# CookiePPP/cookietts

Hardware: AMD Instinct MI355X
Metric: audio samples/sec (22.05kHz) WaveGlow infer, 80×900 mel, 1/2/4/8 GPU; real-time factor (higher is better)
Workload: dtype f32; 1 GPU; WaveGlow full (12 flows, 512 WN ch, 8 groups, 8 layers) fp32 infer, batch 8 x (80x900) mel per GPU, sigma 0.6, random-init weights; batch_per_gpu=8, frames=900, parallelism=utterance-batch shard x1

## Files before the change

cookietts_amd/_lib.py:

```python
from __future__ import annotations

import ctypes as C
import os
import threading

import torch

from . import build as _build

_LOCK = threading.Lock()
_LIB = None


class WaveGlowConfig(C.Structure):
    _fields_ = [(n, C.c_int32) for n in (
        "n_mel_channels", "n_group", "n_flows", "n_early_every", "n_early_size",
        "win_length", "hop_length", "n_layers", "n_channels", "kernel_size", "cond_hidden", "speaker_embed_dim",
        "f32_gemm_mode")]


class StftConfig(C.Structure):
    _fields_ = [("filter_length", C.c_int32), ("hop_length", C.c_int32), ("win_length", C.c_int32),
                ("n_mel_channels", C.c_int32), ("clamp_val", C.c_float)]

# ... 70 lines not shown


class TorchMojiConfig(C.Structure):
    _fields_ = [(n, C.c_int32) for n in ("nb_tokens", "embedding_dim", "hidden_size")]


class TorchMojiWeights(C.Structure):
    _fields_ = [("embed", _FP), ("lstm", (LstmWeights * 2) * 2), ("attention_vector", _FP)]


class TacoDecoderWeights(C.Structure):
    _fields_ = [("bottleneck_w", _FP), ("memory_layer_w", _FP), ("query_w", _FP), ("v_w", _FP), ("loc_conv_w", _FP),
                ("loc_dense_w", _FP), ("prenet_w1", _FP), ("prenet_w2", _FP),
                ("att_rnn", LstmWeights), ("dec_rnn", LstmWeights), ("dec2_rnn", LstmWeights),
                ("proj_w", _FP), ("proj_b", _FP), ("gate_w", _FP), ("gate_b", _FP),
                ("windowed_att_pos_offset", C.c_float), ("exp_smoothing_factor", C.c_float)]


class Conv1dDesc(C.Structure):
    _fields_ = [("c_in", C.c_int32), ("c_out", C.c_int32), ("kernel_size", C.c_int32), ("act", C.c_int32),
                ("slope", C.c_float), ("f32_gemm_mode", C.c_int32)]


class HifiganConfig(C.Structure):
    MAX_UPS, MAX_KERNELS, MAX_DILATIONS = 8, 4, 3
    _fields_ = [(n, C.c_int32) for n in ("num_mels", "upsample_initial_channel", "resblock", "n_ups", "n_kernels")] + [
        ("upsample_rates", C.c_int32 * 8), ("upsample_kernel_sizes", C.c_int32 * 8), ("resblock_kernel_sizes", C.c_int32 * 4),
        ("resblock_dilation_sizes", (C.c_int32 * 3) * 4)]


class TacoMemoryWeights(C.Structure):
    _fields_ = [(n, _FP) for n in ("sylps_w", "sylps_b", "speaker_embedding", "syl_w0", "syl_b0", "syl_w2", "syl_b2",
                                   "syl_res_weight", "tm_gamma", "tm_beta", "tm_mean", "tm_var", "tm_w", "tm_b")]


class RetryConfig(C.Structure):
    _fields_ = [(n, C.c_double) for n in ("diagonality_weighting", "max_focus_weighting", "min_focus_weighting",
                                          "avg_focus_weighting", "target_score", "absolutely_required_score")] + [
        (n, C.c_int32) for n in ("max_attempts", "absolute_maximum_tries", "n_texts", "per_text", "n_mel", "t_cap", "enc_cap")]


class RetryStatus(C.Structure):
    _fields_ = [("done", C.c_int32), ("n_passes", C.c_int32), ("min_best_score", C.c_double), ("min_tries", C.c_int32),
                ("n_without_winner", C.c_int32), ("max_best_length", C.c_int32), ("max_best_T", C.c_int32)]


class MelErrorConfig(C.Structure):
    _fields_ = [("n_windows", C.c_int32), ("filter_lengths", C.c_int32 * 8), ("hop_length", C.c_int32),
                ("n_mel_channels", C.c_int32), ("framing", C.c_int32), ("clamp_val", C.c_float), ("mag_eps", C.c_float)]


class TacoLossParams(C.Structure):
    _fields_ = [("gate_positive_weight", C.c_double), ("sigma", C.c_double), ("weights", C.c_double * 9)]


_CFG = C.POINTER(WaveGlowConfig)
SIGNATURES = {
    "ctts_abi_version": (C.c_int, []),
    "ctts_last_error": (C.c_char_p, []),
    "ctts_waveglow_geometry_for": (C.c_int, [_CFG, C.c_int32, C.POINTER(WaveGlowGeometry)]),
    "ctts_fold_weightnorm_f32": (C.c_int, [_FP, _FP, _FP, C.c_int32, C.c_int32, _FP]),
    "ctts_waveglow_packed_bytes": (C.c_size_t, [_CFG]),
    "ctts_waveglow_pack_upsample": (C.c_int, [_CFG, _FP, _FP, _FP, _FP]),
    "ctts_waveglow_pack_flow": (C.c_int, [_CFG, C.c_int32, C.POINTER(WaveGlowFlowWeights), _FP, _FP]),
    "ctts_waveglow_workspace_bytes": (C.c_size_t, [_CFG, C.c_int32, C.c_int32]),
    "ctts_waveglow_infer_f32": (C.c_int, [_CFG, _FP, _FP, _FP, _FP, C.c_int32, C.c_int32, _FP, C.c_size_t, _FP]),
    "ctts_waveglow_infer_spk_f32": (C.c_int, [_CFG, _FP, _FP, _FP, _FP, _FP, C.c_int32, C.c_int32, _FP, C.c_size_t, _FP]),
    "ctts_waveglow_infer_spk_bf16": (C.c_int, [_CFG, _FP, _FP, _FP, _FP, _FP, _FP, C.c_int32, C.c_int32, _FP, C.c_size_t,
                                              _FP]),
    "ctts_waveglow_infer_spk_bf16x3": (C.c_int, [_CFG, _FP, _FP, _FP, _FP, _FP, _FP, C.c_int32, C.c_int32, _FP, C.c_size_t,
                                               _FP]),
    "ctts_waveglow_infer_spk_f16": (C.c_int, [_CFG, _FP, _FP, _FP, _FP, _FP, _FP, C.c_int32, C.c_int32, _FP, C.c_size_t,
                                             _FP]),
    "ctts_waveglow_pack_flow_f16": (C.c_int, [_CFG, C.c_int32, C.POINTER(WaveGlowFlowWeights), _FP, _FP]),
    "ctts_waveglow_packed_bf16x3_bytes": (C.c_size_t, [_CFG]),
    "ctts_waveglow_pack_flow_bf16x3": (C.c_int, [_CFG, C.c_int32, C.POINTER(WaveGlowFlowWeights), _FP, _FP]),
    "ctts_waveglow_workspace_bf16x3_bytes": (C.c_size_t, [_CFG, C.c_int32, C.c_int32]),
    "ctts_waveglow_packed_bf16_bytes": (C.c_size_t, [_CFG]),
    "ctts_waveglow_pack_flow_bf16": (C.c_int, [_CFG, C.c_int32, C.POINTER(WaveGlowFlowWeights), _FP, _FP]),
    "ctts_waveglow_workspace_bf16_bytes": (C.c_size_t, [_CFG, C.c_int32, C.c_int32]),
    "ctts_waveglow_infer_bf16": (C.c_int, [_CFG, _FP, _FP, _FP, _FP, _FP, C.c_int32, C.c_int32, _FP, C.c_size_t, _FP]),
    "ctts_upsample_squeeze_f32": (C.c_int, [_CFG, _FP, _FP, _FP, C.c_int32, C.c_int32, _FP]),
    "ctts_wn_cond_f32": (C.c_int, [_CFG, _FP, _FP, _FP, _FP, _FP, C.c_int32, C.c_int32, _FP]),
    "ctts_wn_stack_f32": (C.c_int, [_CFG, _FP, C.c_int32, _FP, _FP, _FP, _FP, _FP, C.c_int32, C.c_int32, _FP]),
    "ctts_flow_tail_f32": (C.c_int, [_CFG, _FP, C.c_int32, _FP, _FP, _FP, C.c_int32, C.c_int32, _FP]),
    "ctts_waveglow_flow_f32": (C.c_int, [_CFG, _FP, C.c_int32, _FP, _FP, _FP, C.c_int32, C.c_int32, _FP, C.c_size_t, _FP]),
    "ctts_waveglow_forward_packed_bytes": (C.c_size_t, [_CFG]),
    "ctts_waveglow_pack_forward_mix": (C.c_int, [_CFG, C.c_int32, _FP, _FP, _FP]),
    "ctts_waveglow_forward_workspace_bytes": (C.c_size_t, [_CFG, C.c_int32, C.c_int32]),
    "ctts_waveglow_forward_spk_f32": (C.c_int, [_CFG, _FP, _FP, _FP, _FP, _FP, _FP, _FP, _FP, C.c_int32, C.c_int32, _FP,
                                               C.c_size_t, _FP]),
    "ctts_waveglow_flow_forward_f32": (C.c_int, [_CFG, _FP, _FP, C.c_int32, _FP, _FP, _FP, _FP, _FP, C.c_int32, C.c_int32, _FP,
                                                C.c_size_t, _FP]),
    "ctts_waveflow_packed_bytes": (C.c_size_t, [C.POINTER(WaveFlowConfig)]),
    "ctts_waveflow_pack_flow": (C.c_int, [C.POINTER(WaveFlowConfig), C.c_int32, C.POINTER(WaveFlowFlowWeights), _FP, _FP]),
    "ctts_waveflow_workspace_bytes": (C.c_size_t, [C.POINTER(WaveFlowConfig), C.c_int32, C.c_int32]),
    "ctts_waveflow_inverse_f32": (C.c_int, [C.POINTER(WaveFlowConfig), _FP, _FP, _FP, _FP, C.c_int32, C.c_int32,
                                            C.c_int32, _FP, C.c_size_t, _FP]),
    "ctts_taco_decoder_packed_bytes": (C.c_size_t, [C.POINTER(TacoDecoderConfig)]),
    "ctts_taco_decoder_pack": (C.c_int, [C.POINTER(TacoDecoderConfig), C.POINTER(TacoDecoderWeights), _FP, _FP]),
    "ctts_taco_decoder_max_batch": (C.c_int32, [C.POINTER(TacoDecoderConfig)]),
    "ctts_taco_decoder_workspace_bytes": (C.c_size_t, [C.POINTER(TacoDecoderConfig), C.c_int32, C.c_int32]),
    "ctts_taco_decoder_init_f32": (C.c_int, [C.POINTER(TacoDecoderConfig), _FP, _FP, _FP, C.c_int32, C.c_int32, _FP,
                                             C.c_size_t, _FP]),
    "ctts_taco_decoder_steps_f32": (C.c_int, [C.POINTER(TacoDecoderConfig), _FP, _FP, _FP, _FP, _FP, C.c_int32,
                                              C.c_int32, C.c_int32, C.c_int32, C.c_int32, _FP, _FP]),
    "ctts_taco_decoder_steps_hidden_f32": (C.c_int, [C.POINTER(TacoDecoderConfig), _FP, _FP, _FP, _FP, _FP, _FP, C.c_int32,
                                                     C.c_int32, C.c_int32, C.c_int32, C.c_int32, _FP, _FP]),
    "ctts_taco_decoder_packed_bf16x3_bytes": (C.c_size_t, [C.POINTER(TacoDecoderConfig)]),
    "ctts_taco_decoder_pack_bf16x3": (C.c_int, [C.POINTER(TacoDecoderConfig), C.POINTER(TacoDecoderWeights), _FP, _FP]),
    "ctts_taco_decoder_steps_bf16x3": (C.c_int, [C.POINTER(TacoDecoderConfig), _FP, _FP, _FP, _FP, _FP, _FP, C.c_int32,
                                                 C.c_int32, C.c_int32, C.c_int32, C.c_int32, _FP, _FP]),
    "ctts_taco_prenet_frames_bytes": (C.c_size_t, [C.POINTER(TacoDecoderConfig), C.c_int32, C.c_int32]),
    "ctts_taco_prenet_frames_f32": (C.c_int, [C.POINTER(TacoDecoderConfig), _FP, _FP, _FP, _FP, _FP, C.c_size_t, C.c_int32,
                                              C.c_int32, _FP]),
    "ctts_taco_decoder_steps_forced_f32": (C.c_int, [C.POINTER(TacoDecoderConfig), _FP, _FP, _FP, _FP, C.c_int32, C.c_int32,
                                                     C.c_int32, C.c_int32, C.c_int32, _FP, C.c_size_t, _FP]),
    "ctts_taco_decoder_steps_forced_bf16x3": (C.c_int, [C.POINTER(TacoDecoderConfig), _FP, _FP, _FP, _FP, C.c_int32, C.c_int32,
                                                        C.c_int32, C.c_int32, C.c_int32, _FP, C.c_size_t, _FP]),
    "ctts_taco_project_frames_f32": (C.c_int, [C.POINTER(TacoDecoderConfig), _FP, _FP, _FP, _FP, C.c_int32, C.c_int32, _FP]),
    "ctts_taco_decoder_persistent_bytes": (C.c_size_t, [C.POINTER(TacoDecoderConfig), C.c_int32, C.c_int32]),
    "ctts_taco_decoder_steps_persistent_f32": (C.c_int, [C.POINTER(TacoDecoderConfig), _FP, _FP, _FP, _FP, _FP, C.c_int32,
                                                         C.c_int32, C.c_int32, C.c_int32, C.c_int32, _FP, _FP, C.c_size_t,
                                                         _FP]),
    "ctts_taco_decoder_persistent_debug": (C.c_int, [_FP]),
    "ctts_conv1d_packed_bytes": (C.c_size_t, [C.POINTER(Conv1dDesc)]),
    "ctts_conv1d_pack_f32": (C.c_int, [C.POINTER(Conv1dDesc), _FP, _FP, _FP, _FP, _FP, _FP, C.c_float, _FP, _FP]),
    "ctts_conv1d_f32": (C.c_int, [C.POINTER(Conv1dDesc), _FP, _FP, _FP, C.c_int32, C.c_int32, C.c_int32, C.c_int32,
                                  C.c_int32, _FP]),
    "ctts_lstm_seq_packed_bytes": (C.c_size_t, [C.c_int32, C.c_int32]),
    "ctts_lstm_seq_pack_f32": (C.c_int, [C.POINTER(LstmWeights), C.c_int32, C.c_int32, _FP, _FP]),
    "ctts_lstm_seq_workspace_bytes": (C.c_size_t, [C.c_int32, C.c_int32, C.c_int32]),
    "ctts_lstm_seq_f32": (C.c_int, [_FP, _FP, _FP, C.c_int32, _FP, C.c_int64, C.c_int32, C.c_int32, _FP, C.c_int32,
                                    C.c_int32, C.c_int32, C.c_int32, C.c_int32, C.c_int32, C.c_int32, C.c_int32, _FP,
                                    C.c_size_t, _FP]),
    "ctts_lstm_biseq_f32": (C.c_int, [_FP, _FP, _FP, _FP, _FP, C.c_int64, C.c_int32, C.c_int32, C.c_int32, _FP, C.c_int32,
                                      C.c_int32, C.c_int32, C.c_int32, C.c_int32, C.c_int32, C.c_int32, C.c_int32, C.c_int32,
                                      _FP, _FP, C.c_size_t, _FP]),
    "ctts_lstm_biseq_hardsig_f32": (C.c_int, [_FP, _FP, _FP, _FP, _FP, C.c_int64, C.c_int32, C.c_int32, C.c_int32, _FP, C.c_int32,
                                              C.c_int32, C.c_int32, C.c_int32, C.c_int32, C.c_int32, C.c_int32, C.c_int32,
                                              C.c_int32, _FP, _FP, C.c_size_t, _FP]),
    "ctts_torchmoji_packed_bytes": (C.c_size_t, [C.POINTER(TorchMojiConfig)]),
    "ctts_torchmoji_pack_f32": (C.c_int, [C.POINTER(TorchMojiConfig), C.POINTER(TorchMojiWeights), _FP, _FP]),
    "ctts_torchmoji_workspace_bytes": (C.c_size_t, [C.POINTER(TorchMojiConfig), C.c_int32, C.c_int32]),
    "ctts_torchmoji_lengths": (C.c_int, [_FP, _FP, C.c_int32, C.c_int32, _FP]),
    "ctts_torchmoji_features_f32": (C.c_int, [C.POINTER(TorchMojiConfig), _FP, _FP, _FP, _FP, _FP, C.c_int32, C.c_int32, _FP,
                                              C.c_size_t, _FP]),
    "ctts_attention_pool_f32": (C.c_int, [_FP, _FP, _FP, _FP, _FP, C.c_int32, C.c_int32, C.c_int32, _FP]),
    "ctts_taco_embed_f32": (C.c_int, [_FP, _FP, _FP, _FP, _FP, C.c_int32, C.c_int32, C.c_int32, C.c_int32, C.c_int32,
                                      C.c_int32, _FP]),
    "ctts_taco_memory_f32": (C.c_int, [C.POINTER(TacoMemoryWeights), _FP, _FP, _FP, _FP, _FP, C.c_int32, C.c_int32,
                                       C.c_int32, C.c_int32, C.c_int32, C.c_int32, C.c_int32, _FP]),
    "ctts_taco_memory_sylps_f32": (C.c_int, [C.POINTER(TacoMemoryWeights), _FP, _FP, _FP, _FP, _FP, _FP, C.c_int32, C.c_int32,
                                             C.c_int32, C.c_int32, C.c_int32, C.c_int32, C.c_int32, _FP]),
    "ctts_pad_rows_f32": (C.c_int, [_FP, C.c_int64, C.c_int32, _FP, C.c_int32, C.c_int32, C.c_int32, C.c_int32,
                                    C.c_int32, _FP]),
    "ctts_unpad_rows_f32": (C.c_int, [_FP, _FP, C.c_int64, C.c_int32, C.c_int32, C.c_int32, C.c_int32, C.c_int32,
                                      C.c_int32, _FP]),
    "ctts_stft_packed_bytes": (C.c_size_t, [C.POINTER(StftConfig)]),
    "ctts_stft_pack": (C.c_int, [C.POINTER(StftConfig), _FP, _FP, _FP, _FP]),
    "ctts_stft_workspace_bytes": (C.c_size_t, [C.POINTER(StftConfig), C.c_int32, C.c_int32]),
    "ctts_stft_mel_f32": (C.c_int, [C.POINTER(StftConfig), _FP, _FP, _FP, _FP, C.c_int32, C.c_int32, _FP,
                                    C.c_size_t, _FP]),
    "ctts_stft_pack_inverse": (C.c_int, [C.POINTER(StftConfig), _FP, _FP, _FP, _FP]),
    "ctts_stft_transform_f32": (C.c_int, [C.POINTER(StftConfig), _FP, _FP, _FP, _FP, C.c_int32, C.c_int32, _FP,
                                          C.c_size_t, _FP]),
# ... 15 lines not shown
    "ctts_wgax_packed_bytes": (C.c_size_t, [C.POINTER(WgaxConfig)]),
    "ctts_wgax_pack_flow": (C.c_int, [C.POINTER(WgaxConfig), C.c_int32, C.POINTER(WgaxFlowWeights), _FP, _FP]),
    "ctts_wgax_workspace_bytes": (C.c_size_t, [C.POINTER(WgaxConfig), C.c_int32, C.c_int64]),
    "ctts_wgax_inverse_f32": (C.c_int, [C.POINTER(WgaxConfig), _FP, _FP, _FP, C.c_int32, C.c_int32, C.c_int32, _FP,
                                        C.c_int32, C.c_int64, _FP, C.c_size_t, _FP]),
    "ctts_wgax_packed_f16_bytes": (C.c_size_t, [C.POINTER(WgaxConfig)]),
    "ctts_wgax_pack_flow_f16": (C.c_int, [C.POINTER(WgaxConfig), C.c_int32, C.POINTER(WgaxFlowWeights), _FP, _FP]),
    "ctts_wgax_workspace_f16_bytes": (C.c_size_t, [C.POINTER(WgaxConfig), C.c_int32, C.c_int64]),
    "ctts_wgax_inverse_f16": (C.c_int, [C.POINTER(WgaxConfig), _FP, _FP, _FP, C.c_int32, C.c_int32, C.c_int32, _FP,
                                        C.c_int32, C.c_int64, _FP, C.c_size_t, _FP]),
    "ctts_wgax_sep_packed_bytes": (C.c_size_t, [C.POINTER(WgaxConfig)]),
    "ctts_wgax_sep_pack_flow": (C.c_int, [C.POINTER(WgaxConfig), C.c_int32, C.POINTER(WgaxFlowWeights), C.POINTER(_FP),
                                          C.POINTER(_FP), _FP, _FP]),
    "ctts_wgax_sep_workspace_bytes": (C.c_size_t, [C.POINTER(WgaxConfig), C.c_int32, C.c_int64]),
    "ctts_wgax_sep_inverse_f32": (C.c_int, [C.POINTER(WgaxConfig), _FP, _FP, _FP, C.c_int32, C.c_int32, C.c_int32, _FP,
                                            C.c_int32, C.c_int64, _FP, C.c_size_t, _FP]),
    "ctts_depthwise_conv1d_f32": (C.c_int, [_FP, _FP, _FP, _FP] + [C.c_int32] * 7 + [_FP]),
    "ctts_hifigan_weight_floats": (C.c_size_t, [C.POINTER(HifiganConfig)]),
    "ctts_hifigan_packed_bytes": (C.c_size_t, [C.POINTER(HifiganConfig)]),
    "ctts_hifigan_pack_f32": (C.c_int, [C.POINTER(HifiganConfig), _FP, C.c_size_t, _FP, _FP]),
    "ctts_hifigan_workspace_bytes": (C.c_size_t, [C.POINTER(HifiganConfig), C.c_int32, C.c_int32]),
    "ctts_hifigan_forward_f32": (C.c_int, [C.POINTER(HifiganConfig), _FP, _FP, C.c_int32, _FP, C.c_int32, C.c_int32, _FP,
                                           C.c_size_t, _FP]),
    "ctts_hifigan_packed_f16_bytes": (C.c_size_t, [C.POINTER(HifiganConfig)]),
    "ctts_hifigan_pack_f16": (C.c_int, [C.POINTER(HifiganConfig), _FP, C.c_size_t, _FP, _FP]),
    "ctts_hifigan_workspace_f16_bytes": (C.c_size_t, [C.POINTER(HifiganConfig), C.c_int32, C.c_int32]),
    "ctts_hifigan_forward_f16": (C.c_int, [C.POINTER(HifiganConfig), _FP, _FP, C.c_int32, _FP, C.c_int32, C.c_int32, _FP,
                                           C.c_size_t, _FP]),
    "ctts_hifigan_packed_bf16x3_bytes": (C.c_size_t, [C.POINTER(HifiganConfig)]),
    "ctts_hifigan_pack_bf16x3": (C.c_int, [C.POINTER(HifiganConfig), _FP, C.c_size_t, _FP, _FP]),
    "ctts_hifigan_workspace_bf16x3_bytes": (C.c_size_t, [C.POINTER(HifiganConfig), C.c_int32, C.c_int32]),
    "ctts_hifigan_forward_bf16x3": (C.c_int, [C.POINTER(HifiganConfig), _FP, _FP, C.c_int32, _FP, C.c_int32, C.c_int32, _FP,
                                              C.c_size_t, _FP]),
    "ctts_replicate_halo_f32":(C.c_int, [_FP, C.c_int32, C.c_int32, C.c_int32, C.c_int32, C.c_int32, C.c_int32, _FP]),
    "ctts_embed_rows_f32": (C.c_int, [_FP, _FP, _FP, C.c_int32, C.c_int32, C.c_int32, C.c_int32, C.c_int32, C.c_int32,
                                      C.c_int32, _FP]),
    "ctts_scale_add_rows_f32": (C.c_int, [_FP, _FP, _FP, _FP, C.c_int32, C.c_int32, C.c_int32, C.c_int32, C.c_int32,
                                          _FP]),
    "ctts_deemphasis_f32": (C.c_int, [_FP, _FP, C.c_int32, C.c_int32, C.c_double, _FP]),
    "ctts_alignment_workspace_bytes": (C.c_size_t, [C.c_int32, C.c_int32, C.c_int32]),
    "ctts_alignment_metric_f32": (C.c_int, [_FP, _FP, _FP, C.c_int32, C.c_int32, C.c_int32, C.c_float, _FP, _FP,
                                            C.c_size_t, _FP]),
    "ctts_alignment_metric_masked_f32": (C.c_int, [_FP, _FP, _FP, _FP, C.c_int32, C.c_int32, C.c_int32, C.c_float, _FP, _FP,
                                                   C.c_size_t, _FP]),
    "ctts_first_over_thresh_f32": (C.c_int, [_FP, C.c_int32, C.c_int32, C.c_float, _FP, _FP]),
    "ctts_taco_loss_workspace_bytes": (C.c_size_t, [C.c_int32] * 4),
    "ctts_taco_loss_f32": (C.c_int, [C.POINTER(TacoLossParams)] + [_FP] * 13 + [C.c_int32] * 4 + [_FP, _FP, _FP, C.c_size_t,
                                                                                                  _FP]),
    "ctts_taco_loss_finalize_f32": (C.c_int, [C.POINTER(TacoLossParams)] + [_FP] * 9 + [C.c_int32] * 4 + [_FP, _FP, _FP,
                                                                                                          C.c_size_t, _FP]),
    "ctts_mel_error_packed_bytes": (C.c_size_t, [C.POINTER(MelErrorConfig)]),
    "ctts_mel_error_pack": (C.c_int, [C.POINTER(MelErrorConfig), C.c_int32, _FP, _FP, _FP, _FP]),
    "ctts_mel_error_workspace_bytes": (C.c_size_t, [C.POINTER(MelErrorConfig)] + [C.c_int32] * 3),
    "ctts_mel_error_f32": (C.c_int, [C.POINTER(MelErrorConfig)] + [_FP] * 6 + [C.c_int32] * 5 + [_FP] * 4 + [C.c_int32, _FP,
                                                                                                     C.c_size_t, _FP]),
    "ctts_taco_stop_state_bytes": (C.c_size_t, [C.c_int32]),
    "ctts_taco_stop_reset": (C.c_int, [_FP, C.c_int32, C.c_int32, _FP]),
    "ctts_taco_stop_rule_f32": (C.c_int, [_FP, C.c_int32, C.c_int32, C.c_int32, C.c_int32, C.c_float, C.c_int32, _FP, _FP]),
    "ctts_retry_state_bytes": (C.c_size_t, [C.POINTER(RetryConfig)]),
    "ctts_retry_state_layout": (C.c_int, [C.POINTER(RetryConfig), C.POINTER(C.c_size_t)]),
    "ctts_retry_reset": (C.c_int, [C.POINTER(RetryConfig), _FP, _FP]),
    "ctts_retry_update_f32": (C.c_int, [C.POINTER(RetryConfig), _FP, _FP, _FP, _FP, _FP, _FP, C.c_int32, C.c_int32, _FP, _FP,
                                        _FP]),
    "ctts_retry_vocoder_batch_f32": (C.c_int, [C.POINTER(RetryConfig), _FP, _FP, C.c_int32, C.c_float, _FP]),
    "ctts_pcm16_concat": (C.c_int, [_FP, C.c_int32, _FP, C.c_int32, C.c_int64, C.c_int32, C.c_int32, _FP, C.c_int64, _FP,
                                    _FP]),
    "ctts_affine_rows_f32": (C.c_int, [_FP, C.c_int32, C.c_int32, C.c_int32, C.c_int32, C.c_int32, C.c_int32, C.c_float,
                                       C.c_float, _FP]),
    "ctts_vol_unscale_f32": (C.c_int, [_FP, C.c_int64, _FP]),
    "ctts_resample_rows_f32": (C.c_int, [_FP, _FP] + [C.c_int32] * 9 + [C.c_float, _FP]),
    "ctts_interleave_phases_f32": (C.c_int, [_FP, _FP] + [C.c_int32] * 10 + [_FP]),
    "ctts_last_gemm_loop": (C.c_int, []),
    "ctts_last_winograd_f43_width": (C.c_int, []),
    "ctts_tuning_reload": (C.c_int, []),
    "ctts_tuning_flags": (C.c_int, []),
    "ctts_profile_create": (C.c_int, [C.POINTER(C.c_void_p)]),
    "ctts_profile_bind": (C.c_int, [C.c_void_p]),
    "ctts_profile_collect": (C.c_int, [C.c_void_p, C.c_int32, C.POINTER(C.c_int64), C.POINTER(C.c_double)]),
    "ctts_profile_destroy": (C.c_int, [C.c_void_p]),
}

MODEL_GEMM_MODES = {None: 0, "default": 0, "f32": 1, "bf16x3": 2, "bf16x6": 3}
GEMM_MODES = {"f32": 1, "bf16x3": 2, "bf16x6": 3}


def model_gemm_mode(mode):
    try:
        return MODEL_GEMM_MODES[mode]
    except KeyError:
        raise ValueError(f"f32 GEMM mode {mode!r}: expected one of 'default', 'f32', 'bf16x3', 'bf16x6'") from None


def set_f32_gemm_mode(mode):
    if mode in (None, "default", "f32"):
        return "f32"
    raise RuntimeError(f"cookietts_amd.set_f32_gemm_mode({mode!r}): the process-wide default was removed; "
                       f"call model.set_f32_gemm_mode({mode!r}) on each model instead")


class Profile:

    def __init__(self):
        h = C.c_void_p()
        check(lib().ctts_profile_create(C.byref(h)), "ctts_profile_create")
        self._h = h

    def __enter__(self):
        check(lib().ctts_profile_bind(self._h), "ctts_profile_bind")
        return self

    def __exit__(self, *exc):
        check(lib().ctts_profile_bind(None), "ctts_profile_bind")
        return False

    bind = __enter__

    def unbind(self):
        self.__exit__()

    def collect(self, which):
        n, ms = C.c_int64(), C.c_double()
        check(lib().ctts_profile_collect(self._h, which, C.byref(n), C.byref(ms)), "ctts_profile_collect")
        return int(n.value), float(ms.value)

    def close(self):
        if self._h is not None and _LIB is not None:
            _LIB.ctts_profile_destroy(self._h)
        self._h = None

    def __del__(self):
        try:
            self.close()
        except Exception:
            pass


TUNING_BITS = {"CTTS_F32_NO_GLDS": 0, "CTTS_GEMM_NO_XCD_PAIR": 1, "CTTS_F32_WINOGRAD_FUSED_MIN": 2, "CTTS_BF16_NO_WIDE": 3, "CTTS_BF16_NO_PP": 4,
               "CTTS_F32_WINOGRAD_NO_FUSED": 5, "CTTS_F32_WINOGRAD_F43_MIN": 6, "CTTS_WF_NO_FUSE": 7,
               "CTTS_TACO_NO_FUSE": 8, "CTTS_F32_NO_SMALL": 9, "CTTS_F32_FORCE_SMALL": 10, "CTTS_F32_NO_SPLITK": 11, "CTTS_WF_NO_VEC_INTERP": 12,
               "CTTS_F32_NO_DEFER_SKIP": 13, "CTTS_WF_NO_REGION_SPLIT": 14, "CTTS_WF_NO_ROW_QUEUE": 15, "CTTS_WF_ROW_QUEUE_MIN": 16,
               "CTTS_WF_INJECT_ABORT": 17, "CTTS_WF_QUEUE_DEBUG": 18, "CTTS_F32_NO_ROUND_SPLIT": 19, "CTTS_BF16_PS": 20, "CTTS_BF16_NO_PS": 21,
               "CTTS_F32_WINOGRAD_NO_F43": 22,
               "CTTS_TACO_POLL_DELAY": 23, "CTTS_TACO_VALU": 24, "CTTS_UP_NO_MFMA": 25, "CTTS_F32_NO_WN_FOLD": 26, "CTTS_TACO_BG_NO_PIPE": 27,
               "CTTS_F32_NO_WINOGRAD": 28, "CTTS_F32_WINOGRAD_MIN": 29, "CTTS_F32_WINOGRAD_PLAIN": 30}
TUNING_BITS_EXT = {"CTTS_WF_FWD_ROWWISE": 31}


def tuning_reload():
    check(lib().ctts_tuning_reload(), "ctts_tuning_reload")


def tuning_active(name):
    bit = TUNING_BITS[name] if name in TUNING_BITS else TUNING_BITS_EXT[name]
    return bool(lib().ctts_tuning_flags() >> bit & 1)


PROF_WN_IN = 0
PROF_WN_RS = 1
PROF_WN_SKIP = 2
PROF_WN_IN0F = 3
PROF_WN_SKEND = 4
PROF_WN_RES_F = 5


class HipLibraryError(RuntimeError):
    pass
# ... 61 lines not shown
```

cookietts_amd/csrc/gemm_f32.h:

```cpp
#pragma once

#include "common.h"

namespace ctts {

constexpr int GEMM_KC = 16;
constexpr int GEMM_MAX_SEG = 12;

constexpr int GEMM_BM = 256;
constexpr int GEMM_BN = 128;
inline int gemm_bn(int bm) { return bm == 256 ? 128 : 256; }

enum GemmEpilogue : int {
    GEMM_EPI_SPLIT = 0,
    GEMM_EPI_GATE = 1,
    GEMM_EPI_MAG = 2,
    GEMM_EPI_LOG = 3,
    GEMM_EPI_LRELU = 4,
    GEMM_EPI_TANH = 5,
    GEMM_EPI_GATEX = 7,
    GEMM_EPI_GATE_RS = 6,
};

__host__ __device__ inline bool gemm_epi_is_pair(int epi) {
    return epi == GEMM_EPI_GATE || epi == GEMM_EPI_MAG || epi == GEMM_EPI_GATE_RS || epi == GEMM_EPI_GATEX;
}

enum GateKind : int {
    GATE_GTU = 0,
    GATE_GTRU = 1,
    GATE_GTLRU = 2,
    GATE_GLU = 3,
    GATE_TTU = 4,
    GATE_STU = 5,
    GATE_GTSU = 6,
    GATE_SPTU = 7,
    GATE_GSIU = 8,
    GATE_GSIRU = 9,
    GATE_GTSRU = 10,
    GATE_GSIRRU = 11,
    GATE_GSIRLRU = 12,
    GATE_GSIRRLRU = 13,
    GATE_KINDS = 14
};

#if defined(__HIPCC__)
__device__ __forceinline__ float gemm_lerp(float l0, float a, float l1, float b) { return __builtin_fmaf(l0, a, l1 * b); }

template <int KIND>
__device__ __forceinline__ float gate_eval(float u0, float u1) {
    float f, g;
    if constexpr (KIND == GATE_GLU) f = u0;
    else if constexpr (KIND == GATE_GTSU || KIND == GATE_GTSRU) f = u0 - tanhf(u0);
    else if constexpr (KIND == GATE_GSIU) f = __sinf(u0);
    else if constexpr (KIND == GATE_GSIRU || KIND == GATE_GSIRRU || KIND == GATE_GSIRLRU || KIND == GATE_GSIRRLRU) f = __sinf(16.0f * u0);
    else f = tanhf(u0);
    if constexpr (KIND == GATE_GTRU || KIND == GATE_GTSRU || KIND == GATE_GSIRRU) g = fmaxf(u1, 0.0f);
    else if constexpr (KIND == GATE_GTLRU || KIND == GATE_GSIRLRU) g = u1 > 0.0f ? u1 : 0.01f * u1;
    else if constexpr (KIND == GATE_GSIRRLRU) g = u1 >= 0.0f ? u1 : ((0.01f + 0.1f) / 2.0f) * u1;
    else if constexpr (KIND == GATE_TTU) g = tanhf(u1);
    else if constexpr (KIND == GATE_STU)
        g = 1.0507009873554804934193349852946f * (fmaxf(u1, 0.0f) + fminf(0.0f, 1.6732632423543772848170429916717f * expm1f(u1)));
    else if constexpr (KIND == GATE_SPTU) g = u1 > 20.0f ? u1 : log1pf(expf(u1));
    else g = 1.0f / (1.0f + expf(-u1));
    return f * g;
}
#endif

struct GemmSeg {
    const float* base;
    long long bstride;
    int nch;
    int shift;
    int mb_rows;
    int fresh;
};

struct GemmArgs {
    const float* A;
    const float* bias;
    GemmSeg seg[GEMM_MAX_SEG];
    int nseg;
    int interleave;
    int nch_total;
    int a_nch_alloc;
    int a_ch_off;
    int bm;
    int ld, pad, L;
    int ntiles, MB, batch;
    int M;
    float* dst0; long long dst0_bstride; int acc0;
    const float* src0; long long src0_bstride;
    float* dst1; long long dst1_bstride; int acc1;
    int split;
    int pairC;
    int dst_ld, dst_pad;
    float clip;
    const float* addend; long long addend_bstride;
    int addend_ld, addend_pad;
    int addend_frames;
    const float* addend2; float addend2_sign;
    int map_d, map_par, map_L, map_col0;
    int map_mode;
    int gate;
    int gemm_mode;
    const float* rs_wT;
    const float* rs_bias;
    int rs_rows;
    int gt_limit;
    long long shape_blocks;
    int parts;
    long long part_A, part_seg[4], part_dst0;
    int mseg, mseg_ld, mseg_pad;
    int mseg_ch0, mseg_ch1;
};

__host__ __device__ inline int gemm_dense_row(int epi, int bm, int mb, int r, int C, int M) {
    if (gemm_epi_is_pair(epi)) {
        const int wm = r >> 7, rr = r & 127;
        const int c = (mb * (bm >> 7) + wm) * 64 + (rr & 63);
        if (c >= C) return -1;
        return (rr < 64) ? c : C + c;
    }
    const int row = mb * bm + r;
    return row < M ? row : -1;
}

inline void gemm_apply_defaults(GemmArgs& a) {
    if (a.bm == 0) a.bm = 256;
    if (a.addend_ld == 0) { a.addend_ld = a.ld; a.addend_pad = a.pad; }
}
bool gemm_f32_dma_staged(int nch_total);
int gemm_check_args(int epi, const GemmArgs& a);
int launch_gemm_f32(int epi, const GemmArgs& a, hipStream_t stream);
bool gemm_f32_small_applies(int epi, const GemmArgs& a);
int launch_gemm_f32_small(int epi, const GemmArgs& a, hipStream_t stream);

bool wf_row_persistent_supported(const GemmArgs& a);
int wf_row_cus();
int wf_row_tiles(int L, int body);
struct WfTailDesc;
int launch_wf_row_persistent(const GemmArgs* layers_dev, const WfTailDesc* tails_dev, int nrows, int nlayers, int max_nseg, int L,
                             int batch, int body, unsigned int* counter, unsigned int* flags, unsigned int* abort_word,
                             unsigned int epoch, hipStream_t stream);

int launch_wf_all_rows_layer(const GemmArgs* rows_dev, int nrows, int max_nseg, int L, int batch, hipStream_t stream);

int get_gemm_f32_mode();
void note_gemm_loop(int code);
int last_gemm_loop();
bool gemm_mode_is_split(int gemm_mode);
inline bool gemm_mode_valid(int m) { return m == CTTS_GEMM_DEFAULT || m == CTTS_GEMM_F32 || m == CTTS_GEMM_BF16X3 || m == CTTS_GEMM_BF16X6; }
int gemm_split_level(int gemm_mode);

}
```

cookietts_amd/csrc/gemm_f32.hip:

```cpp
#include <atomic>
#include <cstdlib>
#include <mutex>

#include "gemm_f32.h"
#include "tuning.h"
#include "gemm_bf16.h"

namespace ctts {

typedef float f32x16 __attribute__((ext_vector_type(16)));

namespace {

constexpr int STAGE = GEMM_KC * (256 + 128);
constexpr int GEMM_GLDS_MAX_CHUNKS = 384;

__device__ __forceinline__ float fast_sigmoid(float u) {
    return __builtin_amdgcn_rcpf(1.0f + __builtin_amdgcn_exp2f(u * -1.4426950408889634f));
}
__device__ __forceinline__ float fast_tanh(float u) {
    return 1.0f - 2.0f * __builtin_amdgcn_rcpf(1.0f + __builtin_amdgcn_exp2f(u * 2.8853900817779268f));
}

typedef const __attribute__((address_space(1))) float* gfloat_ptr;
__device__ __forceinline__ float4 load4u(gfloat_ptr p) {
    float4 v;
    v.x = p[0]; v.y = p[1]; v.z = p[2]; v.w = p[3];
    return v;
}

template <int EPI>
__device__ __forceinline__ void split_epilogue(const GemmArgs& a, f32x16 (&acc)[4][2], const float* bias, int M, int row0,
                                               int b, int ncol0, int l31, int lhi, long long part_dst0 = 0) {
#pragma unroll
    for (int mt = 0; mt < 4; ++mt) {
        const int rbase = row0 + mt * 32;
        if (rbase >= M) continue;
        const bool second = rbase >= a.split;
        float* dst = second ? a.dst1 + (size_t)b * a.dst1_bstride : a.dst0 + part_dst0 + (size_t)b * a.dst0_bstride;
        const float* src = second ? dst : (a.src0 ? a.src0 + (size_t)b * a.src0_bstride : dst);
        const int accum = second ? a.acc1 : a.acc0;
        const int rdst = second ? rbase - a.split : rbase;
        float old[2][16];
        if (accum && rbase + 32 <= M) {
#pragma unroll
            for (int nt = 0; nt < 2; ++nt)
#pragma unroll
                for (int r = 0; r < 16; ++r) {
                    const int row = (r & 3) + 8 * (r >> 2) + 4 * lhi;
                    old[nt][r] = src[(size_t)(rdst + row) * a.dst_ld + a.dst_pad + ncol0 + nt * 32 + l31];
                }
        } else if (accum) {
#pragma unroll
            for (int nt = 0; nt < 2; ++nt)
#pragma unroll
                for (int r = 0; r < 16; ++r) {
                    const int row = (r & 3) + 8 * (r >> 2) + 4 * lhi;
                    old[nt][r] = rbase + row < M ? src[(size_t)(rdst + row) * a.dst_ld + a.dst_pad + ncol0 + nt * 32 + l31] : 0.0f;
                }
        } else {
#pragma unroll
            for (int nt = 0; nt < 2; ++nt)
#pragma unroll
                for (int r = 0; r < 16; ++r) old[nt][r] = 0.0f;
        }
#pragma unroll
        for (int nt = 0; nt < 2; ++nt) {
            const int n = ncol0 + nt * 32 + l31;
            if (n < a.L) {
#pragma unroll
                for (int r = 0; r < 16; ++r) {
                    const int row = (r & 3) + 8 * (r >> 2) + 4 * lhi;
                    float v = acc[mt][nt][r] + bias[(rbase - row0) + row] + old[nt][r];
                    if constexpr (EPI == GEMM_EPI_LOG) v = logf(fmaxf(v, a.clip));
                    if constexpr (EPI == GEMM_EPI_LRELU) v = v > 0.f ? v : a.clip * v;
                    if constexpr (EPI == GEMM_EPI_TANH) v = tanhf(v);
                    if (rbase + row < M) dst[(size_t)(rdst + row) * a.dst_ld + a.dst_pad + n] = v;
                }
            }
        }
    }
}

typedef __bf16 bf16x8_t __attribute__((ext_vector_type(8)));
typedef unsigned int u32x4_t __attribute__((ext_vector_type(4)));
__device__ __forceinline__ void split8(const float (&v)[8], u32x4_t& hi, u32x4_t& lo) {
#pragma unroll
    for (int j = 0; j < 4; ++j) {
        const unsigned int h = pack_bf16x2(v[2 * j], v[2 * j + 1]);
        hi[j] = h;
        lo[j] = pack_bf16x2(v[2 * j] - __builtin_bit_cast(float, h << 16), v[2 * j + 1] - __builtin_bit_cast(float, h & 0xffff0000u));
    }
}

__device__ __forceinline__ void split8x3(const float (&v)[8], u32x4_t& hi, u32x4_t& mid, u32x4_t& lo) {
#pragma unroll
    for (int j = 0; j < 4; ++j) {
        const unsigned int h = pack_bf16x2(v[2 * j], v[2 * j + 1]);
        const float r0 = v[2 * j] - __builtin_bit_cast(float, h << 16), r1 = v[2 * j + 1] - __builtin_bit_cast(float, h & 0xffff0000u);
        const unsigned int m = pack_bf16x2(r0, r1);
        hi[j] = h;
        mid[j] = m;
        lo[j] = pack_bf16x2(r0 - __builtin_bit_cast(float, m << 16), r1 - __builtin_bit_cast(float, m & 0xffff0000u));
    }
}

template <int EPI, int WM, int SEGS, bool GLDS, int XS = 0, bool EXT = false>
__global__ __launch_bounds__(256, 2) void conv_gemm_f32_kernel(const GemmArgs a) {
    static_assert(!EXT || (GLDS && SEGS == 4 && XS == 0 && (EPI == GEMM_EPI_SPLIT || EPI == GEMM_EPI_GATE)),
                  "parts / mapped segment: DMA-staged fp32 loop, <= 4 segments, SPLIT or GATE");
    constexpr bool X3 = XS != 0;
    constexpr bool X6 = XS == 6;
    static_assert(XS == 0 || XS == 3 || XS == 6, "main loop: fp32 MFMA, 3 or 6 bf16 products");
    static_assert(!X3 || GLDS, "the split-bf16 loop is built on the DMA-staged pipeline");
    constexpr int NST = GLDS ? 3 : 2;
    constexpr int SEGTAB = NST * STAGE;
    constexpr int CHTAB = SEGTAB + GEMM_MAX_SEG * 4;
    constexpr int LDS_FLOATS = CHTAB + (GLDS ? 2 * GEMM_GLDS_MAX_CHUNKS : 0);
    constexpr int BM = 128 * WM;
    constexpr int WN = 4 / WM;
    constexpr int BN = 64 * WN;
    constexpr int A_STAGE = GEMM_KC * BM;
    constexpr int NA = BM / 64;
    constexpr int NB = BN / 64;
    __shared__ __attribute__((aligned(16))) float lds[LDS_FLOATS];

    const int t = threadIdx.x;
    const int lane = t & 63;
    const int wave = GLDS ? __builtin_amdgcn_readfirstlane(t >> 6) : (t >> 6);
    const int wm = wave / WN, wn = wave % WN;
    const int l31 = lane & 31, lhi = lane >> 5;

    int id = blockIdx.x;
    int mb, tile, b;
    if (a.map_mode == 1) {
        const int x = id & 7, j = id >> 3;
        mb = 2 * (x & 1) + (j & 1);
        const int gt = (j >> 1) * 4 + (x >> 1);
        if (gt >= a.gt_limit) return;
        tile = gt % a.ntiles;
        b = gt / a.ntiles;
    } else {
        mb = id % a.MB;
        id /= a.MB;
        tile = id % a.ntiles;
        b = id / a.ntiles;
    }
    const int n0 = tile * BN;
    [[maybe_unused]] int part = 0;
    if constexpr (EXT) {
        if (b >= a.batch) { part = 1; b -= a.batch; }
    }
#define CTTS_MAP_PAR (EXT && a.parts > 1 ? part : a.map_par)
#define CTTS_A_PTR (EXT ? a.A + (long long)part * a.part_A : a.A)

    gfloat_ptr sbase[4];
    int snch[4];
    if constexpr (SEGS == 4) {
#pragma unroll
        for (int sidx = 0; sidx < 4; ++sidx) {
            const GemmSeg& g = a.seg[sidx];
            sbase[sidx] = (gfloat_ptr)(g.base + (size_t)b * g.bstride + (size_t)(mb * g.mb_rows) * a.ld +
                                       (a.pad + n0 + g.shift));
            snch[sidx] = sidx < a.nseg ? g.nch : 0x7fffffff;
        }
    } else {
#pragma unroll
        for (int sidx = 0; sidx < GEMM_MAX_SEG; ++sidx) {
            if (t == sidx) {
                const GemmSeg& g = a.seg[sidx];
                unsigned int* e = reinterpret_cast<unsigned int*>(lds + SEGTAB + sidx * 4);
                if (sidx < a.nseg) {
                    const float* base = g.base + (size_t)b * g.bstride + (size_t)(mb * g.mb_rows) * a.ld +
                                        (a.pad + n0 + g.shift);
                    const unsigned long long u = reinterpret_cast<unsigned long long>(base);
                    e[0] = (unsigned int)u;
                    e[1] = (unsigned int)(u >> 32);
                    e[2] = (unsigned int)g.nch;
                } else {
                    e[0] = 0; e[1] = 0; e[2] = 0x7fffffffu;
                }
                e[3] = 0;
            }
        }
    }

    const int nalloc = a.a_nch_alloc ? a.a_nch_alloc : a.nch_total;
    const float* ap = CTTS_A_PTR + ((size_t)mb * nalloc + a.a_ch_off) * A_STAGE + t * 4;

    constexpr int UPR = BN / 4;
    constexpr int RPP = 64 / UPR;
    const int brow = GLDS ? wave * RPP + lane / UPR : t >> 4;
    const int bcol = GLDS ? (lane % UPR) * 4 : (t & 15) * 4;
    const size_t thread_off = (size_t)brow * a.ld + bcol;
    const size_t piece_stride = (size_t)4 * RPP * a.ld;
    const size_t chunk_rows = (size_t)GEMM_KC * a.ld;

    f32x16 acc[4][2];
#pragma unroll
    for (int i = 0; i < 4; ++i)
#pragma unroll
        for (int j = 0; j < 2; ++j)
#pragma unroll
            for (int r = 0; r < 16; ++r) acc[i][j][r] = 0.0f;

    float4 ra0, ra1, ra2, ra3, rb0, rb1, rb2, rb3;
    int seg = 0, local = 0;
    const int ilv = a.interleave > 1 ? a.interleave : 0;
    bool in_ilv = ilv > 0;
    if constexpr (SEGS != 4) __syncthreads();
    if constexpr (GLDS) {
        unsigned long long* tab = reinterpret_cast<unsigned long long*>(lds + CHTAB);
        const int ilv0 = a.interleave > 1 ? a.interleave : 0;
        const int n_il = ilv0 * a.seg[0].nch;
        for (int c0 = t; c0 < a.nch_total; c0 += 256) {
            int c = c0, sg, loc;
            if (c < n_il) {
                sg = c % ilv0;
// ... 339 lines not shown
                            }                                                                                     \
                            break;
                        switch (a.gate) {
                            CTTS_GATEX_LOOP(1) CTTS_GATEX_LOOP(2) CTTS_GATEX_LOOP(3) CTTS_GATEX_LOOP(4) CTTS_GATEX_LOOP(5)
                            CTTS_GATEX_LOOP(6) CTTS_GATEX_LOOP(7) CTTS_GATEX_LOOP(8) CTTS_GATEX_LOOP(9) CTTS_GATEX_LOOP(10)
                            CTTS_GATEX_LOOP(11) CTTS_GATEX_LOOP(12) CTTS_GATEX_LOOP(13)
                            default:
                            CTTS_GATEX_LOOP(0)
                        }
#undef CTTS_GATEX_LOOP
                    } else {
                        float add20[16], add21[16];
                        if (EPI == GEMM_EPI_GATE && a.addend2) {
                            const float* ad = a.addend2 + (size_t)b * a.addend_bstride + a.addend_pad + n;
#pragma unroll
                            for (int r = 0; r < 16; ++r) {
                                const int c = min(cbase + mt * 32 + (r & 3) + 8 * (r >> 2) + 4 * lhi, a.pairC - 1);
                                add20[r] = (EXT && part ? -a.addend2_sign : a.addend2_sign) * ad[(size_t)c * a.addend_ld];
                                add21[r] = (EXT && part ? -a.addend2_sign : a.addend2_sign) * ad[(size_t)(a.pairC + c) * a.addend_ld];
                            }
                        }
#pragma unroll
                        for (int r = 0; r < 16; ++r) {
                            const int row = (r & 3) + 8 * (r >> 2) + 4 * lhi;
                            const int c = cbase + mt * 32 + row;
                            float u0 = acc[mt][nt][r] + bias[mt * 32 + row] + add0[r];
                            float u1 = acc[mt + 2][nt][r] + bias[64 + mt * 32 + row] + add1[r];
                            if (EPI == GEMM_EPI_GATE && a.addend2) { u0 += add20[r]; u1 += add21[r]; }
                            float v;
                            if constexpr (EPI == GEMM_EPI_GATE) v = fast_tanh(u0) * fast_sigmoid(u1);
                            else v = sqrtf(u0 * u0 + u1 * u1);
                            if (c < a.pairC && ns_ok) dst[(size_t)c * a.dst_ld + a.dst_pad + ns] = v;
                        }
                    }
                }
            }
        }
    } else if constexpr (EPI == GEMM_EPI_GATE_RS) {
        static_assert(EPI != GEMM_EPI_GATE_RS || WM == 1, "fused res/skip needs the 128-row block shape");
        float actv[2][2][16];
#pragma unroll
        for (int mt = 0; mt < 2; ++mt)
#pragma unroll
            for (int nt = 0; nt < 2; ++nt)
#pragma unroll
                for (int r = 0; r < 16; ++r) {
                    const int row = (r & 3) + 8 * (r >> 2) + 4 * lhi;
                    const bool ok = mt * 32 + row < a.pairC;
                    float u0 = acc[mt][nt][r] + bias[mt * 32 + row];
                    float u1 = acc[mt + 2][nt][r] + bias[64 + mt * 32 + row];
                    if (a.addend) {
                        const float* ad = a.addend + (size_t)b * a.addend_bstride + a.addend_pad + n0 + wn * 64 + nt * 32 + l31;
                        const int c = min(mt * 32 + row, a.pairC - 1);
                        u0 += ad[(size_t)c * a.addend_ld];
                        u1 += ad[(size_t)(a.pairC + c) * a.addend_ld];
                    }
                    actv[mt][nt][r] = ok ? fast_tanh(u0) * fast_sigmoid(u1) : 0.0f;
                }
        __syncthreads();
        for (int i = t * 4; i < 64 * 128; i += 1024)
            *reinterpret_cast<float4*>(lds + i) = *reinterpret_cast<const float4*>(a.rs_wT + i);
        if (t < 128) lds[64 * 128 + t] = a.rs_bias[t];
        __syncthreads();
#pragma unroll
        for (int i = 0; i < 4; ++i)
#pragma unroll
            for (int j = 0; j < 2; ++j)
#pragma unroll
                for (int r = 0; r < 16; ++r) acc[i][j][r] = 0.0f;
#pragma unroll
        for (int s = 0; s < 32; ++s) {
            const int r = s & 15;
            const int ch = (s >> 4) * 32 + (r & 3) + 8 * (r >> 2) + 4 * lhi;
            float a2[4];
#pragma unroll
            for (int mt = 0; mt < 4; ++mt) a2[mt] = lds[ch * 128 + mt * 32 + l31];
#pragma unroll
            for (int mt = 0; mt < 4; ++mt)
#pragma unroll
                for (int nt = 0; nt < 2; ++nt)
                    acc[mt][nt] = __builtin_amdgcn_mfma_f32_32x32x2f32(a2[mt], actv[s >> 4][nt][r], acc[mt][nt], 0, 0, 0);
        }
        split_epilogue<GEMM_EPI_SPLIT>(a, acc, lds + 64 * 128, a.rs_rows, 0, b, n0 + wn * 64, l31, lhi);
    } else {
        split_epilogue<EPI>(a, acc, bias, a.M, mb * BM + wm * 128, b, n0 + wn * 64, l31, lhi, EXT ? (long long)part * a.part_dst0 : 0);
    }
#undef CTTS_MAP_PAR
#undef CTTS_A_PTR
}

inline int gemm_f32_mode() { return CTTS_GEMM_F32; }

template <int EPI, int XS>
void launch_shape_xs(int bm, dim3 grid, hipStream_t stream, const GemmArgs& a) {
    const bool few = a.nseg <= 4;
    if (bm == 128) {
        if (few) hipLaunchKernelGGL((conv_gemm_f32_kernel<EPI, 1, 4, true, XS>), grid, dim3(256), 0, stream, a);
        else hipLaunchKernelGGL((conv_gemm_f32_kernel<EPI, 1, GEMM_MAX_SEG, true, XS>), grid, dim3(256), 0, stream, a);
    } else {
        if (few) hipLaunchKernelGGL((conv_gemm_f32_kernel<EPI, 2, 4, true, XS>), grid, dim3(256), 0, stream, a);
        else hipLaunchKernelGGL((conv_gemm_f32_kernel<EPI, 2, GEMM_MAX_SEG, true, XS>), grid, dim3(256), 0, stream, a);
    }
}

template <int EPI, bool GLDS>
void launch_shape_g(int bm, dim3 grid, hipStream_t stream, const GemmArgs& a) {
    const bool few = a.nseg <= 4;
    if (bm == 128) {
        if (few) hipLaunchKernelGGL((conv_gemm_f32_kernel<EPI, 1, 4, GLDS>), grid, dim3(256), 0, stream, a);
        else hipLaunchKernelGGL((conv_gemm_f32_kernel<EPI, 1, GEMM_MAX_SEG, GLDS>), grid, dim3(256), 0, stream, a);
    } else {
        if (few) hipLaunchKernelGGL((conv_gemm_f32_kernel<EPI, 2, 4, GLDS>), grid, dim3(256), 0, stream, a);
        else hipLaunchKernelGGL((conv_gemm_f32_kernel<EPI, 2, GEMM_MAX_SEG, GLDS>), grid, dim3(256), 0, stream, a);
    }
}

template <int EPI>
void launch_shape(int bm, dim3 grid, hipStream_t stream, const GemmArgs& a) {
    if (tuning().f32_no_glds || a.nch_total > GEMM_GLDS_MAX_CHUNKS) launch_shape_g<EPI, false>(bm, grid, stream, a);
    else if (gemm_split_level(a.gemm_mode) == 6) launch_shape_xs<EPI, 6>(bm, grid, stream, a);
    else if (gemm_split_level(a.gemm_mode) == 3) launch_shape_xs<EPI, 3>(bm, grid, stream, a);
    else launch_shape_g<EPI, true>(bm, grid, stream, a);
}

}

int get_gemm_f32_mode() { return gemm_f32_mode(); }
namespace { thread_local int t_last_loop = 0; }
void note_gemm_loop(int code) { t_last_loop = code; }
int last_gemm_loop() { return t_last_loop; }
int gemm_split_level(int m) {
    if (m == CTTS_GEMM_DEFAULT) m = gemm_f32_mode();
    if (m == CTTS_GEMM_BF16X3) return 3;
    if (m == CTTS_GEMM_BF16X6) return 6;
    return 0;
}
bool gemm_mode_is_split(int m) { return gemm_split_level(m) != 0; }

namespace {
std::mutex g_tune_mu;
Tuning g_tune{};
bool g_tune_loaded = false;
void load_tuning_locked() {
    auto on = [](const char* n) { return getenv(n) != nullptr; };
    auto num = [](const char* n, int d) { const char* v = getenv(n); return v ? atoi(v) : d; };
    g_tune.f32_no_glds = on("CTTS_F32_NO_GLDS");
    g_tune.f32_no_small = on("CTTS_F32_NO_SMALL");
    g_tune.f32_force_small = on("CTTS_F32_FORCE_SMALL");
    g_tune.f32_no_splitk = on("CTTS_F32_NO_SPLITK");
    g_tune.f32_no_round_split = on("CTTS_F32_NO_ROUND_SPLIT");
    g_tune.no_xcd_pair = on("CTTS_GEMM_NO_XCD_PAIR");
    g_tune.bf16_no_wide = on("CTTS_BF16_NO_WIDE");
    g_tune.bf16_no_pp = on("CTTS_BF16_NO_PP");
    g_tune.bf16_wide_min = num("CTTS_BF16_WIDE_MIN", 192);
    g_tune.bf16_ps = on("CTTS_BF16_PS");
    g_tune.bf16_no_ps = on("CTTS_BF16_NO_PS");
    g_tune.wf_no_fuse = on("CTTS_WF_NO_FUSE");
    g_tune.taco_no_fuse = on("CTTS_TACO_NO_FUSE");
    g_tune.taco_valu = on("CTTS_TACO_VALU");
    g_tune.up_no_mfma = on("CTTS_UP_NO_MFMA");
    g_tune.taco_bg_no_pipe = on("CTTS_TACO_BG_NO_PIPE");
    {
        static const int dflt[6] = {0x10000 | 36, 0x10000 | 96, 0x10000 | 12, 0x10000 | 20, 0x10000 | 8, 0x10000 | 8};
        int v[6];
        for (int i = 0; i < 6; ++i) v[i] = dflt[i];
        const char* e = getenv("CTTS_TACO_POLL_DELAY");
        if (e && sscanf(e, "%d,%d,%d,%d,%d,%d", v, v + 1, v + 2, v + 3, v + 4, v + 5) != 6)
            for (int i = 0; i < 6; ++i) v[i] = dflt[i];
        for (int i = 0; i < 6; ++i) g_tune.taco_poll_delay[i] = v[i] < 0 ? 0 : v[i];
        g_tune.taco_poll_delay_set = e != nullptr;
    }
    g_tune.wf_no_vec_interp = on("CTTS_WF_NO_VEC_INTERP");
    g_tune.wf_fwd_rowwise = on("CTTS_WF_FWD_ROWWISE");
    g_tune.wf_no_region_split = on("CTTS_WF_NO_REGION_SPLIT");
    g_tune.wf_no_row_queue = on("CTTS_WF_NO_ROW_QUEUE");
    g_tune.wf_row_queue_min = num("CTTS_WF_ROW_QUEUE_MIN", -1);
    g_tune.wf_inject_abort = num("CTTS_WF_INJECT_ABORT", 0);
    g_tune.wf_queue_debug = num("CTTS_WF_QUEUE_DEBUG", 0);
    g_tune.f32_no_defer_skip = on("CTTS_F32_NO_DEFER_SKIP");
    g_tune.f32_no_wn_fold = on("CTTS_F32_NO_WN_FOLD");
    g_tune.f32_no_winograd = on("CTTS_F32_NO_WINOGRAD");
    g_tune.f32_winograd_min = num("CTTS_F32_WINOGRAD_MIN", -1);
    g_tune.f32_winograd_plain = on("CTTS_F32_WINOGRAD_PLAIN");
    g_tune.f32_winograd_fused_min = num("CTTS_F32_WINOGRAD_FUSED_MIN", -1);
    g_tune.f32_winograd_no_fused = on("CTTS_F32_WINOGRAD_NO_FUSED");
    g_tune.f32_winograd_f43_min = num("CTTS_F32_WINOGRAD_F43_MIN", -1);
    g_tune.f32_winograd_no_f43 = on("CTTS_F32_WINOGRAD_NO_F43");
    g_tune_loaded = true;
}
}

Tuning tuning() {
    std::lock_guard<std::mutex> lk(g_tune_mu);
    if (!g_tune_loaded) load_tuning_locked();
    return g_tune;
}
void reload_tuning() {
    std::lock_guard<std::mutex> lk(g_tune_mu);
    load_tuning_locked();
}

int gemm_check_args(int epi, const GemmArgs& a) {
    CTTS_CHECK_ARG(a.bm == 256 || a.bm == 128, "gemm: bm=%d", a.bm);
    CTTS_CHECK_ARG(gemm_mode_valid(a.gemm_mode), "gemm: f32_gemm_mode %d (0 default, 1 fp32 MFMA, 2 split bf16)", a.gemm_mode);
    const int bn = gemm_bn(a.bm);
    CTTS_CHECK_ARG(a.nseg >= 1 && a.nseg <= GEMM_MAX_SEG, "gemm: nseg=%d", a.nseg);
    int nch = 0;
    for (int s = 0; s < a.nseg; ++s) {
        CTTS_CHECK_ARG(a.seg[s].nch > 0 && a.seg[s].base, "gemm: empty segment %d", s);
        CTTS_CHECK_ARG(a.seg[s].shift >= -a.pad && a.seg[s].shift <= a.pad,
                       "gemm: shift %d exceeds halo %d", a.seg[s].shift, a.pad);
        nch += a.seg[s].nch;
    }
    CTTS_CHECK_ARG(nch == a.nch_total, "gemm: chunk count mismatch %d vs %d", nch, a.nch_total);
    if (a.interleave > 1) {
        CTTS_CHECK_ARG(a.interleave <= a.nseg, "gemm: interleave %d > nseg %d", a.interleave, a.nseg);
        for (int s = 1; s < a.interleave; ++s)
            CTTS_CHECK_ARG(a.seg[s].nch == a.seg[0].nch, "gemm: interleaved segments must have equal length");
    }
    CTTS_CHECK_ARG(a.a_nch_alloc == 0 || a.a_ch_off + a.nch_total <= a.a_nch_alloc, "gemm: A chunk window");
    CTTS_CHECK_ARG(a.ld % 4 == 0 && a.ntiles * bn + 2 * a.pad <= a.ld && a.L <= a.ntiles * bn,
                   "gemm: bad geometry ld=%d pad=%d L=%d ntiles=%d bn=%d", a.ld, a.pad, a.L, a.ntiles, bn);
    CTTS_CHECK_ARG(gemm_epi_is_pair(epi) || a.split % 32 == 0, "gemm: split %d not a multiple of 32", a.split);
    const int cpb = a.bm / 2;
    CTTS_CHECK_ARG(gemm_epi_is_pair(epi) ? (a.pairC > (a.MB - 1) * cpb && a.pairC <= a.MB * cpb)
                                         : (a.M > (a.MB - 1) * a.bm && a.M <= a.MB * a.bm),
                   "gemm: M=%d pairC=%d MB=%d bm=%d", a.M, a.pairC, a.MB, a.bm);
    CTTS_CHECK_ARG(a.dst_ld > 0 && a.dst0, "gemm: destination not set");
    CTTS_CHECK_ARG(a.addend_frames == 0 || ((epi == GEMM_EPI_GATE || epi == GEMM_EPI_GATEX) && a.addend && a.addend_frames <= a.addend_ld - a.addend_pad),
                   "gemm: interpolated addend needs the GATE epilogue (frames=%d)", a.addend_frames);
    CTTS_CHECK_ARG(a.gate >= 0 && a.gate < GATE_KINDS && (a.gate == 0 || epi == GEMM_EPI_GATE), "gemm: gate=%d with epilogue %d",
                   a.gate, epi);
    CTTS_CHECK_ARG((a.addend2 == nullptr && a.map_d == 0) ||
                       (epi == GEMM_EPI_GATE && a.gate == GATE_GTU && a.addend_frames == 0 && a.map_d >= 0 &&
                        (a.addend2 == nullptr || (a.addend && (a.addend2_sign == 1.0f || a.addend2_sign == -1.0f))) &&
                        (a.map_d == 0 || ((a.map_par == 0 || a.map_par == 1) && a.map_L > 0 && a.map_col0 >= 0))),
                   "gemm: second addend / mapped store need the GATE epilogue (epilogue %d, map_d=%d)", epi, a.map_d);
    CTTS_CHECK_ARG(epi != GEMM_EPI_GATE_RS ||
                       (a.bm == 128 && a.pairC <= 64 && a.MB == 1 && a.rs_wT && a.rs_bias && (a.rs_rows == 64 || a.rs_rows == 128)),
                   "gemm: fused res/skip needs bm=128, <= 64 channels, rs_wT / rs_bias and 64 or 128 res/skip rows");
    const int parts = a.parts > 1 ? a.parts : 1;
    CTTS_CHECK_ARG(a.parts >= 0 && a.parts <= 2 && (a.mseg == 0 || a.mseg == 2), "gemm: parts=%d mseg=%d", a.parts, a.mseg);
    if (parts > 1 || a.mseg) {
        CTTS_CHECK_ARG((epi == GEMM_EPI_SPLIT || (epi == GEMM_EPI_GATE && a.gate == GATE_GTU)) && a.bm == 256 && a.nseg <= 4 &&
                           a.interleave <= 1 && gemm_split_level(a.gemm_mode) == 0 && a.shape_blocks == 0 && a.addend_frames == 0,
                       "gemm: parts / mapped segment need the fp32 SPLIT or GATE launch of the 256-row shape (epilogue %d, nseg=%d)", epi, a.nseg);
        CTTS_CHECK_ARG(parts == 1 || epi != GEMM_EPI_SPLIT || (a.acc0 == 0 && a.src0 == nullptr && a.split >= a.M),
                       "gemm: a two-part SPLIT launch stores every row to dst0");
        CTTS_CHECK_ARG(parts == 1 || (long long)parts * a.ntiles * a.batch < (1ll << 31) / a.MB, "gemm: merged grid");
    }
    if (a.mseg) {
        const GemmSeg& g = a.seg[1];
        CTTS_CHECK_ARG(epi == GEMM_EPI_GATE && a.nseg == 2 && a.map_d > 0 && a.map_d % 4 == 0 && a.map_col0 % 4 == 0 && a.mseg_pad >= 0 &&
                           a.mseg_pad % 4 == 0 && a.mseg_ld % 4 == 0 && a.mseg_ld - a.mseg_pad >= 4 && g.bstride % 4 == 0 &&
                           (parts == 1 || a.part_seg[1] % 4 == 0) && reinterpret_cast<uintptr_t>(g.base) % 16 == 0 && g.shift == 0 &&
                           g.mb_rows == 0,
                       "gemm: mapped segment d=%d col0=%d ld=%d pad=%d", a.map_d, a.map_col0, a.mseg_ld, a.mseg_pad);
    }
    return CTTS_OK;
}

bool gemm_f32_dma_staged(int nch_total) { return !tuning().f32_no_glds && nch_total <= GEMM_GLDS_MAX_CHUNKS; }

namespace {
GemmArgs gemm_part_args(const GemmArgs& a, int p) {
    GemmArgs r = a;
    r.parts = 0;
    if (p == 0) return r;
    r.A += a.part_A;
    for (int j = 0; j < r.nseg && j < 4; ++j) r.seg[j].base += a.part_seg[j];
    r.dst0 += a.part_dst0;
    r.map_par = p;
    r.addend2_sign = -a.addend2_sign;
    return r;
}
}

int launch_gemm_f32(int epi, const GemmArgs& a_in, hipStream_t stream) {
    GemmArgs a = a_in;
    gemm_apply_defaults(a);
    if (int rc = gemm_check_args(epi, a)) return rc;
    if (epi == GEMM_EPI_GATE && a.gate != GATE_GTU) epi = GEMM_EPI_GATEX;
    const int parts = a.parts > 1 ? a.parts : 1;
    const bool ext = parts > 1 || a.mseg;
    a.mseg_ch0 = a.mseg_ch1 = 0;
    if (a.mseg) { a.mseg_ch0 = a.seg[0].nch; a.mseg_ch1 = a.seg[0].nch + a.seg[1].nch; }
    CTTS_CHECK_ARG(!a.mseg || gemm_f32_dma_staged(a.nch_total), "gemm: the mapped segment needs the DMA-staged kernels");
    if (parts > 1 && (gemm_f32_small_applies(epi, a) || !gemm_f32_dma_staged(a.nch_total))) {
        for (int p = 0; p < parts; ++p)
            if (int rc = launch_gemm_f32(epi, gemm_part_args(a, p), stream)) return rc;
        return CTTS_OK;
    }
    if (gemm_f32_small_applies(epi, a)) return launch_gemm_f32_small(epi, a, stream);
    long long tiles = (long long)parts * a.ntiles * a.batch;
    if (a.bm == 256 && epi != GEMM_EPI_GATE_RS && a.addend_frames == 0 && a.shape_blocks == 0 && !tuning().f32_no_round_split &&
        !tuning().f32_no_glds && !tuning().f32_no_small && a.nch_total <= GEMM_GLDS_MAX_CHUNKS) {
        const long long slots = 2ll * wf_row_cus();
        const long long rounds = a.MB * tiles / slots;
        const long long rem_tiles = (a.MB * tiles - rounds * slots + a.MB - 1) / a.MB;
        if (rounds >= 2 && rem_tiles > 0 && rem_tiles * a.MB <= slots * 3 / 10 && rem_tiles < a.ntiles &&
            (long long)(a.ntiles - rem_tiles) * gemm_bn(a.bm) < a.L) {
            GemmArgs r = gemm_part_args(a, parts - 1);
            const int bn = gemm_bn(a.bm);
            const long long co = (long long)(a.ntiles - rem_tiles) * bn;
            const long long bo = a.batch - 1;
            for (int j = 0; j < r.nseg; ++j) r.seg[j].base += bo * r.seg[j].bstride + (r.mseg && j == 1 ? 0 : co);
            if (r.dst0) r.dst0 += bo * r.dst0_bstride + (r.map_d > 0 ? 0 : co);
            if (r.map_d > 0) r.map_col0 += (int)co;
            if (r.dst1) r.dst1 += bo * r.dst1_bstride + co;
            if (r.src0) r.src0 += bo * r.src0_bstride + co;
            if (r.addend) r.addend += bo * r.addend_bstride + co;
            if (r.addend2) r.addend2 += bo * r.addend_bstride + co;
            r.L = a.L - (int)co;
            r.ntiles = (int)rem_tiles;
            r.batch = 1;
            if (int rc = launch_gemm_f32_small(epi, r, stream)) return rc;
            tiles -= rem_tiles;
        }
    }
    a.gt_limit = (int)tiles;
    long long blocks = (long long)a.MB * tiles;
    a.map_mode = 0;
    if (a.MB == 4 && epi != GEMM_EPI_GATE_RS && !tuning().no_xcd_pair) {
        a.map_mode = 1;
        blocks = 16ll * ((tiles + 3) / 4);
    }
    CTTS_CHECK_ARG(blocks > 0 && blocks < (1ll << 31), "gemm: grid %lld", blocks);
    dim3 grid((unsigned)blocks);
    note_gemm_loop((tuning().f32_no_glds || a.nch_total > GEMM_GLDS_MAX_CHUNKS) ? 0 : gemm_split_level(a.gemm_mode));
    if (ext) {
        if (epi == GEMM_EPI_GATE) hipLaunchKernelGGL((conv_gemm_f32_kernel<GEMM_EPI_GATE, 2, 4, true, 0, true>), grid, dim3(256), 0, stream, a);
        else hipLaunchKernelGGL((conv_gemm_f32_kernel<GEMM_EPI_SPLIT, 2, 4, true, 0, true>), grid, dim3(256), 0, stream, a);
        CTTS_CHECK_LAUNCH("conv_gemm_f32");
        return CTTS_OK;
    }
    switch (epi) {
        case GEMM_EPI_GATEX: launch_shape<GEMM_EPI_GATEX>(a.bm, grid, stream, a); break;
        case GEMM_EPI_GATE: launch_shape<GEMM_EPI_GATE>(a.bm, grid, stream, a); break;
        case GEMM_EPI_GATE_RS:
            if (tuning().f32_no_glds || a.nch_total > GEMM_GLDS_MAX_CHUNKS) {
                if (a.nseg <= 4) hipLaunchKernelGGL((conv_gemm_f32_kernel<GEMM_EPI_GATE_RS, 1, 4, false>), grid, dim3(256), 0, stream, a);
                else hipLaunchKernelGGL((conv_gemm_f32_kernel<GEMM_EPI_GATE_RS, 1, GEMM_MAX_SEG, false>), grid, dim3(256), 0, stream, a);
            } else if (gemm_split_level(a.gemm_mode) == 6) {
                if (a.nseg <= 4) hipLaunchKernelGGL((conv_gemm_f32_kernel<GEMM_EPI_GATE_RS, 1, 4, true, 6>), grid, dim3(256), 0, stream, a);
                else hipLaunchKernelGGL((conv_gemm_f32_kernel<GEMM_EPI_GATE_RS, 1, GEMM_MAX_SEG, true, 6>), grid, dim3(256), 0, stream, a);
            } else if (gemm_split_level(a.gemm_mode) == 3) {
                if (a.nseg <= 4) hipLaunchKernelGGL((conv_gemm_f32_kernel<GEMM_EPI_GATE_RS, 1, 4, true, 3>), grid, dim3(256), 0, stream, a);
                else hipLaunchKernelGGL((conv_gemm_f32_kernel<GEMM_EPI_GATE_RS, 1, GEMM_MAX_SEG, true, 3>), grid, dim3(256), 0, stream, a);
            } else {
                if (a.nseg <= 4) hipLaunchKernelGGL((conv_gemm_f32_kernel<GEMM_EPI_GATE_RS, 1, 4, true>), grid, dim3(256), 0, stream, a);
                else hipLaunchKernelGGL((conv_gemm_f32_kernel<GEMM_EPI_GATE_RS, 1, GEMM_MAX_SEG, true>), grid, dim3(256), 0, stream, a);
            }
            break;
        case GEMM_EPI_MAG: launch_shape<GEMM_EPI_MAG>(a.bm, grid, stream, a); break;
        case GEMM_EPI_LOG: launch_shape<GEMM_EPI_LOG>(a.bm, grid, stream, a); break;
        case GEMM_EPI_LRELU: launch_shape<GEMM_EPI_LRELU>(a.bm, grid, stream, a); break;
        case GEMM_EPI_TANH: launch_shape<GEMM_EPI_TANH>(a.bm, grid, stream, a); break;
        case GEMM_EPI_SPLIT: launch_shape<GEMM_EPI_SPLIT>(a.bm, grid, stream, a); break;
        default: set_error("gemm: unknown epilogue %d", epi); return CTTS_E_ARG;
    }
    CTTS_CHECK_LAUNCH("conv_gemm_f32");
    return CTTS_OK;
}

}
```

cookietts_amd/csrc/tuning.h:

```cpp
#pragma once

namespace ctts {

struct Tuning {
    bool f32_no_glds;
    bool f32_no_small;
    bool f32_force_small;
    bool f32_no_splitk;
    bool f32_no_round_split;
    bool no_xcd_pair;
    bool bf16_no_wide;
    int bf16_wide_min;
    bool bf16_no_pp;
    bool bf16_ps;
    bool bf16_no_ps;
    bool wf_no_fuse;
    bool taco_poll_delay_set;
    int taco_poll_delay[6];
    bool taco_no_fuse;
    bool taco_bg_no_pipe;
    bool up_no_mfma;
    bool taco_valu;
    bool f32_no_defer_skip;
    bool f32_no_wn_fold;
    bool f32_no_winograd;
    int f32_winograd_min;
    bool f32_winograd_plain;
    int f32_winograd_fused_min;
    int f32_winograd_f43_min;
    bool f32_winograd_no_f43;
    bool f32_winograd_no_fused;
    bool wf_no_region_split;
    bool wf_no_row_queue;
    int wf_row_queue_min;
    int wf_queue_debug;
    int wf_inject_abort;
    bool wf_fwd_rowwise;
    bool wf_no_vec_interp;
};

Tuning tuning();
void reload_tuning();

}
```

cookietts_amd/csrc/waveglow_api.hip:

```cpp
#include <mutex>
#include <vector>

#include "gemm_bf16.h"
#include "gemm_f32.h"
#include "tuning.h"
#include "waveglow_kernels.h"
#include "wn_winograd_layer.h"

namespace ctts {

static thread_local char g_err[512] = "";

void set_error(const char* fmt, ...) {
    va_list ap;
    va_start(ap, fmt);
    vsnprintf(g_err, sizeof(g_err), fmt, ap);
    va_end(ap);
}

namespace {

constexpr size_t ALIGN_F = 64;
inline size_t align_up(size_t v) { return (v + ALIGN_F - 1) / ALIGN_F * ALIGN_F; }
constexpr int A_TILE = GEMM_KC * GEMM_BM;

struct FlowDims { int n_rem, n_half, ch_off; };

struct Plan {
    ctts_waveglow_config c;
    int C, H, K0, n_in;
    int S;
    int nch0, nch1h, nch_in, nch_rs;
    int mb_in;
    int nch_in0f;
    std::vector<FlowDims> fd;
    size_t up_w, up_wp, up_b, cond0_A, cond0_b, cond1_A, cond1_b;
    size_t zero_b;
    bool up_mfma;
    struct Flow {
        size_t start_w, start_b, end_w, end_b, winv, spk_tab;
        std::vector<size_t> in_A, in_b, rs_A, rs_b;
        std::vector<size_t> res_A, res_b, skip_A, skip_b;
        size_t in0f_w, in0f_A, skend_W, skend_b;
        std::vector<size_t> wg_T2_A, wg_T3_A, wg_e_A, wg_o_A;
        size_t wg_dense;
        std::vector<size_t> wq_U_A[4], wq_e_A, wq_o_A;
    };
    std::vector<Flow> fl;
    size_t total;

    static constexpr int F32_SKIP_GROUP = 4;
    int mb_c() const { return (C + GEMM_BM - 1) / GEMM_BM; }
    int n_groups() const { return (c.n_layers + F32_SKIP_GROUP - 1) / F32_SKIP_GROUP; }
    int group_layers(int g) const { return g + 1 < n_groups() ? F32_SKIP_GROUP : c.n_layers - g * F32_SKIP_GROUP; }
    int rs_rows(int layer) const { return layer < c.n_layers - 1 ? 2 * C : C; }
    int rs_mb(int layer) const { return (rs_rows(layer) + GEMM_BM - 1) / GEMM_BM; }
};

int make_plan(const ctts_waveglow_config* cfg, Plan& p) {
    CTTS_CHECK_ARG(cfg != nullptr, "config is NULL");
    p.c = *cfg;
    const auto& c = p.c;
    CTTS_CHECK_ARG(c.n_flows >= 1 && c.n_layers >= 1 && c.n_layers <= 12, "n_flows=%d n_layers=%d", c.n_flows, c.n_layers);
    CTTS_CHECK_ARG(gemm_mode_valid(c.f32_gemm_mode), "f32_gemm_mode=%d (CTTS_GEMM_DEFAULT / _F32 / _BF16X3 / _BF16X6)", c.f32_gemm_mode);
    CTTS_CHECK_ARG(c.n_group >= 4 && c.n_group % 4 == 0 && c.n_group <= 16, "n_group=%d (4, 8, 12 or 16)", c.n_group);
    CTTS_CHECK_ARG(c.kernel_size == 3, "kernel_size=%d (only 3 built)", c.kernel_size);
    CTTS_CHECK_ARG(c.n_channels >= 128 && c.n_channels % 128 == 0, "n_channels=%d (multiple of 128)", c.n_channels);
    CTTS_CHECK_ARG(c.cond_hidden == GEMM_BM, "cond_hidden=%d (reference hard-codes 256)", c.cond_hidden);
    CTTS_CHECK_ARG(c.hop_length > 0 && c.win_length % c.hop_length == 0 && c.hop_length % c.n_group == 0,
                   "win=%d hop=%d n_group=%d", c.win_length, c.hop_length, c.n_group);
    CTTS_CHECK_ARG((c.n_mel_channels * c.n_group) % GEMM_KC == 0, "n_mel*n_group=%d not a multiple of 16",
                   c.n_mel_channels * c.n_group);
    CTTS_CHECK_ARG(c.n_early_every >= 1 && c.n_early_size >= 0 && c.n_early_size % 2 == 0, "early outputs");
    CTTS_CHECK_ARG(c.speaker_embed_dim >= 0 && c.speaker_embed_dim <= 1024, "speaker_embed_dim=%d", c.speaker_embed_dim);
    p.C = c.n_channels;
    p.H = c.cond_hidden;
    p.K0 = c.n_mel_channels * c.n_group;
    p.S = round_up(c.speaker_embed_dim, 32);
    CTTS_CHECK_ARG(p.S == 0 || p.K0 % 32 == 0, "multispeaker needs n_mel*n_group %% 32 == 0");
    p.nch0 = (p.K0 + p.S) / GEMM_KC;
    p.nch1h = p.H / GEMM_KC;
    p.nch_in = (c.kernel_size * p.C + p.H) / GEMM_KC;
    p.nch_rs = p.C / GEMM_KC;
    p.mb_in = 2 * p.C / GEMM_BM;
    p.nch_in0f = c.kernel_size + p.nch1h;
    int n_half = c.n_group / 2, n_rem = c.n_group;
    p.fd.resize(c.n_flows);
    for (int k = 0; k < c.n_flows; ++k) {
        if (k % c.n_early_every == 0 && k > 0) { n_half -= c.n_early_size / 2; n_rem -= c.n_early_size; }
        CTTS_CHECK_ARG(n_half >= 1 && n_rem == 2 * n_half, "flow %d: n_half=%d n_remaining=%d", k, n_half, n_rem);
        p.fd[k] = {n_rem, n_half, c.n_group - n_rem};
    }
    size_t o = 0;
    auto take = [&](size_t n) { size_t r = o; o = align_up(o + n); return r; };
    p.up_w = take((size_t)c.n_mel_channels * c.n_mel_channels * c.win_length);
    p.up_mfma = upsample_mfma_shape(c.n_mel_channels, c.win_length, c.hop_length, c.n_group);
    p.up_wp = p.up_mfma ? take((size_t)c.n_mel_channels * c.n_mel_channels * c.win_length) : 0;
    p.up_b = take(c.n_mel_channels);
    p.cond0_A = take((size_t)c.n_flows * p.nch0 * A_TILE);
    p.cond0_b = take((size_t)c.n_flows * GEMM_BM);
    p.cond1_A = take((size_t)c.n_flows * p.nch1h * A_TILE);
    p.cond1_b = take((size_t)c.n_flows * GEMM_BM);
    p.zero_b = take((size_t)p.mb_in * GEMM_BM);
    p.fl.resize(c.n_flows);
    for (int k = 0; k < c.n_flows; ++k) {
        auto& f = p.fl[k];
        f.start_w = take((size_t)p.C * p.fd[k].n_half);
        f.start_b = take(p.C);
        f.end_w = take((size_t)2 * p.fd[k].n_half * p.C);
        f.end_b = take(2 * p.fd[k].n_half);
        f.winv = take((size_t)p.fd[k].n_rem * p.fd[k].n_rem);
        f.spk_tab = take((size_t)CTTS_N_SPEAKERS * c.speaker_embed_dim);
        for (int i = 0; i < c.n_layers; ++i) {
            f.in_A.push_back(take((size_t)p.mb_in * p.nch_in * A_TILE));
            f.in_b.push_back(take((size_t)p.mb_in * GEMM_BM));
            f.rs_A.push_back(take((size_t)p.rs_mb(i) * p.nch_rs * A_TILE));
            f.rs_b.push_back(take((size_t)p.rs_mb(i) * GEMM_BM));
            f.res_A.push_back(i + 1 < c.n_layers ? take((size_t)p.mb_c() * p.nch_rs * A_TILE) : 0);
            f.res_b.push_back(i + 1 < c.n_layers ? take((size_t)p.mb_c() * GEMM_BM) : 0);
        }
        for (int gi = 0; gi < p.n_groups(); ++gi) {
            f.skip_A.push_back(take((size_t)p.mb_c() * p.group_layers(gi) * p.nch_rs * A_TILE));
            f.skip_b.push_back(take((size_t)p.mb_c() * GEMM_BM));
        }
        f.in0f_w = take((size_t)2 * p.C * FOLD_ROWS * c.kernel_size);
        f.in0f_A = take((size_t)p.mb_in * p.nch_in0f * A_TILE);
        f.skend_W = take((size_t)c.n_layers * p.C * 2 * p.fd[k].n_half);
        f.skend_b = take(2 * p.fd[k].n_half);
        for (int i = 0; i < c.n_layers; ++i) {
            f.wg_T2_A.push_back(take((size_t)p.mb_in * p.nch_rs * A_TILE));
            f.wg_T3_A.push_back(take((size_t)p.mb_in * p.nch_rs * A_TILE));
            f.wg_e_A.push_back(take((size_t)p.mb_in * (p.nch_rs + p.nch1h) * A_TILE));
            f.wg_o_A.push_back(take((size_t)p.mb_in * (p.nch_rs + p.nch1h) * A_TILE));
        }
        const bool f43 = wn_winograd_layer_f43_supported(p.C, p.H);
        for (int i = 0; f43 && i < c.n_layers; ++i) {
            for (auto& u : f.wq_U_A) u.push_back(take((size_t)p.mb_in * p.nch_rs * A_TILE));
            f.wq_e_A.push_back(take((size_t)p.mb_in * (p.nch_rs + p.nch1h) * A_TILE));
            f.wq_o_A.push_back(take((size_t)p.mb_in * (p.nch_rs + p.nch1h) * A_TILE));
        }
        f.wg_dense = take((size_t)(f43 ? 6 : 3) * 2 * p.C * p.C);
    }
    p.total = o;
    return CTTS_OK;
}

struct Geom { int L, ld, pad, ntiles; };

int make_geom(const Plan& p, int frames, Geom& g) {
    CTTS_CHECK_ARG(frames >= 1, "frames=%d", frames);
    const long long T = (long long)frames * p.c.hop_length;
    g.L = (int)(T / p.c.n_group);
    int maxd = 1 << (p.c.n_layers - 1);
    g.pad = round_up(maxd > 128 ? maxd : 128, 32);
    g.ntiles = (g.L + GEMM_BN - 1) / GEMM_BN;
    g.ld = round_up(g.L, 256) + 2 * g.pad;
    return CTTS_OK;
}

struct PairGeom { int d, Lp, ntiles; };
PairGeom pair_geom(const Geom& g, int layer) {
    const int d = 1 << layer;
    const int Lp = (g.L + 2 * d - 1) / (2 * d) * d;
    return {d, Lp, (Lp + GEMM_BN - 1) / GEMM_BN};
}
int pair_ld(const Plan& p, const Geom& g) {
    int nt = 0;
    for (int i = 0; i < p.c.n_layers; ++i) nt = std::max(nt, pair_geom(g, i).ntiles);
    return nt * GEMM_BN;
}
PairGeom quad_geom(const Geom& g, int layer) {
    const int d = 1 << layer;
    const int Lq = (g.L + 4 * d - 1) / (4 * d) * d;
    return {d, Lq, (Lq + 63) / 64};
}
int quad_ld(const Plan& p, const Geom& g) {
    int nt = 0;
    for (int i = 0; i < p.c.n_layers; ++i) nt = std::max(nt, quad_geom(g, i).ntiles);
    return round_up(nt * 64, 128);
}
enum class InForm { Direct, WinogradSeparate, WinogradPaired, WinogradLayer, WinogradLayerF43 };

constexpr long long WINOGRAD_MIN_COLS = 28800;
constexpr long long WINOGRAD_FUSED_MIN_COLS = 28800;
constexpr long long WINOGRAD_F43_MIN_COLS = 28800;

InForm in_form(const Plan& p, const Geom& g, const Tuning& t) {
    auto long_enough = [&](int knob, long long cols) { return (long long)g.L >= (knob >= 0 ? knob : cols); };
    if (t.f32_no_winograd || gemm_split_level(p.c.f32_gemm_mode) != 0 || !long_enough(t.f32_winograd_min, WINOGRAD_MIN_COLS))
        return InForm::Direct;
    if (t.f32_winograd_plain || !gemm_f32_dma_staged(p.nch_rs + p.nch1h)) return InForm::WinogradSeparate;
    if (t.f32_winograd_no_fused || t.f32_no_glds || !wn_winograd_layer_supported(p.C, p.H) ||
        !long_enough(t.f32_winograd_fused_min, WINOGRAD_FUSED_MIN_COLS))
        return InForm::WinogradPaired;
    if (t.f32_winograd_no_f43 || !wn_winograd_layer_f43_supported(p.C, p.H) || !long_enough(t.f32_winograd_f43_min, WINOGRAD_F43_MIN_COLS))
        return InForm::WinogradLayer;
    return InForm::WinogradLayerF43;
}

struct Workspace {
    float *audio, *spect, *spk, *h_tmp, *h_all, *x, *act, *out;
    float* act_all;
    float* a16;
    float* skend;
    float *wgV, *wgT, *wgH;
    int ldp, ldq;
    size_t total;
};

void carve(const Plan& p, const Geom& g, int batch, float* base, InForm in, Workspace& w) {
    size_t o = 0;
    auto take = [&](size_t n) { size_t r = o; o = align_up(o + n); return base ? base + r : nullptr; };
    const size_t B = batch;
    w.audio = take(B * p.c.n_group * g.L);
    w.spect = take(B * p.K0 * g.ld);
    w.spk = take(B * p.c.n_flows * p.S * g.ld);
    w.h_tmp = take(B * p.c.n_flows * p.H * g.ld);
    w.h_all = take(B * p.c.n_flows * p.H * g.ld);
    w.x = take(B * p.C * g.ld);
    w.act = take(B * p.C * g.ld);
    w.out = take(B * p.C * g.ld);
    w.act_all = take((size_t)std::min(p.c.n_layers, (int)Plan::F32_SKIP_GROUP) * B * p.C * g.ld);
    w.a16 = take(B * FOLD_ROWS * g.ld);
    w.skend = take(B * p.c.n_group * g.ld);
    w.wgV = w.wgT = w.wgH = nullptr;
    w.ldp = w.ldq = 0;
    if (in != InForm::Direct) {
        w.ldp = pair_ld(p, g);
        w.ldq = in == InForm::WinogradLayerF43 ? quad_ld(p, g) : 0;
        w.wgV = take(std::max((size_t)4 * w.ldp, (size_t)6 * w.ldq) * B * p.C);
        w.wgT = take((size_t)2 * B * 2 * p.C * w.ldp);
        w.wgH = take(std::max((size_t)2 * w.ldp, (size_t)4 * w.ldq) * B * p.H);
    }
    w.total = o;
}

struct Prof {
    std::mutex mu;
    std::vector<std::pair<hipEvent_t, hipEvent_t>> ev[CTTS_PROF_N];
    std::vector<std::pair<hipEvent_t, hipEvent_t>> pool;
};
thread_local Prof* t_prof = nullptr;

struct ProfScope {
    int which; hipStream_t s; hipEvent_t stop = nullptr; bool active = false;
    ProfScope(int which_, hipStream_t s_) : which(which_), s(s_) {
        Prof* pr = t_prof;
        if (!pr) return;
        std::lock_guard<std::mutex> lk(pr->mu);
        std::pair<hipEvent_t, hipEvent_t> e;
        if (!pr->pool.empty()) { e = pr->pool.back(); pr->pool.pop_back(); }
        else { if (hipEventCreate(&e.first) != hipSuccess || hipEventCreate(&e.second) != hipSuccess) return; }
        (void)hipEventRecord(e.first, s);
        stop = e.second;
        pr->ev[which].push_back(e);
        active = true;
    }
    ~ProfScope() { if (active) (void)hipEventRecord(stop, s); }
};

__global__ __launch_bounds__(256) void speaker_rows_kernel(const float* __restrict__ table, const int64_t* __restrict__ ids,
                                                           float* __restrict__ spk, int k, int n_flows, int S, int sdim,
                                                           int L, int ld, int pad) {
    const int n = blockIdx.x * 256 + threadIdx.x;
    const int e = blockIdx.y, b = blockIdx.z;
    if (n >= ld) return;
    float v = 0.f;
    if (e < sdim && n >= pad && n < pad + L) {
        const long long id = ids[b];
        v = (id >= 0 && id < CTTS_N_SPEAKERS) ? table[(size_t)id * sdim + e] : __builtin_nanf("");
    }
    spk[((size_t)b * n_flows * S + (size_t)k * S + e) * ld + n] = v;
}

size_t fwd_mix_off(const Plan& p, int k) {
    size_t o = 0;
    for (int j = 0; j < k; ++j) o += align_up((size_t)p.fd[j].n_rem * p.fd[j].n_rem);
    return o;
}
int fwd_log_s_rows(const Plan& p, int k) {
    int r = 0;
    for (int j = 0; j < k; ++j) r += p.fd[j].n_half;
    return r;
}

struct FwdSums { double *ls_part, *z_part; int nblk_ls, nblk_z; size_t total; };

void carve_fwd(const Plan& p, const Geom& g, int batch, float* base, InForm in, Workspace& w, FwdSums& f) {
    carve(p, g, batch, base, in, w);
    f.nblk_ls = (g.L + 255) / 256;
    f.nblk_z = (int)(((long long)p.c.n_group * g.L + FWD_SUMSQ_CHUNK - 1) / FWD_SUMSQ_CHUNK);
    size_t o = w.total;
    auto take = [&](size_t doubles) { size_t r = o; o = align_up(o + 2 * doubles); return base ? reinterpret_cast<double*>(base + r) : nullptr; };
    f.ls_part = take((size_t)batch * p.c.n_flows * f.nblk_ls);
    f.z_part = take((size_t)batch * f.nblk_z);
    f.total = o;
}

int workspace_fits(const char* what, size_t have, size_t need) {
    if (need <= have) return CTTS_OK;
    set_error("%s: workspace %zu bytes < required %zu", what, have, need);
    return CTTS_E_WORKSPACE;
}

enum class StackForm { PerLayer, Deferred, Folded };

struct WnCall {
    Plan p; Geom g; Tuning t;
    const float* blob = nullptr;
    int batch = 0, frames = 0;
    hipStream_t s = nullptr;
    Workspace w{};
    FwdSums sums{};
    long long cstride = 0, hstride = 0;
    StackForm stack = StackForm::PerLayer;
    InForm in = InForm::Direct;
    float* audio = nullptr;
    const float* h_all = nullptr;

    int begin(const ctts_waveglow_config* cfg, const void* packed, int batch_, int frames_, void* stream) {
        int rc = make_plan(cfg, p); if (rc) return rc;
        rc = make_geom(p, frames_, g); if (rc) return rc;
        t = tuning();
        blob = static_cast<const float*>(packed); batch = batch_; frames = frames_; s = as_stream(stream);
        cstride = (long long)p.C * g.ld;
        hstride = (long long)p.c.n_flows * p.H * g.ld;
        return CTTS_OK;
    }
    int take_workspace(const char* what, void* workspace, size_t workspace_bytes, bool forward) {
        in = in_form(p, g, t);
        stack = t.f32_no_defer_skip ? StackForm::PerLayer : t.f32_no_wn_fold ? StackForm::Deferred : StackForm::Folded;
        if (forward) carve_fwd(p, g, batch, static_cast<float*>(workspace), in, w, sums);
        else carve(p, g, batch, static_cast<float*>(workspace), in, w);
        audio = w.audio; h_all = w.h_all;
        return workspace_fits(what, workspace_bytes, (forward ? sums.total : w.total) * sizeof(float));
    }

    const float* h(int k) const { return h_all + (size_t)k * p.H * g.ld; }
    size_t act_stride() const { return (size_t)batch * p.C * g.ld; }
    float* act(int i) const { return stack == StackForm::PerLayer ? w.act : w.act_all + (size_t)(i % Plan::F32_SKIP_GROUP) * act_stride(); }
    bool group_ends(int i) const { return i == p.c.n_layers - 1 || (i + 1) % Plan::F32_SKIP_GROUP == 0; }
    bool in_place(int i) const { return in != InForm::WinogradSeparate && (1 << i) % 4 == 0; }
    size_t plane(int rows) const { return (size_t)batch * rows * w.ldp; }

    GemmArgs header() const {
        GemmArgs a{};
        a.gemm_mode = p.c.f32_gemm_mode;
        a.ld = g.ld; a.pad = g.pad; a.L = g.L; a.ntiles = g.ntiles; a.batch = batch;
        a.dst_ld = g.ld; a.dst_pad = g.pad;
        return a;
    }
    GemmArgs in_gemm(int k, int i) const {
        const auto& f = p.fl[k];
        const bool fold0 = stack == StackForm::Folded && i == 0;
        const int dil = 1 << i, nch = fold0 ? 1 : p.nch_rs;
        const float* taps = fold0 ? w.a16 : w.x;
        const long long tstride = fold0 ? (long long)FOLD_ROWS * g.ld : cstride;
        GemmArgs a = header();
        a.A = blob + (fold0 ? f.in0f_A : f.in_A[i]); a.bias = blob + f.in_b[i];
        a.nseg = 4; a.interleave = 3; a.nch_total = fold0 ? p.nch_in0f : p.nch_in; a.MB = p.mb_in;
        for (int tap = 0; tap < 3; ++tap) a.seg[tap] = {taps, tstride, nch, (tap - 1) * dil, 0, 0};
        a.seg[3] = {h(k), hstride, p.nch1h, 0, 0, 0};
        a.dst0 = act(i); a.dst0_bstride = cstride;
        a.M = 2 * p.C; a.pairC = p.C;
        return a;
    }
    GemmArgs behind(size_t A, size_t bias, int rows, const float* acts, int n, int split, bool acc1) const {
        GemmArgs a = header();
        a.A = blob + A; a.bias = blob + bias;
        a.nseg = n; a.nch_total = n * p.nch_rs; a.MB = (rows + GEMM_BM - 1) / GEMM_BM;
        for (int j = 0; j < n; ++j) a.seg[j] = {acts + (size_t)j * act_stride(), cstride, p.nch_rs, 0, 0, 0};
        a.M = rows; a.split = split;
        a.dst0 = w.x; a.dst0_bstride = cstride; a.acc0 = 1;
        a.dst1 = w.out; a.dst1_bstride = cstride; a.acc1 = acc1 ? 1 : 0;
        return a;
    }
    GemmArgs res(int k, int i) const { return behind(p.fl[k].res_A[i], p.fl[k].res_b[i], p.C, act(i), 1, p.C, false); }
    GemmArgs skip_group(int k, int gi) const { return behind(p.fl[k].skip_A[gi], p.fl[k].skip_b[gi], p.C, w.act_all, p.group_layers(gi), 0, gi > 0); }
    GemmArgs res_skip(int k, int i) const {
        return behind(p.fl[k].rs_A[i], p.fl[k].rs_b[i], p.rs_rows(i), act(i), 1, i == p.c.n_layers - 1 ? 0 : p.C, i > 0);
    }
    GemmArgs cond0(const float* spect, const float* spk, float* h_tmp) const {
        GemmArgs a = header();
        a.A = blob + p.cond0_A; a.bias = blob + p.cond0_b;
        a.nseg = 1; a.nch_total = p.nch0; a.MB = p.c.n_flows;
        a.seg[0] = {spect, (long long)p.K0 * g.ld, p.K0 / GEMM_KC, 0, 0, 0};
        if (p.S) {
            a.nseg = 2;
            a.seg[1] = {spk, (long long)p.c.n_flows * p.S * g.ld, p.S / GEMM_KC, 0, p.S, 0};
        }
        a.dst0 = h_tmp; a.dst0_bstride = hstride; a.acc0 = 0;
        a.dst1 = h_tmp; a.dst1_bstride = hstride; a.acc1 = 0;
        a.split = p.c.n_flows * GEMM_BM;
        a.M = p.c.n_flows * GEMM_BM;
        return a;
    }
    GemmArgs cond1(const float* spect, const float* spk, float* h_tmp, float* h_out) const {
        GemmArgs a = cond0(spect, spk, h_tmp);
        a.A = blob + p.cond1_A; a.bias = blob + p.cond1_b;
        a.nseg = 1; a.nch_total = p.nch1h;
        a.seg[0] = {h_tmp, hstride, p.nch1h, 0, GEMM_BM, 0};
        a.dst0 = h_out; a.dst1 = h_out;
        return a;
    }
    GemmArgs wg_header(int i) const {
        const PairGeom pg = pair_geom(g, i);
        GemmArgs a{};
        a.gemm_mode = p.c.f32_gemm_mode;
        a.ld = w.ldp; a.pad = 0; a.L = pg.Lp; a.ntiles = pg.ntiles; a.batch = batch; a.MB = p.mb_in;
        a.M = 2 * p.C;
        if (in == InForm::WinogradPaired) a.parts = 2;
        return a;
    }
    GemmArgs wg_T(int k, int i, int j) const {
        const auto& f = p.fl[k];
        GemmArgs a = wg_header(i);
        a.A = blob + (j == 0 ? f.wg_T2_A[i] : f.wg_T3_A[i]); a.bias = blob + p.zero_b;
        a.nseg = 1; a.nch_total = p.nch_rs;
        a.seg[0] = {w.wgV + (1 + j) * plane(p.C), (long long)p.C * w.ldp, p.nch_rs, 0, 0, 0};
        a.split = 2 * p.C;
        a.dst0 = w.wgT + j * plane(2 * p.C); a.dst0_bstride = (long long)2 * p.C * w.ldp; a.dst_ld = w.ldp; a.dst_pad = 0;
        if (a.parts == 2) {
            a.part_A = (long long)f.wg_T3_A[i] - (long long)f.wg_T2_A[i];
            a.part_seg[0] = (long long)plane(p.C);
            a.part_dst0 = (long long)plane(2 * p.C);
        }
        return a;
    }
    GemmArgs wg_gate(int k, int i, int j) const {
        const auto& f = p.fl[k];
        GemmArgs a = wg_header(i);
        a.A = blob + (j == 0 ? f.wg_e_A[i] : f.wg_o_A[i]); a.bias = blob + f.in_b[i];
        a.nseg = 2; a.nch_total = p.nch_rs + p.nch1h;
        a.seg[0] = {w.wgV + (j == 0 ? 0 : 3) * plane(p.C), (long long)p.C * w.ldp, p.nch_rs, 0, 0, 0};
        if (in_place(i)) {
            a.seg[1] = {h(k), hstride, p.nch1h, 0, 0, 0};
            a.mseg = 2; a.mseg_ld = g.ld; a.mseg_pad = g.pad;
        } else {
            a.seg[1] = {w.wgH + j * plane(p.H), (long long)p.H * w.ldp, p.nch1h, 0, 0, 0};
        }
        a.split = 0; a.pairC = p.C;
        a.dst0 = act(i); a.dst0_bstride = cstride; a.dst_ld = g.ld; a.dst_pad = g.pad;
        a.addend = w.wgT; a.addend2 = w.wgT + plane(2 * p.C); a.addend_bstride = (long long)2 * p.C * w.ldp;
        a.addend2_sign = j == 0 ? 1.0f : -1.0f;
        a.map_d = 1 << i; a.map_L = g.L; a.map_par = j;
        if (a.parts == 2) {
            a.part_A = (long long)f.wg_o_A[i] - (long long)f.wg_e_A[i];
            a.part_seg[0] = (long long)(3 * plane(p.C));
            a.part_seg[1] = in_place(i) ? 0 : (long long)plane(p.H);
        }
        return a;
    }
    WnWinogradLayerArgs wg_layer(int k, int i) const {
        const auto& f = p.fl[k];
        const bool f43 = in == InForm::WinogradLayerF43;
        const PairGeom sg = f43 ? quad_geom(g, i) : pair_geom(g, i);
        const int ldw = f43 ? w.ldq : w.ldp;
        WnWinogradLayerArgs a{};
        if (f43) {
            a.form = WNWG_F43;
            a.A_T2 = blob + f.wq_U_A[0][i]; a.A_T3 = blob + f.wq_U_A[1][i]; a.A_T4 = blob + f.wq_U_A[2][i]; a.A_T5 = blob + f.wq_U_A[3][i];
            a.A_e = blob + f.wq_e_A[i]; a.A_o = blob + f.wq_o_A[i];
        } else {
            a.A_T2 = blob + f.wg_T2_A[i]; a.A_T3 = blob + f.wg_T3_A[i]; a.A_e = blob + f.wg_e_A[i]; a.A_o = blob + f.wg_o_A[i];
        }
        a.bias = blob + f.in_b[i];
        a.V = w.wgV; a.vplane = (long long)batch * p.C * ldw;
        a.Hc = w.wgH; a.hplane = (long long)batch * p.H * ldw;
        a.h2 = h(k); a.h_bstride = hstride;
        a.act = act(i); a.act_bstride = cstride;
        a.C = p.C; a.H = p.H; a.batch = batch;
        a.ldp = ldw; a.Lp = sg.Lp; a.ntiles = sg.ntiles;
        a.d = sg.d; a.L = g.L; a.ld = g.ld; a.pad = g.pad;
        a.in_place = in_place(i);
        return a;
    }

    int gemm(int prof_slot, int epi, const GemmArgs& a) const {
        ProfScope ps(prof_slot, s);
        return launch_gemm_f32(epi, a, s);
    }
    int wg_transform(int k, int i) const {
        if (in == InForm::WinogradLayerF43) {
            const PairGeom qg = quad_geom(g, i);
            const int ncols = t.f32_no_small ? round_up(qg.ntiles * 64, 128) : qg.ntiles * 64;
// ... 29 lines not shown
        const auto& f = p.fl[k];
        const auto& d = p.fd[k];
        return launch_wn_start(a_in, blob + f.start_w, blob + f.start_b, w.x, batch, p.C, p.c.n_group, d.ch_off, d.n_half, g.L, g.ld, g.pad, s);
    }
    int skip_end(int k, int gi, bool tail, float* wave, const CouplingForward* fwd) const {
        const auto& f = p.fl[k];
        const auto& d = p.fd[k];
        ProfScope ps(CTTS_PROF_WN_SKEND, s);
        return launch_skip_end(w.act_all, (long long)act_stride(), p.group_layers(gi),
                               blob + f.skend_W + (size_t)gi * Plan::F32_SKIP_GROUP * p.C * 2 * d.n_half, w.skend, gi == 0, tail,
                               blob + f.skend_b, blob + f.winv, audio, wave, batch, p.C, p.c.n_group, d.ch_off, d.n_half, g.L, g.ld,
                               g.pad, s, tail ? fwd : nullptr);
    }
    int flow_tail(int k, const float* out, float* a_io, float* wave, const CouplingForward* fwd) const {
        const auto& f = p.fl[k];
        const auto& d = p.fd[k];
        return launch_flow_tail(out, a_io, wave, blob + f.end_w, blob + f.end_b, blob + f.winv, batch, p.C, p.c.n_group, d.ch_off,
                                d.n_half, g.L, g.ld, g.pad, s, fwd);
    }

    int flow_folded(int k, float* wave, const CouplingForward* fwd) const {
        const auto& d = p.fd[k];
        int rc = start(k, audio);
        if (rc) return rc;
        if ((rc = launch_wn_start_ones(audio, w.a16, batch, p.c.n_group, d.ch_off, d.n_half, g.L, g.ld, g.pad, s))) return rc;
        for (int i = 0; i < p.c.n_layers; ++i) {
            const bool last = i == p.c.n_layers - 1;
            if ((rc = in_layer(k, i))) return rc;
            if (!last && (rc = gemm(CTTS_PROF_WN_RES_F, GEMM_EPI_SPLIT, res(k, i)))) return rc;
            if (group_ends(i) && (rc = skip_end(k, i / Plan::F32_SKIP_GROUP, last, wave, fwd))) return rc;
        }
        return CTTS_OK;
    }
    int stack_deferred(int k, const float* a_in) const {
        int rc = start(k, a_in);
        if (rc) return rc;
        for (int i = 0; i < p.c.n_layers; ++i) {
            if ((rc = in_layer(k, i))) return rc;
            if (i < p.c.n_layers - 1 && (rc = gemm(CTTS_PROF_WN_RS, GEMM_EPI_SPLIT, res(k, i)))) return rc;
            if (group_ends(i) && (rc = gemm(CTTS_PROF_WN_SKIP, GEMM_EPI_SPLIT, skip_group(k, i / Plan::F32_SKIP_GROUP)))) return rc;
        }
        return CTTS_OK;
    }
    int stack_per_layer(int k, const float* a_in) const {
        int rc = start(k, a_in);
        if (rc) return rc;
        for (int i = 0; i < p.c.n_layers; ++i) {
            if ((rc = in_layer(k, i))) return rc;
            if ((rc = gemm(CTTS_PROF_WN_RS, GEMM_EPI_SPLIT, res_skip(k, i)))) return rc;
        }
        return CTTS_OK;
    }
    int run_flow(int k, float* wave, const CouplingForward* fwd) const {
        if (stack == StackForm::Folded) return flow_folded(k, wave, fwd);
        const int rc = stack == StackForm::Deferred ? stack_deferred(k, audio) : stack_per_layer(k, audio);
        return rc ? rc : flow_tail(k, w.out, audio, wave, fwd);
    }
    int run_flow_forward(const float* fwd_blob, int k, const float* wave, float* log_s_flow, long long ls_bstride) const {
        const auto& d = p.fd[k];
        int rc = launch_flow_head_forward(fwd_blob + fwd_mix_off(p, k), wave, audio, batch, p.c.n_group, d.ch_off, d.n_rem, g.L, s);
        if (rc) return rc;
        const CouplingForward cf{log_s_flow, ls_bstride, sums.ls_part + (size_t)k * sums.nblk_ls, (long long)p.c.n_flows * sums.nblk_ls};
        return run_flow(k, nullptr, &cf);
    }

    int upsample(const float* mel, float* spect) const {
        return launch_upsample_squeeze(mel, blob + p.up_w, p.up_mfma ? blob + p.up_wp : nullptr, blob + p.up_b, spect, batch,
                                       p.c.n_mel_channels, frames, p.c.win_length, p.c.hop_length, p.c.n_group, g.ld, g.pad, s);
    }
    int speaker_rows(const int64_t* ids, float* spk) const {
        if (p.S == 0) return CTTS_OK;
        CTTS_CHECK_ARG(ids != nullptr, "multispeaker model (speaker_embed_dim=%d) needs speaker ids (glow.py:193)", p.c.speaker_embed_dim);
        for (int k = 0; k < p.c.n_flows; ++k)
            hipLaunchKernelGGL(speaker_rows_kernel, dim3((g.ld + 255) / 256, p.S, batch), dim3(256), 0, s, blob + p.fl[k].spk_tab, ids,
                               spk, k, p.c.n_flows, p.S, p.c.speaker_embed_dim, g.L, g.ld, g.pad);
        CTTS_CHECK_LAUNCH("speaker_rows");
        return CTTS_OK;
    }
    int cond(const float* spect, const float* spk, float* h_tmp, float* h_out) const {
        CTTS_CHECK_ARG(p.S == 0 || spk != nullptr, "wn_cond: multispeaker model needs the speaker rows");
        const int rc = launch_gemm_f32(GEMM_EPI_SPLIT, cond0(spect, spk, h_tmp), s);
        return rc ? rc : launch_gemm_f32(GEMM_EPI_SPLIT, cond1(spect, spk, h_tmp, h_out), s);
    }
    int conditioning(const float* mel, const int64_t* ids) const {
        int rc = upsample(mel, w.spect);
        if (rc) return rc;
        if ((rc = speaker_rows(ids, w.spk))) return rc;
        return cond(w.spect, w.spk, w.h_tmp, w.h_all);
    }
};

constexpr int BF_SKIP_GROUP = 4;
struct BfPlan {
    std::vector<std::vector<size_t>> in_A, rs_A;
    std::vector<std::vector<size_t>> skip_A;
    std::vector<size_t> skip_b;
    size_t cond0_A, cond1_A;
    size_t total;
    int nch_in, nch_rs, nch_c0, nch_c1;
    int mb_c, n_groups;
    int P;
    int f16;
    int group_layers(int g, int n_layers) const { return std::min(BF_SKIP_GROUP, n_layers - g * BF_SKIP_GROUP); }
};

void make_bf_plan(const Plan& p, BfPlan& q, int P, int f16 = 0) {
    size_t o = 0;
    auto take = [&](size_t n) { size_t r = o; o = (o + n + 127) / 128 * 128; return r; };
    q.P = P;
    q.f16 = f16;
    q.nch_in = P * (p.c.kernel_size * p.C + p.H) / BGEMM_KC;
    q.nch_rs = P * p.C / BGEMM_KC;
    q.nch_c0 = P * (p.K0 + p.S) / BGEMM_KC;
    q.nch_c1 = P * p.H / BGEMM_KC;
    q.cond0_A = take((size_t)p.c.n_flows * q.nch_c0 * BGEMM_KC * BGEMM_BM);
    q.cond1_A = take((size_t)p.c.n_flows * q.nch_c1 * BGEMM_KC * BGEMM_BM);
    q.mb_c = (p.C + BGEMM_BM - 1) / BGEMM_BM;
    q.n_groups = (p.c.n_layers + BF_SKIP_GROUP - 1) / BF_SKIP_GROUP;
    q.in_A.assign(p.c.n_flows, {});
    q.rs_A.assign(p.c.n_flows, {});
    q.skip_A.assign(p.c.n_flows, {});
    for (int k = 0; k < p.c.n_flows; ++k) {
        for (int i = 0; i < p.c.n_layers; ++i) {
            q.in_A[k].push_back(take((size_t)p.mb_in * q.nch_in * BGEMM_KC * BGEMM_BM));
            q.rs_A[k].push_back(i < p.c.n_layers - 1 ? take((size_t)q.mb_c * q.nch_rs * BGEMM_KC * BGEMM_BM) : 0);
        }
        for (int gi = 0; gi < q.n_groups; ++gi)
            q.skip_A[k].push_back(take((size_t)q.mb_c * q.group_layers(gi, p.c.n_layers) * q.nch_rs * BGEMM_KC * BGEMM_BM));
        q.skip_b.push_back(take((size_t)2 * 2 * q.mb_c * BGEMM_BM));
    }
    q.total = o;
}

struct BfWs {
    float *audio, *spect, *spk;
    bf16_t *spect_bf, *spk_bf, *h_tmp_bf, *h_bf, *x, *act, *out;
    long long spect_lo, spk_lo, h_lo, x_lo, act_lo;
    size_t total_bytes;
};

void carve_bf(const Plan& p, const Geom& g, int batch, char* base, BfWs& w, int P) {
    size_t o = 0;
    auto take = [&](size_t bytes) { size_t r = o; o = (o + bytes + 255) / 256 * 256; return base ? base + r : nullptr; };
    const size_t B = batch;
    const size_t planes = P == 3 ? 2 : 1;
    w.audio = (float*)take(B * p.c.n_group * g.L * 4);
    w.spect = (float*)take(B * p.K0 * g.ld * 4);
    w.spect_bf = (bf16_t*)take(planes * B * p.K0 * g.ld * 2);
    w.spk = (float*)take(B * p.c.n_flows * p.S * g.ld * 4);
    w.spk_bf = (bf16_t*)take(planes * B * p.c.n_flows * p.S * g.ld * 2);
    w.h_tmp_bf = (bf16_t*)take(planes * B * p.c.n_flows * p.H * g.ld * 2);
    w.h_bf = (bf16_t*)take(planes * B * p.c.n_flows * p.H * g.ld * 2);
    w.x = (bf16_t*)take(planes * B * p.C * g.ld * 2);
    w.act = (bf16_t*)take(planes * B * p.C * g.ld * 2 * std::min(p.c.n_layers, BF_SKIP_GROUP));
    w.out = (bf16_t*)take(planes * B * p.C * g.ld * 2);
    const long long on = P == 3 ? 1 : 0;
    w.spect_lo = on * (long long)(B * p.K0 * g.ld);
    w.spk_lo = on * (long long)(B * p.c.n_flows * p.S * g.ld);
    w.h_lo = on * (long long)(B * p.c.n_flows * p.H * g.ld);
    w.x_lo = on * (long long)(B * p.C * g.ld);
    w.act_lo = on * (long long)(B * p.C * g.ld) * std::min(p.c.n_layers, BF_SKIP_GROUP);
    w.total_bytes = o;
}

int push_segs(BGemmArgs& a, int idx, int P, const bf16_t* base, long long lo_off, long long bstride, int nch, int shift,
              int mb_rows) {
    for (int pi = 0; pi < P; ++pi) a.seg[idx++] = {pi == 1 ? base + lo_off : base, bstride, nch, shift, mb_rows};
// ... 281 lines not shown
        return CTTS_OK;
    };
    if ((rc = d2d(f.start_w, w->start_w, (size_t)C * d.n_half))) return rc;
    if ((rc = d2d(f.start_b, w->start_b, C))) return rc;
    if ((rc = d2d(f.end_w, w->end_w, (size_t)2 * d.n_half * C))) return rc;
    if ((rc = d2d(f.end_b, w->end_b, 2 * d.n_half))) return rc;
    if ((rc = d2d(f.winv, w->w_inverse, (size_t)d.n_rem * d.n_rem))) return rc;
    CTTS_CHECK_ARG(w->cond_w[0] && w->cond_w[1] && w->cond_w[2] && w->cond_b[0] && w->cond_b[1] && w->cond_b[2],
                   "pack_flow: NULL cond weights");
    const int sdim = p.c.speaker_embed_dim;
    if ((rc = launch_pack_a(blob + p.cond0_A + (size_t)k * p.nch0 * A_TILE, w->cond_w[0], GEMM_BM, 1, p.nch0, 0, p.K0,
                            GEMM_EPI_SPLIT, C, H, 0, p.K0 + sdim, 1, s))) return rc;
    if (sdim) {
        if ((rc = launch_pack_a(blob + p.cond0_A + (size_t)k * p.nch0 * A_TILE, w->cond_w[0] + p.K0, GEMM_BM, 1, p.nch0,
                                p.K0, sdim, GEMM_EPI_SPLIT, C, H, 0, p.K0 + sdim, 1, s))) return rc;
        if ((rc = d2d(f.spk_tab, w->speaker_embed, (size_t)CTTS_N_SPEAKERS * sdim))) return rc;
    }
    if ((rc = launch_pack_bias(blob + p.cond0_b + (size_t)k * GEMM_BM, GEMM_BM, 1, w->cond_b[0], 0, nullptr, 0,
                               GEMM_EPI_SPLIT, C, H, s))) return rc;
    if ((rc = launch_pack_a(blob + p.cond1_A + (size_t)k * p.nch1h * A_TILE, w->cond_w[1], GEMM_BM, 1, p.nch1h, 0, H,
                            GEMM_EPI_SPLIT, C, H, 0, H, 1, s))) return rc;
    if ((rc = launch_pack_bias(blob + p.cond1_b + (size_t)k * GEMM_BM, GEMM_BM, 1, w->cond_b[1], 0, nullptr, 0,
                               GEMM_EPI_SPLIT, C, H, s))) return rc;
    for (int i = 0; i < p.c.n_layers; ++i) {
        CTTS_CHECK_ARG(w->in_w[i] && w->in_b[i] && w->rs_w[i] && w->rs_b[i], "pack_flow: NULL layer %d weights", i);
        for (int t = 0; t < ks; ++t)
            if ((rc = launch_pack_a(blob + f.in_A[i], w->in_w[i] + t, GEMM_BM, p.mb_in, p.nch_in, 0, C, GEMM_EPI_GATE, C,
                                    2 * C, 0, (long long)C * ks, ks, s, ks, t))) return rc;
        if ((rc = launch_pack_a(blob + f.in_A[i], w->cond_w[2], GEMM_BM, p.mb_in, p.nch_in, ks * C, H, GEMM_EPI_GATE, C,
                                2 * C, (long long)2 * C * i, H, 1, s))) return rc;
        if ((rc = launch_pack_bias(blob + f.in_b[i], GEMM_BM, p.mb_in, w->in_b[i], 0, w->cond_b[2], (long long)2 * C * i,
                                   GEMM_EPI_GATE, C, 2 * C, s))) return rc;
        const int rows = p.rs_rows(i);
        if ((rc = launch_pack_a(blob + f.rs_A[i], w->rs_w[i], GEMM_BM, p.rs_mb(i), p.nch_rs, 0, C, GEMM_EPI_SPLIT, C, rows,
                                0, C, 1, s))) return rc;
        if ((rc = launch_pack_bias(blob + f.rs_b[i], GEMM_BM, p.rs_mb(i), w->rs_b[i], 0, nullptr, 0, GEMM_EPI_SPLIT, C, rows,
                                   s))) return rc;
        const bool last = i == p.c.n_layers - 1;
        const int gi = i / Plan::F32_SKIP_GROUP, gj = i % Plan::F32_SKIP_GROUP;
        if (!last) {
            if ((rc = launch_pack_a(blob + f.res_A[i], w->rs_w[i], GEMM_BM, p.mb_c(), p.nch_rs, 0, C, GEMM_EPI_SPLIT, C, C,
                                    0, C, 1, s))) return rc;
            if ((rc = launch_pack_bias(blob + f.res_b[i], GEMM_BM, p.mb_c(), w->rs_b[i], 0, nullptr, 0, GEMM_EPI_SPLIT, C, C,
                                       s))) return rc;
        }
        if ((rc = launch_pack_a(blob + f.skip_A[gi], w->rs_w[i], GEMM_BM, p.mb_c(), p.group_layers(gi) * p.nch_rs, gj * C, C,
                                GEMM_EPI_SPLIT, C, C, last ? 0 : C, C, 1, s))) return rc;
        hipLaunchKernelGGL(skip_bias_kernel, dim3((p.mb_c() * GEMM_BM + 255) / 256), dim3(256), 0, s, blob + f.skip_b[gi],
                           w->rs_b[i] + (last ? 0 : C), C, p.mb_c() * GEMM_BM, gj == 0 ? 1 : 0);
        CTTS_CHECK_LAUNCH("skip_bias_f32");
    }
    auto pack_gate = [&](size_t A, const float* U, long long u_ld, int u_step, int i) -> int {
        const int nch = p.nch_rs + p.nch1h;
        const int rc = launch_pack_a(blob + A, U, GEMM_BM, p.mb_in, nch, 0, C, GEMM_EPI_GATE, C, 2 * C, 0, u_ld, u_step, s);
        return rc ? rc : launch_pack_a(blob + A, w->cond_w[2], GEMM_BM, p.mb_in, nch, C, H, GEMM_EPI_GATE, C, 2 * C, (long long)2 * C * i, H, 1, s);
    };
    for (int i = 0; i < p.c.n_layers; ++i) {
        float* dense = blob + f.wg_dense;
        const size_t dn = (size_t)2 * C * C;
        if ((rc = launch_winograd_g(w->in_w[i], dense, 2 * C, C, s))) return rc;
        if ((rc = launch_pack_a(blob + f.wg_T2_A[i], dense, GEMM_BM, p.mb_in, p.nch_rs, 0, C, GEMM_EPI_SPLIT, C, 2 * C, 0, C, 1, s))) return rc;
        if ((rc = launch_pack_a(blob + f.wg_T3_A[i], dense + dn, GEMM_BM, p.mb_in, p.nch_rs, 0, C, GEMM_EPI_SPLIT, C, 2 * C, 0, C, 1, s))) return rc;
        if ((rc = pack_gate(f.wg_e_A[i], w->in_w[i], (long long)C * ks, ks, i))) return rc;
        if ((rc = pack_gate(f.wg_o_A[i], dense + 2 * dn, C, 1, i))) return rc;
    }
    for (int i = 0; i < (f.wq_e_A.empty() ? 0 : p.c.n_layers); ++i) {
        float* dense = blob + f.wg_dense;
        const size_t dn = (size_t)2 * C * C;
        if ((rc = launch_winograd_g43(w->in_w[i], dense, 2 * C, C, s))) return rc;
        for (int j = 0; j < 4; ++j)
            if ((rc = launch_pack_a(blob + f.wq_U_A[j][i], dense + (1 + j) * dn, GEMM_BM, p.mb_in, p.nch_rs, 0, C, GEMM_EPI_SPLIT, C, 2 * C, 0, C, 1, s))) return rc;
        if ((rc = pack_gate(f.wq_e_A[i], dense, C, 1, i))) return rc;
        if ((rc = pack_gate(f.wq_o_A[i], dense + 5 * dn, C, 1, i))) return rc;
    }
    if ((rc = launch_fold_in0(w->in_w[0], w->start_w, w->start_b, blob + f.in0f_w, C, d.n_half, ks, s))) return rc;
    for (int t = 0; t < ks; ++t)
        if ((rc = launch_pack_a(blob + f.in0f_A, blob + f.in0f_w + t, GEMM_BM, p.mb_in, p.nch_in0f, 0, FOLD_ROWS, GEMM_EPI_GATE, C,
                                2 * C, 0, (long long)FOLD_ROWS * ks, ks, s, ks, t))) return rc;
    if ((rc = launch_pack_a(blob + f.in0f_A, w->cond_w[2], GEMM_BM, p.mb_in, p.nch_in0f, ks * FOLD_ROWS, H, GEMM_EPI_GATE, C,
                            2 * C, 0, H, 1, s))) return rc;
    return launch_fold_skend(w->rs_w, w->rs_b, w->end_w, w->end_b, blob + f.skend_W, blob + f.skend_b, C, p.c.n_layers, d.n_half, s);
}

size_t ctts_waveglow_workspace_bytes(const ctts_waveglow_config* cfg, int32_t batch, int32_t frames) {
    Plan p; Geom g; Workspace w;
    if (make_plan(cfg, p) || make_geom(p, frames, g) || batch < 1) return 0;
    carve(p, g, batch, nullptr, in_form(p, g, tuning()), w);
    return w.total * sizeof(float);
}

int ctts_upsample_squeeze_f32(const ctts_waveglow_config* cfg, const void* packed, const float* mel, float* spect,
                              int32_t batch, int32_t frames, void* stream) {
    WnCall c;
    const int rc = c.begin(cfg, packed, batch, frames, stream); if (rc) return rc;
    CTTS_CHECK_ARG(packed && mel && spect && batch >= 1, "upsample_squeeze: bad argument");
    return c.upsample(mel, spect);
}

int ctts_wn_cond_f32(const ctts_waveglow_config* cfg, const void* packed, const float* spect, const float* spk_rows,
                     float* h_tmp, float* h_all, int32_t batch, int32_t frames, void* stream) {
    WnCall c;
    const int rc = c.begin(cfg, packed, batch, frames, stream); if (rc) return rc;
    CTTS_CHECK_ARG(packed && spect && h_tmp && h_all && batch >= 1, "wn_cond: bad argument");
    return c.cond(spect, spk_rows, h_tmp, h_all);
}

int ctts_wn_stack_f32(const ctts_waveglow_config* cfg, const void* packed, int32_t flow, const float* audio,
                      const float* h_all, float* x, float* act, float* out, int32_t batch, int32_t frames,
                      void* stream) {
    WnCall c;
    const int rc = c.begin(cfg, packed, batch, frames, stream); if (rc) return rc;
    CTTS_CHECK_ARG(flow >= 0 && flow < c.p.c.n_flows, "wn_stack: flow %d", flow);
    CTTS_CHECK_ARG(packed && audio && h_all && x && act && out && batch >= 1, "wn_stack: bad argument");
    c.w.x = x; c.w.act = act; c.w.out = out; c.h_all = h_all;
    return c.stack_per_layer(flow, audio);
}

int ctts_flow_tail_f32(const ctts_waveglow_config* cfg, const void* packed, int32_t flow, const float* out,
                       float* audio, float* wave, int32_t batch, int32_t frames, void* stream) {
    WnCall c;
    const int rc = c.begin(cfg, packed, batch, frames, stream); if (rc) return rc;
    CTTS_CHECK_ARG(flow >= 0 && flow < c.p.c.n_flows, "flow_tail: flow %d", flow);
    CTTS_CHECK_ARG(packed && out && audio && batch >= 1, "flow_tail: bad argument");
    return c.flow_tail(flow, out, audio, wave, nullptr);
}

int ctts_waveglow_flow_f32(const ctts_waveglow_config* cfg, const void* packed, int32_t flow, float* audio,
                           const float* h_all, float* wave, int32_t batch, int32_t frames, void* workspace,
                           size_t workspace_bytes, void* stream) {
    WnCall c;
    int rc = c.begin(cfg, packed, batch, frames, stream); if (rc) return rc;
    CTTS_CHECK_ARG(flow >= 0 && flow < c.p.c.n_flows, "waveglow_flow: flow %d", flow);
    CTTS_CHECK_ARG(packed && audio && h_all && workspace && batch >= 1, "waveglow_flow: bad argument");
    if ((rc = c.take_workspace("waveglow_flow", workspace, workspace_bytes, false))) return rc;
    c.audio = audio; c.h_all = h_all;
    return c.run_flow(flow, wave, nullptr);
}

size_t ctts_waveglow_forward_packed_bytes(const ctts_waveglow_config* cfg) {
    Plan p;
    if (make_plan(cfg, p)) return 0;
    return fwd_mix_off(p, p.c.n_flows) * sizeof(float);
}

int ctts_waveglow_pack_forward_mix(const ctts_waveglow_config* cfg, int32_t flow, const float* w, void* packed_fwd,
                                   void* stream) {
    Plan p;
    int rc = make_plan(cfg, p); if (rc) return rc;
    CTTS_CHECK_ARG(flow >= 0 && flow < p.c.n_flows, "pack_forward_mix: flow %d", flow);
    CTTS_CHECK_ARG(w && packed_fwd, "pack_forward_mix: NULL pointer");
    const size_t n = (size_t)p.fd[flow].n_rem * p.fd[flow].n_rem;
    CTTS_CHECK_HIP(hipMemcpyAsync(static_cast<float*>(packed_fwd) + fwd_mix_off(p, flow), w, n * sizeof(float),
                                  hipMemcpyDeviceToDevice, as_stream(stream)));
    return CTTS_OK;
}

size_t ctts_waveglow_forward_workspace_bytes(const ctts_waveglow_config* cfg, int32_t batch, int32_t frames) {
    Plan p; Geom g; Workspace w; FwdSums f;
    if (make_plan(cfg, p) || make_geom(p, frames, g)) return 0;
    if (batch < 1) { set_error("forward_workspace_bytes: batch=%d", batch); return 0; }
    carve_fwd(p, g, batch, nullptr, in_form(p, g, tuning()), w, f);
    return f.total * sizeof(float);
}

int ctts_waveglow_flow_forward_f32(const ctts_waveglow_config* cfg, const void* packed, const void* packed_fwd, int32_t flow,
                                   float* z, const float* wave, const float* h_all, float* log_s, double* sum_log_s,
                                   int32_t batch, int32_t frames, void* workspace, size_t workspace_bytes, void* stream) {
    WnCall c;
    int rc = c.begin(cfg, packed, batch, frames, stream); if (rc) return rc;
    CTTS_CHECK_ARG(flow >= 0 && flow < c.p.c.n_flows, "waveglow_flow_forward: flow %d", flow);
    CTTS_CHECK_ARG(packed && packed_fwd && z && h_all && workspace && batch >= 1, "waveglow_flow_forward: bad argument");
    CTTS_CHECK_ARG(wave == nullptr || flow == 0, "waveglow_flow_forward: only flow 0 reads the waveform (flow %d)", flow);
    if ((rc = c.take_workspace("waveglow_flow_forward", workspace, workspace_bytes, true))) return rc;
    c.audio = z; c.h_all = h_all;
    rc = c.run_flow_forward(static_cast<const float*>(packed_fwd), flow, wave, log_s, (long long)c.p.fd[flow].n_half * c.g.L);
    if (rc || !sum_log_s) return rc;
    const FwdSums& f = c.sums;
    return launch_sum_partials(f.ls_part + (size_t)flow * f.nblk_ls, (long long)c.p.c.n_flows * f.nblk_ls, 0, f.nblk_ls, sum_log_s, 1, 1,
                               batch, c.s);
}

int ctts_waveglow_forward_spk_f32(const ctts_waveglow_config* cfg, const void* packed, const void* packed_fwd, const float* mel,
                                  const float* audio, const int64_t* speaker_ids, float* z, float* log_s, double* sums,
                                  int32_t batch, int32_t frames, void* workspace, size_t workspace_bytes, void* stream) {
    WnCall c;
    int rc = c.begin(cfg, packed, batch, frames, stream); if (rc) return rc;
    const Plan& p = c.p;
    CTTS_CHECK_ARG(packed && packed_fwd && mel && audio && z && workspace && batch >= 1, "forward: bad argument");
    CTTS_CHECK_ARG(p.S == 0 || speaker_ids != nullptr, "multispeaker model (speaker_embed_dim=%d) needs speaker ids (glow.py:193)",
                   p.c.speaker_embed_dim);
    if ((rc = c.take_workspace("forward", workspace, workspace_bytes, true))) return rc;
    c.audio = z;
    if ((rc = c.conditioning(mel, speaker_ids))) return rc;
    const int L = c.g.L, S = fwd_log_s_rows(p, p.c.n_flows);
    for (int k = 0; k < p.c.n_flows; ++k) {
        float* ls = log_s ? log_s + (size_t)fwd_log_s_rows(p, k) * L : nullptr;
        rc = c.run_flow_forward(static_cast<const float*>(packed_fwd), k, k == 0 ? audio : nullptr, ls, (long long)S * L);
        if (rc) return rc;
    }
    if (!sums) return CTTS_OK;
    const FwdSums& f = c.sums;
    rc = launch_sum_partials(f.ls_part, (long long)p.c.n_flows * f.nblk_ls, f.nblk_ls, f.nblk_ls, sums, p.c.n_flows + 1, p.c.n_flows,
                             batch, c.s);
    if (rc) return rc;
    rc = launch_sumsq_partials(z, f.z_part, batch, (long long)p.c.n_group * L, f.nblk_z, c.s);
    if (rc) return rc;
    return launch_sum_partials(f.z_part, f.nblk_z, 0, f.nblk_z, sums + p.c.n_flows, p.c.n_flows + 1, 1, batch, c.s);
}

int ctts_waveglow_infer_f32(const ctts_waveglow_config* cfg, const void* packed, const float* mel,
                            const float* z_scaled, float* wave, int32_t batch, int32_t frames, void* workspace,
                            size_t workspace_bytes, void* stream) {
    return ctts_waveglow_infer_spk_f32(cfg, packed, mel, z_scaled, nullptr, wave, batch, frames, workspace,
                                       workspace_bytes, stream);
}

int ctts_waveglow_infer_spk_f32(const ctts_waveglow_config* cfg, const void* packed, const float* mel,
                                const float* z_scaled, const int64_t* speaker_ids, float* wave, int32_t batch,
                                int32_t frames, void* workspace, size_t workspace_bytes, void* stream) {
    WnCall c;
    int rc = c.begin(cfg, packed, batch, frames, stream); if (rc) return rc;
    CTTS_CHECK_ARG(packed && mel && z_scaled && wave && workspace && batch >= 1, "infer: bad argument");
    if ((rc = c.take_workspace("infer", workspace, workspace_bytes, false))) return rc;
    CTTS_CHECK_HIP(hipMemcpyAsync(c.audio, z_scaled, (size_t)batch * c.p.c.n_group * c.g.L * sizeof(float), hipMemcpyDeviceToDevice, c.s));
    if ((rc = c.conditioning(mel, speaker_ids))) return rc;
    for (int k = c.p.c.n_flows - 1; k >= 0; --k)
        if ((rc = c.run_flow(k, k == 0 ? wave : nullptr, nullptr))) return rc;
    return CTTS_OK;
}


int ctts_last_gemm_loop(void) { return last_gemm_loop(); }
int ctts_last_winograd_f43_width(void) { return last_wn_winograd_f43_width(); }
int ctts_tuning_reload(void) { reload_tuning(); return CTTS_OK; }
int ctts_tuning_flags(void) {
    const Tuning t = tuning();
    return (t.f32_no_glds ? 1 : 0) | (t.no_xcd_pair ? 2 : 0) | (t.bf16_no_wide ? 8 : 0) | (t.bf16_no_pp ? 16 : 0) |
           (t.wf_no_fuse ? 128 : 0) | (t.taco_no_fuse ? 256 : 0) | (t.f32_no_small ? 512 : 0) | (t.f32_force_small ? 1024 : 0) |
           (t.f32_no_splitk ? 2048 : 0) | (t.wf_no_vec_interp ? 4096 : 0) | (t.f32_no_defer_skip ? 8192 : 0) |
           (t.wf_no_region_split ? 16384 : 0) | (t.wf_no_row_queue ? 32768 : 0) | (t.wf_row_queue_min >= 0 ? 65536 : 0) |
           (t.wf_inject_abort ? 131072 : 0) | (t.wf_queue_debug ? 262144 : 0) | (t.f32_no_round_split ? 524288 : 0) |
           (t.bf16_ps ? (1 << 20) : 0) | (t.bf16_no_ps ? (1 << 21) : 0) | (t.taco_poll_delay_set ? (1 << 23) : 0) |
           (t.taco_valu ? (1 << 24) : 0) | (t.up_no_mfma ? (1 << 25) : 0) | (t.f32_no_wn_fold ? (1 << 26) : 0) |
           (t.taco_bg_no_pipe ? (1 << 27) : 0) | (t.f32_no_winograd ? (1 << 28) : 0) | (t.f32_winograd_min >= 0 ? (1 << 29) : 0) |
           (t.f32_winograd_plain ? (1 << 30) : 0) | (t.f32_winograd_fused_min >= 0 ? 4 : 0) | (t.f32_winograd_no_fused ? 32 : 0) |
           (t.f32_winograd_f43_min >= 0 ? (1 << 6) : 0) | (t.f32_winograd_no_f43 ? (1 << 22) : 0) |
           (t.wf_fwd_rowwise ? (int)(1u << 31) : 0);
}

int ctts_profile_create(void** handle) {
    CTTS_CHECK_ARG(handle, "profile_create: NULL");
    *handle = new Prof();
    return CTTS_OK;
}

int ctts_profile_bind(void* handle) {
    t_prof = static_cast<Prof*>(handle);
    return CTTS_OK;
}

int ctts_profile_collect(void* handle, int32_t which, int64_t* launches, double* total_ms) {
    Prof* pr = static_cast<Prof*>(handle);
    CTTS_CHECK_ARG(pr && which >= 0 && which < CTTS_PROF_N && launches && total_ms, "profile_collect: bad argument");
    std::lock_guard<std::mutex> lk(pr->mu);
    double tot = 0.0;
    int64_t n = 0;
    for (auto& e : pr->ev[which]) {
        float ms = 0.f;
        CTTS_CHECK_HIP(hipEventSynchronize(e.second));
        CTTS_CHECK_HIP(hipEventElapsedTime(&ms, e.first, e.second));
        tot += ms; ++n;
        pr->pool.push_back(e);
    }
    pr->ev[which].clear();
    *launches = n; *total_ms = tot;
    return CTTS_OK;
}

int ctts_profile_destroy(void* handle) {
    Prof* pr = static_cast<Prof*>(handle);
    if (!pr) return CTTS_OK;
    if (t_prof == pr) t_prof = nullptr;
    {
        std::lock_guard<std::mutex> lk(pr->mu);
        for (int w = 0; w < CTTS_PROF_N; ++w)
            for (auto& e : pr->ev[w]) { (void)hipEventDestroy(e.first); (void)hipEventDestroy(e.second); }
        for (auto& e : pr->pool) { (void)hipEventDestroy(e.first); (void)hipEventDestroy(e.second); }
    }
    delete pr;
    return CTTS_OK;
}

static size_t packed_bf16_bytes_impl(const ctts_waveglow_config* cfg, int P) {
    Plan p; BfPlan q;
    if (make_plan(cfg, p)) return 0;
    if (p.C % BGEMM_KC != 0 || p.H % BGEMM_KC != 0) { set_error("bf16: channels must be multiples of 32"); return 0; }
    make_bf_plan(p, q, P);
    return q.total * sizeof(bf16_t);
}

static int pack_flow_bf16_impl(const ctts_waveglow_config* cfg, int32_t k, const ctts_waveglow_flow_weights* w,
                               void* packed_bf16, void* stream, int P, int f16 = 0) {
    Plan p; BfPlan q;
    int rc = make_plan(cfg, p); if (rc) return rc;
// ... 176 lines not shown
```

cookietts_amd/waveglow.py:

```python
from __future__ import annotations

import ctypes as C
import math

import torch
import torch.nn as nn

from . import _cache, _lib
from ._wn import WNConv, folded_weight

__all__ = ["WaveGlow", "WaveGlowLoss", "Invertible1x1Conv", "WN"]


class _Conv1dParams(nn.Module):

    def __init__(self, in_ch, out_ch, k, bias=True):
        super().__init__()
        self.weight = nn.Parameter(torch.empty(out_ch, in_ch, k))
        nn.init.kaiming_uniform_(self.weight, a=math.sqrt(5))
        if bias:
            bound = 1.0 / math.sqrt(in_ch * k)
            self.bias = nn.Parameter(torch.empty(out_ch).uniform_(-bound, bound))
        else:
            self.register_parameter("bias", None)


class WaveGlowLoss(nn.Module):

    def __init__(self, sigma=1.0):
        super().__init__()
        self.sigma = sigma
        self.sigma2 = sigma * sigma
        self.sigma2_2 = 2 * sigma * sigma

    def forward(self, model_output):
        z, log_s_list, log_det_W_list = model_output
        log_s_total = sum(torch.sum(log_s) for log_s in log_s_list)
        log_det_W_total = sum(log_det_W_list)
        loss = torch.sum(z * z) / self.sigma2_2 - log_s_total - log_det_W_total
        return loss / (z.size(0) * z.size(1) * z.size(2))


class Invertible1x1Conv(nn.Module):

    def __init__(self, c):
        super().__init__()
        self.conv = _Conv1dParams(c, c, 1, bias=False)
        W = torch.linalg.qr(torch.randn(c, c))[0]
        if torch.det(W) < 0:
            W[:, 0] = -1 * W[:, 0]
        self.conv.weight.data = W.view(c, c, 1).contiguous()


class WN(nn.Module):

    def __init__(self, n_in_channels, n_mel_channels, n_layers, n_channels, kernel_size,
                 speaker_embed_dim, rezero):
        super().__init__()
        assert kernel_size % 2 == 1
        assert n_channels % 2 == 0
        self.n_layers = n_layers
        self.n_channels = n_channels
        self.speaker_embed_dim = speaker_embed_dim
        if rezero:
            self.alpha_i = nn.ParameterList([nn.Parameter(torch.rand(1) * 0.02 + 0.09) for _ in range(n_layers)])
        if speaker_embed_dim:
            self.speaker_embed = nn.Embedding(_lib.N_SPEAKERS, speaker_embed_dim)
            self.speaker_embed.weight.data.mul_(0.05)
        hidden = 256
        self.start = WNConv((n_channels, n_in_channels, 1))
        self.end = _Conv1dParams(n_channels, 2 * n_in_channels, 1)
        self.end.weight.data.zero_()
        self.end.bias.data.zero_()
        self.cond_layers = nn.ModuleList([
            WNConv((hidden, n_mel_channels + speaker_embed_dim, 1)),
            WNConv((hidden, hidden, 1)),
            WNConv((2 * n_channels * n_layers, hidden, 1))])
        self.in_layers = nn.ModuleList()
        self.res_skip_layers = nn.ModuleList()
        for i in range(n_layers):
            self.in_layers.append(WNConv((2 * n_channels, n_channels, kernel_size)))
            rs = 2 * n_channels if i < n_layers - 1 else n_channels
            self.res_skip_layers.append(WNConv((rs, n_channels, 1)))


_MODES = {
    "f32": (None, None, "ctts_waveglow_workspace_bytes", "ctts_waveglow_infer_spk_f32"),
    "bf16": ("ctts_waveglow_packed_bf16_bytes", "ctts_waveglow_pack_flow_bf16", "ctts_waveglow_workspace_bf16_bytes",
             "ctts_waveglow_infer_spk_bf16"),
    "bf16x3": ("ctts_waveglow_packed_bf16x3_bytes", "ctts_waveglow_pack_flow_bf16x3", "ctts_waveglow_workspace_bf16x3_bytes",
               "ctts_waveglow_infer_spk_bf16x3"),
    "f16": ("ctts_waveglow_packed_bf16_bytes", "ctts_waveglow_pack_flow_f16", "ctts_waveglow_workspace_bf16_bytes",
            "ctts_waveglow_infer_spk_f16"),
}


class WaveGlow(_cache.PackedModule):
    GPU_ONLY = "WaveGlow HIP path needs the model on a GPU (no CPU fallback)"

    def __init__(self, yoyo, yoyo_WN, n_mel_channels, n_flows, n_group, n_early_every, n_early_size,
                 memory_efficient, spect_scaling, upsample_mode, WN_config, win_length, hop_length):
        super().__init__()
        if upsample_mode not in ('normal', 'simple', 'simple_half'):
            raise ValueError(f"upsample_mode = {upsample_mode} invalid")
        if memory_efficient:
            raise NotImplementedError("memory_efficient builds no layers in the reference (glow.py:263)")
        assert n_group % 2 == 0
        assert hop_length % n_group == 0 and win_length % hop_length == 0

        def need(cond, what):
            if not cond:
                raise NotImplementedError(f"cookietts_amd.WaveGlow (glow.py topology): {what} is not built on the HIP path")
        wn = WN_config
        need(n_group in (4, 8, 12, 16), f"n_group={n_group} (4, 8, 12 or 16: the un-squeeze writes whole float4s, the flow-boundary "
             "kernels hold <= 8 half-channels)")
        need((hop_length // n_group) % 4 == 0, f"hop_length / n_group = {hop_length // n_group} (a multiple of 4: latent rows of any "
             "number of frames are then whole float4s)")
        need(wn['kernel_size'] == 3, f"WN kernel_size={wn['kernel_size']} (3: the dilated in-layers are three K segments of one GEMM)")
        need(wn['n_channels'] >= 128 and wn['n_channels'] % 128 == 0, f"WN n_channels={wn['n_channels']} (a multiple of 128: the GEMM's m-block)")
        need(1 <= wn['n_layers'] <= 12, f"WN n_layers={wn['n_layers']} (1..12: dilation 2^11 is the largest halo)")
        need((n_mel_channels * n_group) % 16 == 0, f"n_mel_channels * n_group = {n_mel_channels * n_group} (a multiple of 16: one K chunk)")
        need(not wn['speaker_embed_dim'] or (n_mel_channels * n_group) % 32 == 0,
             "a speaker embedding with n_mel_channels * n_group not a multiple of 32")
        self.spect_scaling = spect_scaling
        self.multispeaker = WN_config['speaker_embed_dim'] > 0
        self.n_mel_channels = n_mel_channels
        self.n_flows = n_flows
        self.n_group = n_group
        self.n_early_every = n_early_every
        self.n_early_size = n_early_size
        self.win_length = win_length
        self.hop_length = hop_length
        self.WN_config = dict(WN_config)

        self.upsample_mode = upsample_mode
        self.upsample_groups = {'normal': 1, 'simple': n_mel_channels, 'simple_half': n_mel_channels // 2}[upsample_mode]
        assert n_mel_channels % self.upsample_groups == 0
        self.upsample = nn.Module()
        opg = n_mel_channels // self.upsample_groups
        w = torch.empty(n_mel_channels, opg, win_length)
        nn.init.kaiming_uniform_(w, a=math.sqrt(5))
        bound = 1.0 / math.sqrt(opg * win_length)
        self.upsample.weight = nn.Parameter(w)
        self.upsample.bias = nn.Parameter(torch.empty(n_mel_channels).uniform_(-bound, bound))

        self.WN = nn.ModuleList()
        self.convinv = nn.ModuleList()
        n_half = n_group // 2
        n_remaining_channels = n_group
        for k in range(n_flows):
            if k % n_early_every == 0 and k > 0:
                n_half = n_half - n_early_size // 2
                n_remaining_channels = n_remaining_channels - n_early_size
            self.convinv.append(Invertible1x1Conv(n_remaining_channels))
            self.WN.append(WN(n_half, n_mel_channels * n_group, **WN_config))
        self.n_remaining_channels = n_remaining_channels

        self._compute_dtype = torch.float32
        self._f32_gemm_mode = None
        self._fwd = None

    def c_config(self):
        wn = self.WN_config
        return _lib.WaveGlowConfig(
            n_mel_channels=self.n_mel_channels, n_group=self.n_group, n_flows=self.n_flows,
            n_early_every=self.n_early_every, n_early_size=self.n_early_size,
            win_length=self.win_length, hop_length=self.hop_length, n_layers=wn['n_layers'],
            n_channels=wn['n_channels'], kernel_size=wn['kernel_size'], cond_hidden=256,
            speaker_embed_dim=wn.get('speaker_embed_dim', 0), f32_gemm_mode=_lib.model_gemm_mode(self._f32_gemm_mode))

    def set_f32_gemm_mode(self, mode):
        _lib.model_gemm_mode(mode)
        self._f32_gemm_mode = mode
        return self

    def _invalidate(self):
        super()._invalidate()
        self._fwd = None
        for m in self.convinv:
            if hasattr(m, 'W_inverse'):
                del m.W_inverse

    def set_compute_dtype(self, dtype):
        if dtype not in (torch.float32, torch.bfloat16, torch.float16, "bf16x3"):
            raise NotImplementedError(f"compute dtype {dtype} is not built (float32, bfloat16, float16 or 'bf16x3')")
        if dtype != torch.float32 and self.n_group > 8:
            raise NotImplementedError(f"reduced-precision compute with n_group={self.n_group}: the bf16 / f16 flow-boundary kernels hold "
                                      "<= 8 channels (fp32 takes 16)")
        self._compute_dtype = dtype
        self._invalidate()
        return self

    def _mode(self):
        if self._compute_dtype == "bf16x3":
            return "bf16x3"
        if self._compute_dtype == torch.float16:
            return "f16"
        return "bf16" if (self._compute_dtype == torch.bfloat16 or next(self.parameters()).dtype == torch.bfloat16) else "f32"

    @staticmethod
    def remove_weightnorm(model):
        for wn in model.WN:
            wn.start.remove_weight_norm()
            for layer in list(wn.in_layers) + list(wn.cond_layers) + list(wn.res_skip_layers):
                layer.remove_weight_norm()
        model._invalidate()
        return model

    @staticmethod
    def _scaled(t, alpha, stream, keep):
        a = alpha.detach().float().contiguous()
        y = torch.empty_like(t)
        rows, cols = (t.shape[0], t[0].numel()) if t.dim() > 1 else (1, t.numel())
        _lib.check(_lib.lib().ctts_scale_add_rows_f32(_lib.ptr(t), _lib.ptr(a), None, _lib.ptr(y), 1, rows, cols, cols, 0,
                                                      stream), "ctts_scale_add_rows_f32")
        keep += [a, y, t]
        return y

    def _ensure_packed(self, device):
        return self.packed(device, lambda: self._pack(device))

    def _pack(self, device):
        bytes16, pack16, _, _ = _MODES[self._mode()]
        lib = _lib.lib()
        for p in self.parameters():
            if p.device != device:
                raise RuntimeError(f"parameter on {p.device}, input on {device}: move the model first")
        cfg = self.c_config()
        nbytes = _lib.nbytes(lib.ctts_waveglow_packed_bytes, C.byref(cfg), what="unsupported WaveGlow config")
        with torch.cuda.device(device):
            stream = _lib.stream(device)
            blob = torch.zeros(nbytes // 4, dtype=torch.float32, device=device)
            bblob = None
            if bytes16:
                nb = _lib.nbytes(getattr(lib, bytes16), C.byref(cfg), what="unsupported bf16 WaveGlow config")
                bblob = torch.zeros(nb // 2, dtype=torch.int16, device=device)
            keep = []
            up_w = self.upsample.weight.detach().float().contiguous()
            if self.upsample_groups > 1:
                n_mel, opg = self.n_mel_channels, self.n_mel_channels // self.upsample_groups
                ipg = n_mel // self.upsample_groups
                dense = torch.zeros(n_mel, n_mel, self.win_length, dtype=torch.float32, device=device)
                for gi in range(self.upsample_groups):
                    dense[gi * ipg:(gi + 1) * ipg, gi * opg:(gi + 1) * opg] = up_w[gi * ipg:(gi + 1) * ipg]
                up_w = dense
            up_b = self.upsample.bias.detach().float().contiguous()
            keep += [up_w, up_b]
            _lib.check(lib.ctts_waveglow_pack_upsample(C.byref(cfg), _lib.ptr(up_w), _lib.ptr(up_b),
                                                      _lib.ptr(blob), stream), "ctts_waveglow_pack_upsample")
            n_layers = self.WN_config['n_layers']
            for k in range(self.n_flows):
                wn = self.WN[k]
                fw = _lib.WaveGlowFlowWeights()
                fw.start_w = folded_weight(wn.start, stream, keep).data_ptr()
                fw.start_b = _cache.dev(wn.start.bias, keep)
                for j in range(3):
                    fw.cond_w[j] = folded_weight(wn.cond_layers[j], stream, keep).data_ptr()
                    fw.cond_b[j] = _cache.dev(wn.cond_layers[j].bias, keep)
                arrs = {}
                for name, layers in (("in", wn.in_layers), ("rs", wn.res_skip_layers)):
                    wa = (C.c_void_p * n_layers)()
                    ba = (C.c_void_p * n_layers)()
                    for i in range(n_layers):
                        wt = folded_weight(layers[i], stream, keep)
                        bt = layers[i].bias.detach().float().contiguous()
                        if name == "rs" and hasattr(wn, 'alpha_i'):
                            wt, bt = self._scaled(wt, wn.alpha_i[i], stream, keep), self._scaled(bt, wn.alpha_i[i], stream, keep)
                        keep.append(bt)
                        wa[i], ba[i] = wt.data_ptr(), bt.data_ptr()
                    arrs[name] = (wa, ba)
                fw.in_w, fw.in_b = arrs["in"]
                fw.rs_w, fw.rs_b = arrs["rs"]
                fw.end_w = _cache.dev(wn.end.weight, keep)
                fw.end_b = _cache.dev(wn.end.bias, keep)
                W = self.convinv[k].conv.weight.detach().squeeze(-1)
                W_inverse = W.float().cpu().inverse().to(device).contiguous()
                self.convinv[k].W_inverse = W_inverse[..., None]
                keep.append(W_inverse)
                fw.w_inverse = W_inverse.data_ptr()
                if wn.speaker_embed_dim:
                    fw.speaker_embed = _cache.dev(wn.speaker_embed.weight, keep)
                _lib.check(lib.ctts_waveglow_pack_flow(C.byref(cfg), k, C.byref(fw), _lib.ptr(blob), stream),
                           f"ctts_waveglow_pack_flow({k})")
                if bblob is not None:
                    _lib.check(getattr(lib, pack16)(C.byref(cfg), k, C.byref(fw), _lib.ptr(bblob), stream), f"{pack16}({k})")
            torch.cuda.current_stream(device).synchronize()
        return blob, bblob

    def steps_for(self, frames):
        return frames * self.hop_length // self.n_group

    def _speaker_ids(self, speaker_id, device, B):
        if not self.multispeaker:
            return None
        if speaker_id is None:
            raise RuntimeError("this WaveGlow is multispeaker (speaker_embed_dim > 0): pass speaker_id")
        if not speaker_id.is_cuda and speaker_id.numel() and \
                (int(speaker_id.min()) < 0 or int(speaker_id.max()) >= _lib.N_SPEAKERS):
            raise IndexError("speaker id out of range of the embedding table")
        ids = speaker_id.detach().to(device=device, dtype=torch.int64).reshape(-1).contiguous()
        assert ids.shape[0] == B, (tuple(ids.shape), B)
        return ids

    def infer_from_noise(self, spect, z_scaled, speaker_id=None):
        if self.spect_scaling:
            raise NotImplementedError("spect_scaling=True is broken in the reference (glow.py:233-235)")
        if spect.dim() == 2:
            spect = spect.unsqueeze(0)
        device = spect.device
        blob, bblob = self._ensure_packed(device)
        lib = _lib.lib()
        B, M, F = spect.shape
        assert M == self.n_mel_channels, (M, self.n_mel_channels)
        L = self.steps_for(F)
        assert tuple(z_scaled.shape) == (B, self.n_group, L), (tuple(z_scaled.shape), (B, self.n_group, L))
        mel = spect.detach().float().contiguous()
        z = z_scaled.detach().to(device=device, dtype=torch.float32).contiguous()
        ids = self._speaker_ids(speaker_id, device, B)
        mode = self._mode()
        _, _, ws_bytes, infer = _MODES[mode]
        cfg = self.c_config()
        nbytes = _lib.nbytes(getattr(lib, ws_bytes), C.byref(cfg), B, F, what="workspace query failed")
        ws = self.workspace((device, B, F, mode, nbytes), lambda: nbytes)
        wave = torch.empty(B, L * self.n_group, dtype=torch.float32, device=device)
        blobs = (blob,) if bblob is None else (blob, bblob)
        with torch.cuda.device(device):
            _lib.check(getattr(lib, infer)(C.byref(cfg), *map(_lib.ptr, blobs), _lib.ptr(mel), _lib.ptr(z), _lib.ptr(ids),
                                           _lib.ptr(wave), B, F, _lib.ptr(ws), ws.numel() * 4, _lib.stream(device)), infer)
        return wave.to(spect.dtype)

    def infer(self, spect, speaker_id=None, sigma=1.0):
        if spect.dim() == 2:
            spect = spect.unsqueeze(0)
        B, _, F = spect.shape
        z = torch.randn(B, self.n_group, self.steps_for(F), device=spect.device, dtype=torch.float32)
        return self.infer_from_noise(spect, z * sigma, speaker_id=speaker_id)

    def _ensure_forward_packed(self, device):
        blob, _ = self._ensure_packed(device)
        if self._fwd is None or self._fwd[0] is not blob:
            lib = _lib.lib()
            cfg = self.c_config()
            nbytes = _lib.nbytes(lib.ctts_waveglow_forward_packed_bytes, C.byref(cfg), what="unsupported WaveGlow config")
            with torch.cuda.device(device):
                stream = _lib.stream(device)
                fwd = torch.zeros(nbytes // 4, dtype=torch.float32, device=device)
                keep, logdets = [], []
                for k in range(self.n_flows):
                    W = self.convinv[k].conv.weight.detach().squeeze(-1).float()
                    logdets.append(torch.logdet(W.cpu()))
                    Wd = W.to(device).contiguous()
                    keep.append(Wd)
                    _lib.check(lib.ctts_waveglow_pack_forward_mix(C.byref(cfg), k, _lib.ptr(Wd), _lib.ptr(fwd), stream),
                               f"ctts_waveglow_pack_forward_mix({k})")
                torch.cuda.current_stream(device).synchronize()
            self._fwd = (blob, fwd, torch.stack(logdets))
        return self._fwd

    def _forward_refusals(self, spect, audio):
        if audio is None:
            raise ValueError("WaveGlow.forward needs the audio [B, frames * hop_length] (glow.py:267); audio is None")
        if self.spect_scaling:
            raise NotImplementedError("spect_scaling=True is broken in the reference (glow.py:233-235)")
        if self.training and torch.is_grad_enabled():
            raise NotImplementedError("no backward pass: WaveGlow.forward on the HIP path is the analysis pass only - call "
                                      "model.eval() or run it under torch.no_grad()")
        mode = self._mode()
        if mode != "f32":
            raise NotImplementedError(f"WaveGlow.forward with compute mode {mode!r}: the 16-bit flow boundaries have no forward "
                                      "form (fp32 compute only; set_f32_gemm_mode's bf16x3 / bf16x6 are fp32 tensors and do run)")
        F = spect.shape[-1]
        if audio.dim() != 2 or audio.shape[1] != F * self.hop_length:
            raise ValueError(f"audio of shape {tuple(audio.shape)} for {F} frames: forward needs exactly frames * hop_length = "
                             f"{F * self.hop_length} samples per item (a shorter audio moves the WN's zero padding, so its "
                             "result is not a crop of the full-length one)")

    def _forward_core(self, spect, audio, speaker_id, want_log_s):
        if spect.dim() == 2:
            spect = spect.unsqueeze(0)
        self._forward_refusals(spect, audio)
        device = spect.device
        blob, fwd, logdets = self._ensure_forward_packed(device)
        lib = _lib.lib()
        B, M, F = spect.shape
        assert M == self.n_mel_channels, (M, self.n_mel_channels)
        assert audio.shape[0] == B, (tuple(audio.shape), B)
        L = self.steps_for(F)
        mel = spect.detach().float().contiguous()
        wave = audio.detach().to(device=device, dtype=torch.float32).contiguous()
        ids = self._speaker_ids(speaker_id, device, B)
        cfg = self.c_config()
        nbytes = _lib.nbytes(lib.ctts_waveglow_forward_workspace_bytes, C.byref(cfg), B, F, what="workspace query failed")
        ws = self.workspace((device, B, F, "forward", nbytes), lambda: nbytes)
        S = sum(c.conv.weight.shape[0] // 2 for c in self.convinv)
        z = torch.empty(B, self.n_group, L, dtype=torch.float32, device=device)
        log_s = torch.empty(B, S, L, dtype=torch.float32, device=device) if want_log_s else None
        sums = torch.empty(B, self.n_flows + 1, dtype=torch.float64, device=device)
        with torch.cuda.device(device):
            _lib.check(lib.ctts_waveglow_forward_spk_f32(C.byref(cfg), _lib.ptr(blob), _lib.ptr(fwd), _lib.ptr(mel), _lib.ptr(wave),
                                                         _lib.ptr(ids), _lib.ptr(z), _lib.ptr(log_s), _lib.ptr(sums), B, F,
                                                         _lib.ptr(ws), ws.numel() * 4, _lib.stream(device)),
                       "ctts_waveglow_forward_spk_f32")
        return z, log_s, sums, logdets

    def forward(self, spect, audio=None, speaker_id=None):
        z, log_s, _, logdets = self._forward_core(spect, audio, speaker_id, want_log_s=True)
        dt = spect.dtype
        log_s = log_s.to(dt)
        out, off = [], 0
        for c in self.convinv:
            nh = c.conv.weight.shape[0] // 2
# ... 14 lines not shown
```

include/cookietts_hip.h:

```cpp
#ifndef COOKIETTS_HIP_H
#define COOKIETTS_HIP_H

#include <stddef.h>
#include <stdint.h>

#ifdef __cplusplus
extern "C" {
#endif

#define CTTS_OK 0
#define CTTS_E_ARG (-1)
#define CTTS_E_LAUNCH (-2)
#define CTTS_E_WORKSPACE (-3)
#define CTTS_E_ABORT (-4)

#define CTTS_ABI_VERSION 7

#define CTTS_GEMM_DEFAULT 0
#define CTTS_GEMM_F32 1
#define CTTS_GEMM_BF16X3 2
#define CTTS_GEMM_BF16X6 3
#define CTTS_N_SPEAKERS 512

int ctts_abi_version(void);
const char* ctts_last_error(void);

typedef struct ctts_waveglow_config {
    int32_t n_mel_channels;
    int32_t n_group;
    int32_t n_flows;
    int32_t n_early_every;
    int32_t n_early_size;
    int32_t win_length;
    int32_t hop_length;
    int32_t n_layers;
    int32_t n_channels;
    int32_t kernel_size;
    int32_t cond_hidden;
    int32_t speaker_embed_dim;
    int32_t f32_gemm_mode;
} ctts_waveglow_config;

typedef struct ctts_waveglow_geometry {
    int32_t steps;
    int32_t ld;
    int32_t pad;
    int32_t n_remaining;
} ctts_waveglow_geometry;

int ctts_waveglow_geometry_for(const ctts_waveglow_config* cfg, int32_t frames,
                               ctts_waveglow_geometry* out);


int ctts_fold_weightnorm_f32(const float* v, const float* g, float* w, int32_t out_ch,
                             int32_t fan, void* stream);

typedef struct ctts_waveglow_flow_weights {
    const float* start_w;
    const float* start_b;
    const float* cond_w[3];
    const float* cond_b[3];
    const float* const* in_w;
    const float* const* in_b;
    const float* const* rs_w;
    const float* const* rs_b;
    const float* end_w;
    const float* end_b;
    const float* w_inverse;
    const float* speaker_embed;
} ctts_waveglow_flow_weights;

size_t ctts_waveglow_packed_bytes(const ctts_waveglow_config* cfg);
int ctts_waveglow_pack_upsample(const ctts_waveglow_config* cfg, const float* up_w,
                                const float* up_b, void* packed, void* stream);
int ctts_waveglow_pack_flow(const ctts_waveglow_config* cfg, int32_t flow,
                            const ctts_waveglow_flow_weights* w, void* packed, void* stream);


size_t ctts_waveglow_workspace_bytes(const ctts_waveglow_config* cfg, int32_t batch,
                                     int32_t frames);

int ctts_waveglow_infer_f32(const ctts_waveglow_config* cfg, const void* packed,
                            const float* mel, const float* z_scaled, float* wave,
                            int32_t batch, int32_t frames, void* workspace,
                            size_t workspace_bytes, void* stream);
int ctts_waveglow_infer_spk_f32(const ctts_waveglow_config* cfg, const void* packed, const float* mel,
                                const float* z_scaled, const int64_t* speaker_ids, float* wave, int32_t batch,
                                int32_t frames, void* workspace, size_t workspace_bytes, void* stream);

size_t ctts_waveglow_packed_bf16_bytes(const ctts_waveglow_config* cfg);
int ctts_waveglow_pack_flow_bf16(const ctts_waveglow_config* cfg, int32_t flow,
                                 const ctts_waveglow_flow_weights* w, void* packed_bf16, void* stream);
size_t ctts_waveglow_workspace_bf16_bytes(const ctts_waveglow_config* cfg, int32_t batch,
                                          int32_t frames);
int ctts_waveglow_infer_bf16(const ctts_waveglow_config* cfg, const void* packed,
                             const void* packed_bf16, const float* mel, const float* z_scaled,
                             float* wave, int32_t batch, int32_t frames, void* workspace,
                             size_t workspace_bytes, void* stream);
int ctts_waveglow_infer_spk_bf16(const ctts_waveglow_config* cfg, const void* packed, const void* packed_bf16,
                                 const float* mel, const float* z_scaled, const int64_t* speaker_ids, float* wave,
                                 int32_t batch, int32_t frames, void* workspace, size_t workspace_bytes,
                                 void* stream);

int ctts_waveglow_pack_flow_f16(const ctts_waveglow_config* cfg, int32_t flow,
                                const ctts_waveglow_flow_weights* w, void* packed_f16, void* stream);
int ctts_waveglow_infer_spk_f16(const ctts_waveglow_config* cfg, const void* packed, const void* packed_f16,
                                const float* mel, const float* z_scaled, const int64_t* speaker_ids, float* wave,
                                int32_t batch, int32_t frames, void* workspace, size_t workspace_bytes,
                                void* stream);

size_t ctts_waveglow_packed_bf16x3_bytes(const ctts_waveglow_config* cfg);
int ctts_waveglow_pack_flow_bf16x3(const ctts_waveglow_config* cfg, int32_t flow,
                                   const ctts_waveglow_flow_weights* w, void* packed_bf16x3, void* stream);
size_t ctts_waveglow_workspace_bf16x3_bytes(const ctts_waveglow_config* cfg, int32_t batch,
                                            int32_t frames);
int ctts_waveglow_infer_spk_bf16x3(const ctts_waveglow_config* cfg, const void* packed, const void* packed_bf16x3,
                                   const float* mel, const float* z_scaled, const int64_t* speaker_ids, float* wave,
                                   int32_t batch, int32_t frames, void* workspace, size_t workspace_bytes,
                                   void* stream);


int ctts_upsample_squeeze_f32(const ctts_waveglow_config* cfg, const void* packed,
                              const float* mel, float* spect, int32_t batch, int32_t frames,
                              void* stream);
int ctts_wn_cond_f32(const ctts_waveglow_config* cfg, const void* packed, const float* spect,
                     const float* spk_rows, float* h_tmp, float* h_all, int32_t batch, int32_t frames,
                     void* stream);
int ctts_wn_stack_f32(const ctts_waveglow_config* cfg, const void* packed, int32_t flow,
                      const float* audio, const float* h_all, float* x, float* act, float* out,
                      int32_t batch, int32_t frames, void* stream);
int ctts_flow_tail_f32(const ctts_waveglow_config* cfg, const void* packed, int32_t flow,
                       const float* out, float* audio, float* wave, int32_t batch,
                       int32_t frames, void* stream);

int ctts_waveglow_flow_f32(const ctts_waveglow_config* cfg, const void* packed, int32_t flow, float* audio,
                           const float* h_all, float* wave, int32_t batch, int32_t frames, void* workspace,
                           size_t workspace_bytes, void* stream);

size_t ctts_waveglow_forward_packed_bytes(const ctts_waveglow_config* cfg);
int ctts_waveglow_pack_forward_mix(const ctts_waveglow_config* cfg, int32_t flow, const float* w, void* packed_fwd,
                                   void* stream);
size_t ctts_waveglow_forward_workspace_bytes(const ctts_waveglow_config* cfg, int32_t batch, int32_t frames);
int ctts_waveglow_forward_spk_f32(const ctts_waveglow_config* cfg, const void* packed, const void* packed_fwd, const float* mel,
                                  const float* audio, const int64_t* speaker_ids, float* z, float* log_s, double* sums,
                                  int32_t batch, int32_t frames, void* workspace, size_t workspace_bytes, void* stream);
int ctts_waveglow_flow_forward_f32(const ctts_waveglow_config* cfg, const void* packed, const void* packed_fwd, int32_t flow,
                                   float* z, const float* wave, const float* h_all, float* log_s, double* sum_log_s,
                                   int32_t batch, int32_t frames, void* workspace, size_t workspace_bytes, void* stream);


#define CTTS_MIX_PERMUTE 0
#define CTTS_MIX_CONV1X1 1
#define CTTS_GATE_GTU 0
#define CTTS_GATE_GTRU 1
#define CTTS_GATE_GTLRU 2
#define CTTS_GATE_GLU 3
#define CTTS_GATE_TTU 4
#define CTTS_GATE_STU 5
#define CTTS_GATE_GTSU 6
#define CTTS_GATE_SPTU 7
#define CTTS_GATE_GSIU 8
#define CTTS_GATE_GSIRU 9
#define CTTS_GATE_GTSRU 10
#define CTTS_GATE_GSIRRU 11
#define CTTS_GATE_GSIRLRU 12
#define CTTS_GATE_GSIRRLRU 13
typedef struct ctts_waveflow_config {
    int32_t n_mel_channels;
    int32_t n_flows;
    int32_t n_group;
    int32_t n_layers;
    int32_t n_channels;
    int32_t kernel_size_w;
    int32_t kernel_size_h;
    int32_t dilation_h;
    int32_t seperable_conv;
    int32_t cond_precomputed;
    int32_t gated_unit;
    int32_t merge_res_skip;
    int32_t n_early_every;
    int32_t n_early_size;
    int32_t mixing;
    int32_t mix_first;
    int32_t dilation_w[12];
    int32_t dilation_h_l[12];
    int32_t f32_gemm_mode;
} ctts_waveflow_config;

typedef struct ctts_waveflow_flow_weights {
    const float* start_w;
    const float* start_b;
    const float* cond_w;
    const float* cond_b;
    const float* const* in_w;
    const float* const* in_b;
    const float* const* rs_w;
    const float* const* rs_b;
    const float* end_w;
    const float* end_b;
    const float* const* dw_w;
    const float* const* dw_b;
    const float* w_inverse;
} ctts_waveflow_flow_weights;

size_t ctts_waveflow_packed_bytes(const ctts_waveflow_config* cfg);
int ctts_waveflow_pack_flow(const ctts_waveflow_config* cfg, int32_t flow,
                            const ctts_waveflow_flow_weights* w, void* packed, void* stream);
size_t ctts_waveflow_workspace_bytes(const ctts_waveflow_config* cfg, int32_t batch,
                                     int32_t samples);
int ctts_waveflow_inverse_f32(const ctts_waveflow_config* cfg, const void* packed, const float* z,
                              const float* mel, float* audio, int32_t batch, int32_t samples,
                              int32_t frames, void* workspace, size_t workspace_bytes,
                              void* stream);
// ... 450 lines not shown
```

Before: 3.956 million samples/s.

## Compose upsample and conditioning convs into one per-phase GEMM from mel

Adds an option that folds the transposed-conv upsampler and the two linear conditioning layers of every flow into one weight matrix per output phase. This is precomputed in double precision at pack time, and a single GEMM then runs directly on padded mel frames. A new phase-store epilogue writes the interleaved per-sample conditioning rows, so the spect and h_tmp intermediates and their GEMMs are skipped. The path is enabled by default for single-speaker fp32 when a FLOP heuristic favours it. It adds packing cost, blob size and a different rounding order.

```diff
diff --git a/cookietts_amd/_lib.py b/cookietts_amd/_lib.py
--- a/cookietts_amd/_lib.py
+++ b/cookietts_amd/_lib.py
@@ -176,6 +176,14 @@
     "ctts_waveglow_infer_bf16": (C.c_int, [_CFG, _FP, _FP, _FP, _FP, _FP, C.c_int32, C.c_int32, _FP, C.c_size_t, _FP]),
     "ctts_upsample_squeeze_f32": (C.c_int, [_CFG, _FP, _FP, _FP, C.c_int32, C.c_int32, _FP]),
     "ctts_wn_cond_f32": (C.c_int, [_CFG, _FP, _FP, _FP, _FP, _FP, C.c_int32, C.c_int32, _FP]),
+    "ctts_waveglow_has_composed_cond": (C.c_int, [_CFG]),
+    "ctts_waveglow_packed_bytes_opt": (C.c_size_t, [_CFG, C.c_int32]),
+    "ctts_waveglow_pack_cond_composed": (C.c_int, [_CFG, C.c_int32, C.POINTER(WaveGlowFlowWeights), _FP, _FP]),
+    "ctts_waveglow_workspace_bytes_opt": (C.c_size_t, [_CFG, C.c_int32, C.c_int32, C.c_int32]),
+    "ctts_waveglow_infer_spk_f32_opt": (C.c_int, [_CFG, _FP, _FP, _FP, _FP, _FP, C.c_int32, C.c_int32, _FP, C.c_size_t, C.c_int32,
+                                                 _FP]),
+    "ctts_wn_cond_composed_scratch_bytes": (C.c_size_t, [_CFG, C.c_int32, C.c_int32]),
+    "ctts_wn_cond_composed_f32": (C.c_int, [_CFG, _FP, _FP, _FP, _FP, C.c_int32, C.c_int32, _FP]),
     "ctts_wn_stack_f32": (C.c_int, [_CFG, _FP, C.c_int32, _FP, _FP, _FP, _FP, _FP, C.c_int32, C.c_int32, _FP]),
     "ctts_flow_tail_f32": (C.c_int, [_CFG, _FP, C.c_int32, _FP, _FP, _FP, C.c_int32, C.c_int32, _FP]),
     "ctts_waveglow_flow_f32": (C.c_int, [_CFG, _FP, C.c_int32, _FP, _FP, _FP, C.c_int32, C.c_int32, _FP, C.c_size_t, _FP]),
@@ -357,6 +365,7 @@
 
 MODEL_GEMM_MODES = {None: 0, "default": 0, "f32": 1, "bf16x3": 2, "bf16x6": 3}
 GEMM_MODES = {"f32": 1, "bf16x3": 2, "bf16x6": 3}
+WG_OPT_COMPOSED_COND = 1
 
 
 def model_gemm_mode(mode):
diff --git a/cookietts_amd/csrc/gemm_f32.h b/cookietts_amd/csrc/gemm_f32.h
--- a/cookietts_amd/csrc/gemm_f32.h
+++ b/cookietts_amd/csrc/gemm_f32.h
@@ -20,6 +20,7 @@
     GEMM_EPI_TANH = 5,
     GEMM_EPI_GATEX = 7,
     GEMM_EPI_GATE_RS = 6,
+    GEMM_EPI_PHASE = 8,
 };
 
 __host__ __device__ inline bool gemm_epi_is_pair(int epi) {
@@ -113,6 +114,7 @@
     long long part_A, part_seg[4], part_dst0;
     int mseg, mseg_ld, mseg_pad;
     int mseg_ch0, mseg_ch1;
+    int phase;
 };
 
 __host__ __device__ inline int gemm_dense_row(int epi, int bm, int mb, int r, int C, int M) {
diff --git a/cookietts_amd/csrc/gemm_f32.hip b/cookietts_amd/csrc/gemm_f32.hip
--- a/cookietts_amd/csrc/gemm_f32.hip
+++ b/cookietts_amd/csrc/gemm_f32.hip
@@ -80,6 +80,31 @@
             }
         }
     }
+}
+
+__device__ __forceinline__ void phase_epilogue(const GemmArgs& a, f32x16 (&acc)[4][2], const float* bias, int mb, int rloc0, int b,
+                                               int ncol0, int l31, int lhi) {
+    const int P = a.phase;
+    float* dst = a.dst0 + (size_t)b * a.dst0_bstride + ((size_t)(mb / P) * 256 + (size_t)(mb % P) * (256 / P)) * a.dst_ld + a.dst_pad;
+#pragma unroll
+    for (int mt = 0; mt < 4; ++mt)
+#pragma unroll
+        for (int nt = 0; nt < 2; ++nt) {
+            const int n = ncol0 + nt * 32 + l31;
+            if (n < a.L) {
+#pragma unroll
+                for (int rg = 0; rg < 4; ++rg) {
+                    const int rt = mt * 32 + 8 * rg + 4 * lhi;
+                    const int R = rloc0 + rt;
+                    float4 v;
+                    v.x = acc[mt][nt][4 * rg + 0] + bias[rt + 0];
+                    v.y = acc[mt][nt][4 * rg + 1] + bias[rt + 1];
+                    v.z = acc[mt][nt][4 * rg + 2] + bias[rt + 2];
+                    v.w = acc[mt][nt][4 * rg + 3] + bias[rt + 3];
+                    *reinterpret_cast<float4*>(dst + (size_t)(R / P) * a.dst_ld + (size_t)P * n + R % P) = v;
+                }
+            }
+        }
 }
 
 typedef __bf16 bf16x8_t __attribute__((ext_vector_type(8)));
@@ -133,7 +158,13 @@
 
     int id = blockIdx.x;
     int mb, tile, b;
-    if (a.map_mode == 1) {
+    if constexpr (EPI == GEMM_EPI_PHASE) {
+        const int nt_ = a.ntiles * a.batch;
+        mb = id / nt_;
+        id -= mb * nt_;
+        tile = id % a.ntiles;
+        b = id / a.ntiles;
+    } else if (a.map_mode == 1) {
         const int x = id & 7, j = id >> 3;
         mb = 2 * (x & 1) + (j & 1);
         const int gt = (j >> 1) * 4 + (x >> 1);
@@ -639,6 +670,9 @@
                     acc[mt][nt] = __builtin_amdgcn_mfma_f32_32x32x2f32(a2[mt], actv[s >> 4][nt][r], acc[mt][nt], 0, 0, 0);
         }
         split_epilogue<GEMM_EPI_SPLIT>(a, acc, lds + 64 * 128, a.rs_rows, 0, b, n0 + wn * 64, l31, lhi);
+    } else if constexpr (EPI == GEMM_EPI_PHASE) {
+        static_assert(EPI != GEMM_EPI_PHASE || (WM == 2 && SEGS == 4 && XS == 0 && !EXT), "phase store: the 256-row fp32 shape, <= 4 segments");
+        phase_epilogue(a, acc, bias, mb, wm * 128, b, n0 + wn * 64, l31, lhi);
     } else {
         split_epilogue<EPI>(a, acc, bias, a.M, mb * BM + wm * 128, b, n0 + wn * 64, l31, lhi, EXT ? (long long)part * a.part_dst0 : 0);
     }
@@ -743,6 +777,7 @@
     g_tune.f32_winograd_no_fused = on("CTTS_F32_WINOGRAD_NO_FUSED");
     g_tune.f32_winograd_f43_min = num("CTTS_F32_WINOGRAD_F43_MIN", -1);
     g_tune.f32_winograd_no_f43 = on("CTTS_F32_WINOGRAD_NO_F43");
+    g_tune.f32_cond_chain = on("CTTS_F32_COND_CHAIN");
     g_tune_loaded = true;
 }
 }
@@ -806,6 +841,16 @@
                        "gemm: a two-part SPLIT launch stores every row to dst0");
         CTTS_CHECK_ARG(parts == 1 || (long long)parts * a.ntiles * a.batch < (1ll << 31) / a.MB, "gemm: merged grid");
     }
+    if (epi == GEMM_EPI_PHASE) {
+        CTTS_CHECK_ARG(a.bm == 256 && a.nseg <= 4 && a.interleave <= 1 && gemm_split_level(a.gemm_mode) == 0 && parts == 1 && !a.mseg &&
+                           a.shape_blocks == 0,
+                       "gemm: the phase store needs the fp32 launch of the 256-row shape with <= 4 segments (nseg=%d)", a.nseg);
+        CTTS_CHECK_ARG(a.phase >= 4 && a.phase <= 256 && (a.phase & (a.phase - 1)) == 0 && a.MB % a.phase == 0 && a.M == a.MB * a.bm,
+                       "gemm: phase=%d MB=%d M=%d", a.phase, a.MB, a.M);
+        CTTS_CHECK_ARG(a.dst_pad >= 0 && a.dst_pad % 4 == 0 && a.dst_ld % 4 == 0 && a.dst0_bstride % 4 == 0 &&
+                           reinterpret_cast<uintptr_t>(a.dst0) % 16 == 0 && (long long)a.phase * a.L <= a.dst_ld - a.dst_pad,
+                       "gemm: phase store dst_ld=%d dst_pad=%d phase=%d L=%d", a.dst_ld, a.dst_pad, a.phase, a.L);
+    }
     if (a.mseg) {
         const GemmSeg& g = a.seg[1];
         CTTS_CHECK_ARG(epi == GEMM_EPI_GATE && a.nseg == 2 && a.map_d > 0 && a.map_d % 4 == 0 && a.map_col0 % 4 == 0 && a.mseg_pad >= 0 &&
@@ -843,6 +888,18 @@
     a.mseg_ch0 = a.mseg_ch1 = 0;
     if (a.mseg) { a.mseg_ch0 = a.seg[0].nch; a.mseg_ch1 = a.seg[0].nch + a.seg[1].nch; }
     CTTS_CHECK_ARG(!a.mseg || gemm_f32_dma_staged(a.nch_total), "gemm: the mapped segment needs the DMA-staged kernels");
+    if (epi == GEMM_EPI_PHASE) {
+        const bool glds = gemm_f32_dma_staged(a.nch_total);
+        const long long blocks = (long long)a.MB * a.ntiles * a.batch;
+        CTTS_CHECK_ARG(blocks > 0 && blocks < (1ll << 31), "gemm: grid %lld", blocks);
+        a.gt_limit = a.ntiles * a.batch;
+        a.map_mode = 0;
+        note_gemm_loop(0);
+        if (glds) hipLaunchKernelGGL((conv_gemm_f32_kernel<GEMM_EPI_PHASE, 2, 4, true>), dim3((unsigned)blocks), dim3(256), 0, stream, a);
+        else hipLaunchKernelGGL((conv_gemm_f32_kernel<GEMM_EPI_PHASE, 2, 4, false>), dim3((unsigned)blocks), dim3(256), 0, stream, a);
+        CTTS_CHECK_LAUNCH("conv_gemm_f32");
+        return CTTS_OK;
+    }
     if (parts > 1 && (gemm_f32_small_applies(epi, a) || !gemm_f32_dma_staged(a.nch_total))) {
         for (int p = 0; p < parts; ++p)
             if (int rc = launch_gemm_f32(epi, gemm_part_args(a, p), stream)) return rc;
diff --git a/cookietts_amd/csrc/tuning.h b/cookietts_amd/csrc/tuning.h
--- a/cookietts_amd/csrc/tuning.h
+++ b/cookietts_amd/csrc/tuning.h
@@ -30,6 +30,7 @@
     int f32_winograd_f43_min;
     bool f32_winograd_no_f43;
     bool f32_winograd_no_fused;
+    bool f32_cond_chain;
     bool wf_no_region_split;
     bool wf_no_row_queue;
     int wf_row_queue_min;
diff --git a/cookietts_amd/csrc/waveglow_api.hip b/cookietts_amd/csrc/waveglow_api.hip
--- a/cookietts_amd/csrc/waveglow_api.hip
+++ b/cookietts_amd/csrc/waveglow_api.hip
@@ -37,6 +37,9 @@
     size_t up_w, up_wp, up_b, cond0_A, cond0_b, cond1_A, cond1_b;
     size_t zero_b;
     bool up_mfma;
+    bool cc;
+    int ccP, ccJ, nch_cc;
+    size_t cc_A, cc_b, cc_w10;
     struct Flow {
         size_t start_w, start_b, end_w, end_b, winv, spk_tab;
         std::vector<size_t> in_A, in_b, rs_A, rs_b;
@@ -57,9 +60,11 @@
     int rs_mb(int layer) const { return (rs_rows(layer) + GEMM_BM - 1) / GEMM_BM; }
 };
 
-int make_plan(const ctts_waveglow_config* cfg, Plan& p) {
+int make_plan(const ctts_waveglow_config* cfg, Plan& p, int options = 0) {
     CTTS_CHECK_ARG(cfg != nullptr, "config is NULL");
     p.c = *cfg;
+    CTTS_CHECK_ARG((options & ~CTTS_WG_OPT_COMPOSED_COND) == 0, "options=%d (CTTS_WG_OPT_*)", options);
+    const bool want_cc = (options & CTTS_WG_OPT_COMPOSED_COND) != 0;
     const auto& c = p.c;
     CTTS_CHECK_ARG(c.n_flows >= 1 && c.n_layers >= 1 && c.n_layers <= 12, "n_flows=%d n_layers=%d", c.n_flows, c.n_layers);
     CTTS_CHECK_ARG(gemm_mode_valid(c.f32_gemm_mode), "f32_gemm_mode=%d (CTTS_GEMM_DEFAULT / _F32 / _BF16X3 / _BF16X6)", c.f32_gemm_mode);
@@ -141,6 +146,17 @@
         }
         f.wg_dense = take((size_t)(f43 ? 6 : 3) * 2 * p.C * p.C);
     }
+    p.ccP = c.hop_length / c.n_group;
+    p.ccJ = c.win_length / c.hop_length;
+    p.nch_cc = p.ccJ * c.n_mel_channels / GEMM_KC;
+    p.cc = want_cc && p.S == 0 && c.n_mel_channels % GEMM_KC == 0 && p.ccJ >= 1 && p.ccJ <= 4 && p.ccP >= 4 && p.ccP <= GEMM_BM &&
+           (p.ccP & (p.ccP - 1)) == 0;
+    p.cc_A = p.cc_b = p.cc_w10 = 0;
+    if (p.cc) {
+        p.cc_A = take((size_t)c.n_flows * p.ccP * p.nch_cc * A_TILE);
+        p.cc_b = take((size_t)c.n_flows * p.ccP * GEMM_BM);
+        p.cc_w10 = take((size_t)c.n_flows * 2 * p.H * p.K0);
+    }
     p.total = o;
     return CTTS_OK;
 }
@@ -198,8 +214,20 @@
     return InForm::WinogradLayerF43;
 }
 
+bool cond_composed(const Plan& p, int frames, const Tuning& t) {
+    if (!p.cc || t.f32_cond_chain || gemm_split_level(p.c.f32_gemm_mode) != 0) return false;
+    const long long tiles_f = (frames + GEMM_BN - 1) / GEMM_BN, tiles_l = ((long long)frames * p.ccP + GEMM_BN - 1) / GEMM_BN;
+    return tiles_f * p.ccP * p.ccJ * p.c.n_mel_channels < tiles_l * (p.K0 + p.H);
+}
+struct MelGeom { int ntiles, pad, ld; };
+MelGeom mel_geom(int frames) {
+    const int nt = (frames + GEMM_BN - 1) / GEMM_BN;
+    return {nt, 4, nt * GEMM_BN + 8};
+}
+
 struct Workspace {
     float *audio, *spect, *spk, *h_tmp, *h_all, *x, *act, *out;
+    float* melp;
     float* act_all;
     float* a16;
     float* skend;
@@ -208,14 +236,15 @@
     size_t total;
 };
 
-void carve(const Plan& p, const Geom& g, int batch, float* base, InForm in, Workspace& w) {
+void carve(const Plan& p, const Geom& g, int batch, float* base, InForm in, bool composed, Workspace& w) {
     size_t o = 0;
     auto take = [&](size_t n) { size_t r = o; o = align_up(o + n); return base ? base + r : nullptr; };
     const size_t B = batch;
     w.audio = take(B * p.c.n_group * g.L);
-    w.spect = take(B * p.K0 * g.ld);
+    w.spect = composed ? nullptr : take(B * p.K0 * g.ld);
+    w.melp = composed ? take(B * p.c.n_mel_channels * mel_geom(g.L / p.ccP).ld) : nullptr;
     w.spk = take(B * p.c.n_flows * p.S * g.ld);
-    w.h_tmp = take(B * p.c.n_flows * p.H * g.ld);
+    w.h_tmp = composed ? nullptr : take(B * p.c.n_flows * p.H * g.ld);
     w.h_all = take(B * p.c.n_flows * p.H * g.ld);
     w.x = take(B * p.C * g.ld);
     w.act = take(B * p.C * g.ld);
@@ -273,6 +302,54 @@
     spk[((size_t)b * n_flows * S + (size_t)k * S + e) * ld + n] = v;
 }
 
+
+__global__ __launch_bounds__(256) void cond_compose_w10_kernel(const float* __restrict__ w1, const float* __restrict__ w0,
+                                                               double* __restrict__ w10, int H, int K0) {
+    const int c = blockIdx.x * 256 + threadIdx.x, r = blockIdx.y;
+    if (c >= K0) return;
+    double s = 0.0;
+    for (int h = 0; h < H; ++h) s += (double)w1[(size_t)r * H + h] * (double)w0[(size_t)h * K0 + c];
+    w10[(size_t)r * K0 + c] = s;
+}
+
+__global__ __launch_bounds__(GEMM_BM) void cond_compose_A_kernel(const double* __restrict__ w10, const float* __restrict__ up_w,
+                                                                 float* __restrict__ A, int n_mel, int G, int hop, int win, int P,
+                                                                 int nch) {
+    const int rl = threadIdx.x, kidx = blockIdx.x, m = blockIdx.y;
+    const int r = m * (GEMM_BM / P) + rl / P, p = rl % P;
+    const int j = kidx / n_mel, ci = kidx % n_mel;
+    const float* u = up_w + (size_t)ci * n_mel * win + hop * j + G * p;
+    const double* wr = w10 + (size_t)r * n_mel * G;
+    double s = 0.0;
+    for (int co = 0; co < n_mel; ++co)
+        for (int q = 0; q < G; ++q) s += wr[co * G + q] * (double)u[(size_t)co * win + q];
+    A[(((size_t)m * nch + kidx / GEMM_KC) * GEMM_KC + kidx % GEMM_KC) * GEMM_BM + rl] = (float)s;
+}
+
+__global__ __launch_bounds__(GEMM_BM) void cond_compose_bias_kernel(const float* __restrict__ w0, const float* __restrict__ b0,
+                                                                    const float* __restrict__ w1, const float* __restrict__ b1,
+                                                                    const float* __restrict__ up_b, float* __restrict__ bias, int K0,
+                                                                    int G, int P) {
+    __shared__ double t0[GEMM_BM];
+    const int r = threadIdx.x;
+    double s = b0[r];
+    for (int c = 0; c < K0; ++c) s += (double)w0[(size_t)r * K0 + c] * (double)up_b[c / G];
+    t0[r] = s;
+    __syncthreads();
+    s = b1[r];
+    for (int h = 0; h < GEMM_BM; ++h) s += (double)w1[(size_t)r * GEMM_BM + h] * t0[h];
+    const int HR = GEMM_BM / P;
+    for (int p = 0; p < P; ++p) bias[(size_t)(r / HR) * GEMM_BM + (r % HR) * P + p] = (float)s;
+}
+
+__global__ __launch_bounds__(256) void mel_pad_kernel(const float* __restrict__ mel, float* __restrict__ melp, int frames, int ld, int pad) {
+    const int n = blockIdx.x * 256 + threadIdx.x;
+    const size_t row = (size_t)blockIdx.z * gridDim.y + blockIdx.y;
+    if (n >= ld) return;
+    const int f = n - pad;
+    melp[row * ld + n] = f >= 0 && f < frames ? mel[row * frames + f] : 0.0f;
+}
+
 size_t fwd_mix_off(const Plan& p, int k) {
     size_t o = 0;
     for (int j = 0; j < k; ++j) o += align_up((size_t)p.fd[j].n_rem * p.fd[j].n_rem);
@@ -286,8 +363,8 @@
 
 struct FwdSums { double *ls_part, *z_part; int nblk_ls, nblk_z; size_t total; };
 
-void carve_fwd(const Plan& p, const Geom& g, int batch, float* base, InForm in, Workspace& w, FwdSums& f) {
-    carve(p, g, batch, base, in, w);
+void carve_fwd(const Plan& p, const Geom& g, int batch, float* base, InForm in, bool composed, Workspace& w, FwdSums& f) {
+    carve(p, g, batch, base, in, composed, w);
     f.nblk_ls = (g.L + 255) / 256;
     f.nblk_z = (int)(((long long)p.c.n_group * g.L + FWD_SUMSQ_CHUNK - 1) / FWD_SUMSQ_CHUNK);
     size_t o = w.total;
@@ -315,11 +392,12 @@
     long long cstride = 0, hstride = 0;
     StackForm stack = StackForm::PerLayer;
     InForm in = InForm::Direct;
+    bool composed = false;
     float* audio = nullptr;
     const float* h_all = nullptr;
 
-    int begin(const ctts_waveglow_config* cfg, const void* packed, int batch_, int frames_, void* stream) {
-        int rc = make_plan(cfg, p); if (rc) return rc;
+    int begin(const ctts_waveglow_config* cfg, const void* packed, int batch_, int frames_, void* stream, int options = 0) {
+        int rc = make_plan(cfg, p, options); if (rc) return rc;
         rc = make_geom(p, frames_, g); if (rc) return rc;
         t = tuning();
         blob = static_cast<const float*>(packed); batch = batch_; frames = frames_; s = as_stream(stream);
@@ -330,8 +408,9 @@
     int take_workspace(const char* what, void* workspace, size_t workspace_bytes, bool forward) {
         in = in_form(p, g, t);
         stack = t.f32_no_defer_skip ? StackForm::PerLayer : t.f32_no_wn_fold ? StackForm::Deferred : StackForm::Folded;
-        if (forward) carve_fwd(p, g, batch, static_cast<float*>(workspace), in, w, sums);
-        else carve(p, g, batch, static_cast<float*>(workspace), in, w);
+        composed = cond_composed(p, frames, t);
+        if (forward) carve_fwd(p, g, batch, static_cast<float*>(workspace), in, composed, w, sums);
+        else carve(p, g, batch, static_cast<float*>(workspace), in, composed, w);
         audio = w.audio; h_all = w.h_all;
         return workspace_fits(what, workspace_bytes, (forward ? sums.total : w.total) * sizeof(float));
     }
@@ -401,6 +480,20 @@
         a.nseg = 1; a.nch_total = p.nch1h;
         a.seg[0] = {h_tmp, hstride, p.nch1h, 0, GEMM_BM, 0};
         a.dst0 = h_out; a.dst1 = h_out;
+        return a;
+    }
+    GemmArgs cond_composed_gemm(const float* melp, float* h_out) const {
+        const MelGeom mg = mel_geom(frames);
+        GemmArgs a{};
+        a.gemm_mode = p.c.f32_gemm_mode;
+        a.ld = mg.ld; a.pad = mg.pad; a.L = frames; a.ntiles = mg.ntiles; a.batch = batch;
+        a.A = blob + p.cc_A; a.bias = blob + p.cc_b;
+        a.nseg = p.ccJ; a.nch_total = p.nch_cc; a.MB = p.c.n_flows * p.ccP;
+        for (int j = 0; j < p.ccJ; ++j)
+            a.seg[j] = {melp, (long long)p.c.n_mel_channels * mg.ld, p.c.n_mel_channels / GEMM_KC, -j, 0, 0};
+        a.M = a.MB * GEMM_BM; a.split = a.M;
+        a.phase = p.ccP;
+        a.dst0 = h_out; a.dst0_bstride = hstride; a.dst_ld = g.ld; a.dst_pad = g.pad;
         return a;
     }
     GemmArgs wg_header(int i) const {
@@ -596,7 +689,15 @@
         const int rc = launch_gemm_f32(GEMM_EPI_SPLIT, cond0(spect, spk, h_tmp), s);
         return rc ? rc : launch_gemm_f32(GEMM_EPI_SPLIT, cond1(spect, spk, h_tmp, h_out), s);
     }
+    int cond_from_mel(const float* mel, float* melp, float* h_out) const {
+        CTTS_CHECK_ARG(p.cc, "wn_cond_composed: the packed model holds no composed conditioning matrix");
+        const MelGeom mg = mel_geom(frames);
+        hipLaunchKernelGGL(mel_pad_kernel, dim3((mg.ld + 255) / 256, p.c.n_mel_channels, batch), dim3(256), 0, s, mel, melp, frames, mg.ld, mg.pad);
+        CTTS_CHECK_LAUNCH("mel_pad");
+        return launch_gemm_f32(GEMM_EPI_PHASE, cond_composed_gemm(melp, h_out), s);
+    }
     int conditioning(const float* mel, const int64_t* ids) const {
+        if (composed) return cond_from_mel(mel, w.melp, w.h_all);
         int rc = upsample(mel, w.spect);
         if (rc) return rc;
         if ((rc = speaker_rows(ids, w.spk))) return rc;
@@ -1044,10 +1145,47 @@
     return launch_fold_skend(w->rs_w, w->rs_b, w->end_w, w->end_b, blob + f.skend_W, blob + f.skend_b, C, p.c.n_layers, d.n_half, s);
 }
 
+size_t ctts_waveglow_packed_bytes_opt(const ctts_waveglow_config* cfg, int32_t options) {
+    Plan p;
+    if (make_plan(cfg, p, options)) return 0;
+    return p.total * sizeof(float);
+}
+
+int ctts_waveglow_has_composed_cond(const ctts_waveglow_config* cfg) {
+    Plan p;
+    return make_plan(cfg, p, CTTS_WG_OPT_COMPOSED_COND) == CTTS_OK && p.cc ? 1 : 0;
+}
+
+int ctts_waveglow_pack_cond_composed(const ctts_waveglow_config* cfg, int32_t k, const ctts_waveglow_flow_weights* w, void* packed,
+                                     void* stream) {
+    Plan p;
+    int rc = make_plan(cfg, p, CTTS_WG_OPT_COMPOSED_COND); if (rc) return rc;
+    CTTS_CHECK_ARG(p.cc, "pack_cond_composed: this config has no composed conditioning (ctts_waveglow_has_composed_cond)");
+    CTTS_CHECK_ARG(k >= 0 && k < p.c.n_flows, "pack_cond_composed: flow %d", k);
+    CTTS_CHECK_ARG(w && packed && w->cond_w[0] && w->cond_w[1] && w->cond_b[0] && w->cond_b[1], "pack_cond_composed: NULL pointer");
+    hipStream_t s = as_stream(stream);
+    float* blob = static_cast<float*>(packed);
+    const int H = p.H;
+    double* w10 = reinterpret_cast<double*>(blob + p.cc_w10) + (size_t)k * H * p.K0;
+    hipLaunchKernelGGL(cond_compose_w10_kernel, dim3((p.K0 + 255) / 256, H), dim3(256), 0, s, w->cond_w[1], w->cond_w[0], w10, H, p.K0);
+    hipLaunchKernelGGL(cond_compose_A_kernel, dim3(p.ccJ * p.c.n_mel_channels, p.ccP), dim3(GEMM_BM), 0, s, w10, blob + p.up_w,
+                       blob + p.cc_A + (size_t)k * p.ccP * p.nch_cc * A_TILE, p.c.n_mel_channels, p.c.n_group, p.c.hop_length,
+                       p.c.win_length, p.ccP, p.nch_cc);
+    hipLaunchKernelGGL(cond_compose_bias_kernel, dim3(1), dim3(GEMM_BM), 0, s, w->cond_w[0], w->cond_b[0], w->cond_w[1], w->cond_b[1],
+                       blob + p.up_b, blob + p.cc_b + (size_t)k * p.ccP * GEMM_BM, p.K0, p.c.n_group, p.ccP);
+    CTTS_CHECK_LAUNCH("cond_compose");
+    return CTTS_OK;
+}
+
 size_t ctts_waveglow_workspace_bytes(const ctts_waveglow_config* cfg, int32_t batch, int32_t frames) {
+    return ctts_waveglow_workspace_bytes_opt(cfg, batch, frames, 0);
+}
+
+size_t ctts_waveglow_workspace_bytes_opt(const ctts_waveglow_config* cfg, int32_t batch, int32_t frames, int32_t options) {
     Plan p; Geom g; Workspace w;
-    if (make_plan(cfg, p) || make_geom(p, frames, g) || batch < 1) return 0;
-    carve(p, g, batch, nullptr, in_form(p, g, tuning()), w);
+    if (make_plan(cfg, p, options) || make_geom(p, frames, g) || batch < 1) return 0;
+    const Tuning t = tuning();
+    carve(p, g, batch, nullptr, in_form(p, g, t), cond_composed(p, frames, t), w);
     return w.total * sizeof(float);
 }
 
@@ -1065,6 +1203,20 @@
     const int rc = c.begin(cfg, packed, batch, frames, stream); if (rc) return rc;
     CTTS_CHECK_ARG(packed && spect && h_tmp && h_all && batch >= 1, "wn_cond: bad argument");
     return c.cond(spect, spk_rows, h_tmp, h_all);
+}
+
+size_t ctts_wn_cond_composed_scratch_bytes(const ctts_waveglow_config* cfg, int32_t batch, int32_t frames) {
+    Plan p;
+    if (make_plan(cfg, p, CTTS_WG_OPT_COMPOSED_COND) || !p.cc || batch < 1 || frames < 1) return 0;
+    return (size_t)batch * p.c.n_mel_channels * mel_geom(frames).ld * sizeof(float);
+}
+
+int ctts_wn_cond_composed_f32(const ctts_waveglow_config* cfg, const void* packed, const float* mel, float* scratch, float* h_all,
+                              int32_t batch, int32_t frames, void* stream) {
+    WnCall c;
+    const int rc = c.begin(cfg, packed, batch, frames, stream, CTTS_WG_OPT_COMPOSED_COND); if (rc) return rc;
+    CTTS_CHECK_ARG(packed && mel && scratch && h_all && batch >= 1, "wn_cond_composed: bad argument");
+    return c.cond_from_mel(mel, scratch, h_all);
 }
 
 int ctts_wn_stack_f32(const ctts_waveglow_config* cfg, const void* packed, int32_t flow, const float* audio,
@@ -1121,7 +1273,8 @@
     Plan p; Geom g; Workspace w; FwdSums f;
     if (make_plan(cfg, p) || make_geom(p, frames, g)) return 0;
     if (batch < 1) { set_error("forward_workspace_bytes: batch=%d", batch); return 0; }
-    carve_fwd(p, g, batch, nullptr, in_form(p, g, tuning()), w, f);
+    const Tuning t = tuning();
+    carve_fwd(p, g, batch, nullptr, in_form(p, g, t), cond_composed(p, frames, t), w, f);
     return f.total * sizeof(float);
 }
 
@@ -1180,8 +1333,15 @@
 int ctts_waveglow_infer_spk_f32(const ctts_waveglow_config* cfg, const void* packed, const float* mel,
                                 const float* z_scaled, const int64_t* speaker_ids, float* wave, int32_t batch,
                                 int32_t frames, void* workspace, size_t workspace_bytes, void* stream) {
+    return ctts_waveglow_infer_spk_f32_opt(cfg, packed, mel, z_scaled, speaker_ids, wave, batch, frames, workspace, workspace_bytes, 0,
+                                           stream);
+}
+
+int ctts_waveglow_infer_spk_f32_opt(const ctts_waveglow_config* cfg, const void* packed, const float* mel,
+                                    const float* z_scaled, const int64_t* speaker_ids, float* wave, int32_t batch,
+                                    int32_t frames, void* workspace, size_t workspace_bytes, int32_t options, void* stream) {
     WnCall c;
-    int rc = c.begin(cfg, packed, batch, frames, stream); if (rc) return rc;
+    int rc = c.begin(cfg, packed, batch, frames, stream, options); if (rc) return rc;
     CTTS_CHECK_ARG(packed && mel && z_scaled && wave && workspace && batch >= 1, "infer: bad argument");
     if ((rc = c.take_workspace("infer", workspace, workspace_bytes, false))) return rc;
     CTTS_CHECK_HIP(hipMemcpyAsync(c.audio, z_scaled, (size_t)batch * c.p.c.n_group * c.g.L * sizeof(float), hipMemcpyDeviceToDevice, c.s));
diff --git a/cookietts_amd/waveglow.py b/cookietts_amd/waveglow.py
--- a/cookietts_amd/waveglow.py
+++ b/cookietts_amd/waveglow.py
@@ -85,7 +85,7 @@
 
 
 _MODES = {
-    "f32": (None, None, "ctts_waveglow_workspace_bytes", "ctts_waveglow_infer_spk_f32"),
+    "f32": (None, None, "ctts_waveglow_workspace_bytes_opt", "ctts_waveglow_infer_spk_f32_opt"),
     "bf16": ("ctts_waveglow_packed_bf16_bytes", "ctts_waveglow_pack_flow_bf16", "ctts_waveglow_workspace_bf16_bytes",
              "ctts_waveglow_infer_spk_bf16"),
     "bf16x3": ("ctts_waveglow_packed_bf16x3_bytes", "ctts_waveglow_pack_flow_bf16x3", "ctts_waveglow_workspace_bf16x3_bytes",
@@ -158,6 +158,7 @@
 
         self._compute_dtype = torch.float32
         self._f32_gemm_mode = None
+        self._composed_cond = True
         self._fwd = None
 
     def c_config(self):
@@ -168,6 +169,12 @@
             win_length=self.win_length, hop_length=self.hop_length, n_layers=wn['n_layers'],
             n_channels=wn['n_channels'], kernel_size=wn['kernel_size'], cond_hidden=256,
             speaker_embed_dim=wn.get('speaker_embed_dim', 0), f32_gemm_mode=_lib.model_gemm_mode(self._f32_gemm_mode))
+
+    def _options(self):
+        if not (self._composed_cond and self.upsample_mode == 'normal' and not self.multispeaker and self._mode() == "f32"):
+            return 0
+        cfg = self.c_config()
+        return _lib.WG_OPT_COMPOSED_COND if _lib.lib().ctts_waveglow_has_composed_cond(C.byref(cfg)) else 0
 
     def set_f32_gemm_mode(self, mode):
         _lib.model_gemm_mode(mode)
@@ -227,7 +234,8 @@
             if p.device != device:
                 raise RuntimeError(f"parameter on {p.device}, input on {device}: move the model first")
         cfg = self.c_config()
-        nbytes = _lib.nbytes(lib.ctts_waveglow_packed_bytes, C.byref(cfg), what="unsupported WaveGlow config")
+        options = self._options()
+        nbytes = _lib.nbytes(lib.ctts_waveglow_packed_bytes_opt, C.byref(cfg), options, what="unsupported WaveGlow config")
         with torch.cuda.device(device):
             stream = _lib.stream(device)
             blob = torch.zeros(nbytes // 4, dtype=torch.float32, device=device)
@@ -282,6 +290,9 @@
                     fw.speaker_embed = _cache.dev(wn.speaker_embed.weight, keep)
                 _lib.check(lib.ctts_waveglow_pack_flow(C.byref(cfg), k, C.byref(fw), _lib.ptr(blob), stream),
                            f"ctts_waveglow_pack_flow({k})")
+                if options & _lib.WG_OPT_COMPOSED_COND:
+                    _lib.check(lib.ctts_waveglow_pack_cond_composed(C.byref(cfg), k, C.byref(fw), _lib.ptr(blob), stream),
+                               f"ctts_waveglow_pack_cond_composed({k})")
                 if bblob is not None:
                     _lib.check(getattr(lib, pack16)(C.byref(cfg), k, C.byref(fw), _lib.ptr(bblob), stream), f"{pack16}({k})")
             torch.cuda.current_stream(device).synchronize()
@@ -320,13 +331,14 @@
         mode = self._mode()
         _, _, ws_bytes, infer = _MODES[mode]
         cfg = self.c_config()
-        nbytes = _lib.nbytes(getattr(lib, ws_bytes), C.byref(cfg), B, F, what="workspace query failed")
+        opt = (self._options(),) if mode == "f32" else ()
+        nbytes = _lib.nbytes(getattr(lib, ws_bytes), C.byref(cfg), B, F, *opt, what="workspace query failed")
         ws = self.workspace((device, B, F, mode, nbytes), lambda: nbytes)
         wave = torch.empty(B, L * self.n_group, dtype=torch.float32, device=device)
         blobs = (blob,) if bblob is None else (blob, bblob)
         with torch.cuda.device(device):
             _lib.check(getattr(lib, infer)(C.byref(cfg), *map(_lib.ptr, blobs), _lib.ptr(mel), _lib.ptr(z), _lib.ptr(ids),
-                                           _lib.ptr(wave), B, F, _lib.ptr(ws), ws.numel() * 4, _lib.stream(device)), infer)
+                                           _lib.ptr(wave), B, F, _lib.ptr(ws), ws.numel() * 4, *opt, _lib.stream(device)), infer)
         return wave.to(spect.dtype)
 
     def infer(self, spect, speaker_id=None, sigma=1.0):
diff --git a/include/cookietts_hip.h b/include/cookietts_hip.h
--- a/include/cookietts_hip.h
+++ b/include/cookietts_hip.h
@@ -20,6 +20,7 @@
 #define CTTS_GEMM_F32 1
 #define CTTS_GEMM_BF16X3 2
 #define CTTS_GEMM_BF16X6 3
+#define CTTS_WG_OPT_COMPOSED_COND 1
 #define CTTS_N_SPEAKERS 512
 
 int ctts_abi_version(void);
@@ -129,6 +130,17 @@
 int ctts_wn_stack_f32(const ctts_waveglow_config* cfg, const void* packed, int32_t flow,
                       const float* audio, const float* h_all, float* x, float* act, float* out,
                       int32_t batch, int32_t frames, void* stream);
+int ctts_waveglow_has_composed_cond(const ctts_waveglow_config* cfg);
+size_t ctts_waveglow_packed_bytes_opt(const ctts_waveglow_config* cfg, int32_t options);
+int ctts_waveglow_pack_cond_composed(const ctts_waveglow_config* cfg, int32_t flow, const ctts_waveglow_flow_weights* w,
+                                     void* packed, void* stream);
+size_t ctts_waveglow_workspace_bytes_opt(const ctts_waveglow_config* cfg, int32_t batch, int32_t frames, int32_t options);
+int ctts_waveglow_infer_spk_f32_opt(const ctts_waveglow_config* cfg, const void* packed, const float* mel,
+                                    const float* z_scaled, const int64_t* speaker_ids, float* wave, int32_t batch,
+                                    int32_t frames, void* workspace, size_t workspace_bytes, int32_t options, void* stream);
+size_t ctts_wn_cond_composed_scratch_bytes(const ctts_waveglow_config* cfg, int32_t batch, int32_t frames);
+int ctts_wn_cond_composed_f32(const ctts_waveglow_config* cfg, const void* packed, const float* mel, float* scratch,
+                              float* h_all, int32_t batch, int32_t frames, void* stream);
 int ctts_flow_tail_f32(const ctts_waveglow_config* cfg, const void* packed, int32_t flow,
                        const float* out, float* audio, float* wave, int32_t batch,
                        int32_t frames, void* stream);
```

Measured after the change: 4.022 million samples/s, median of 6. +1.7%, better.
